# Project-MONAI/MONAI

Hardware: AMD Instinct MI355X
Metric: voxels/s sliding-window 3D seg (512^3 vol, 96^3 win, ov 0.5) at 1/8 GPU (higher is better)
Workload: dtype f32; 1 GPU; BasicUNet 5-class seed 1, 512^3 CT phantom in HBM, 96^3 win ov 0.5 gaussian, sw_batch 4 (engine: <= 64 windows per launch); parallelism=1 GPU

## Files before the change

include/monai_amd.h:

```cpp
#ifndef MONAI_AMD_H
#define MONAI_AMD_H

#include <stddef.h>
#include <stdint.h>

#ifdef __cplusplus
extern "C" {
#endif

#define MH_OK 0
#define MH_ERR_ARG (-1)
#define MH_ERR_LAUNCH (-2)
#define MH_ERR_UNSUPPORTED (-3)

typedef struct mh_tensor5 {
    float* data;
    int64_t n_stride;
    const float* nrm;
    int64_t nrm_n_stride;
    int32_t N, C, D, H, W;
} mh_tensor5;

int mh_version(void);
const char* mh_last_error(void);



int mh_window_extract_f32(const float* vol, int C, int D, int H, int W, const int32_t* sz, int nz,
                          const int32_t* sy, int ny, const int32_t* sx, int nx, int w0, int nwin, int rd, int rh,
                          int rw, float* out, void* stream);

int mh_sw_blend_f32(const float* logits, int64_t window_stride, const float* imp, float* out, int K, int D, int H, int W,
                    int rd, int rh, int rw, const int32_t* sz, int nz, const int32_t* sy, int ny, const int32_t* sx,
                    int nx, int premultiplied, void* stream);

int mh_sw_blend_buffered_f32(const float* logits, int64_t window_stride, const float* imp, float* out, int K, int D, int H, int W, int rd, int rh, int rw,
                             const int32_t* sz, int nz, const int32_t* sy, int ny, const int32_t* sx, int nx, int buffer_axis, int buffer_steps, int premultiplied, void* stream);

int mh_sw_mosaic_class_counts(int n, int log2m, int32_t* counts5);
int mh_sw_blend_mosaic_f32(const float* logits, const int64_t* class_base, int log2m_z, int log2m_y, int log2m_x, const float* imp, int imp_factored, float* out, int K,
                           int D, int H, int W, int rd, int rh, int rw, const int32_t* sz, int nz, const int32_t* sy, int ny, const int32_t* sx, int nx,
                           void* stream);

int mh_sw_blend_argmax_f32(const float* logits, int64_t window_stride, const float* imp, void* labels, int labels_u8, int K, int D,
                           int H, int W, int rd, int rh, int rw, const int32_t* sz, int nz, const int32_t* sy, int ny,
                           const int32_t* sx, int nx, int premultiplied, void* stream);

int mh_patch_accumulate_f32(float* values, uint8_t* counts, const float* patch, int NC, int D, int H, int W, int pd, int ph,
                            int pw, int z0, int y0, int x0, void* stream);
int mh_patch_accumulate_batch_f32(float* values, uint8_t* counts, const float* patches, int npatch, const int32_t* loc, int NC, int D, int H, int W,
                                  int pd, int ph, int pw, void* stream);
int mh_avg_finalize_f32(float* values, const uint8_t* counts, int64_t n, void* stream);


#define MH_ALGO_AUTO 0
#define MH_ALGO_DIRECT 1
#define MH_ALGO_WINO2D 2
#define MH_ALGO_H2 3
#define MH_ALGO_FP32 4
int mh_conv3d_k3_select(int algo, int input_bounded, int Cin, int Cout, int D, int H, int W);
int mh_conv3d_k3_num_configs(void);
int mh_conv3d_k3_h2_config(void);
int mh_conv3d_k3_h2c_config(void);
int mh_conv3d_k3_c1_config(void);
int mh_conv3d_k3_h2v_config(void);
int mh_conv3d_k3_h2w_config(void);
int mh_conv3d_k3_h2w_fits(int D, int H, int W);
int mh_conv3d_k3_accepts(int cfg, int Cin, int Cout);
int64_t mh_conv3d_k3_packed_floats(int cfg, int Cin, int Cout);
int mh_conv3d_k3_pack_f32(int cfg, const float* w, int Cin, int Cout, float* packed, void* stream);
int mh_conv3d_k3_stat_tiles(int cfg, int D, int H, int W);
int mh_conv3d_k3_f32(int cfg, const mh_tensor5* in, const float* packed_w, const float* bias,
                     const mh_tensor5* out, float* stats, void* stream);
int mh_conv3d_k3_pool_accepts(int cfg, int Cin, int Cout, int D, int H, int W);
int mh_conv3d_k3_pool_f32(int cfg, const mh_tensor5* in, const float* packed_w, const float* bias, const mh_tensor5* out, float* stats, float* pool_max, float* pool_min,
                          int64_t pool_n_stride, void* stream);
int mh_pool_select_f32(float* pool_max, const float* pool_min, const float* nrm, int64_t nrm_n_stride, int N, int C, int64_t n_stride, int64_t vol, void* stream);
int mh_conv3d_k3_accumulate_f32(int cfg, const mh_tensor5* in, const float* packed_w, const float* bias, const mh_tensor5* out, float* stats, void* stream);

int mh_instnorm_stat_tiles(int D, int H, int W);
int mh_instnorm_stats_f32(const mh_tensor5* x, float* stats, void* stream);
int mh_instnorm_finalize_f32(const float* stats, int tiles, int N, int C, const float* gamma, const float* beta,
                             float eps, float slope, float* nrm, int64_t nrm_n_stride, void* stream);
int mh_groupnorm_finalize_f32(const float* stats, int tiles, int N, int C, int groups, const float* gamma, const float* beta, float eps,
                              float slope, float* nrm, int64_t nrm_n_stride, void* stream);

int mh_nrm_identity_f32(float* nrm, int N, int C, int64_t nrm_n_stride, void* stream);

int mh_maxpool2_f32(const mh_tensor5* in, const mh_tensor5* out, void* stream);

int mh_deconv_k2s2_f32(const mh_tensor5* in, const float* w, const float* bias, const mh_tensor5* out,
                       void* stream);

int mh_deconv_k2s2_h2_accepts(int Cin, int Cout, int D, int H, int W);
int64_t mh_deconv_k2s2_h2_packed_floats(int Cin, int Cout);
int mh_deconv_k2s2_h2_pack_f32(const float* w, int Cin, int Cout, float* packed, void* stream);
int mh_deconv_k2s2_h2_f32(const mh_tensor5* in, const float* packed, const float* bias, const mh_tensor5* out, void* stream);

int mh_upconv_k4s2_accepts(int Cin, int Cout, int Dl, int Hl, int Wl);
int64_t mh_upconv_k4s2_packed_floats(int Cin, int Cout);
int mh_upconv_k4s2_pack_f32(const float* w4, int Cin, int Cout, float* packed, void* stream);
int mh_upconv_k4s2_stat_tiles(int Dl, int Hl, int Wl);
int mh_upconv_k4s2_f32(const mh_tensor5* low, const float* packed, const float* bias_table, const mh_tensor5* out, int accumulate, float* stats, void* stream);

int mh_conv3d_k3s2_accepts(int Cin, int Cout, int D, int H, int W);
int64_t mh_conv3d_k3s2_packed_floats(int Cin, int Cout);
int64_t mh_conv3d_k3s2_workspace_floats(int N, int Cin, int D, int H, int W);
int mh_conv3d_k3s2_stat_tiles(int D, int H, int W);
int mh_conv3d_k3s2_pack_f32(const float* w, int Cin, int Cout, float* packed, void* stream);
int mh_conv3d_k3s2_f32(const mh_tensor5* in, const float* packed, const float* bias, const mh_tensor5* out, float* workspace, float* stats, int fused, void* stream);

int mh_conv1x1_f32(const mh_tensor5* in, const float* w, const float* bias, const mh_tensor5* out,
                   void* stream);
int mh_conv1x1_stat_tiles(int D, int H, int W);
int mh_conv1x1_stats_f32(const mh_tensor5* in, const float* w, const float* bias, const mh_tensor5* out, float* stats, void* stream);

int mh_conv1x1_h2_accepts(int Cin, int Cout, int D, int H, int W);
int64_t mh_conv1x1_h2_packed_floats(int Cin, int Cout);
int mh_conv1x1_h2_pack_f32(const float* w, int Cout, int Cin, float* packed, void* stream);
int mh_conv1x1_h2_f32(const mh_tensor5* in, const float* packed, const float* bias, const mh_tensor5* out, float* stats, void* stream);

int mh_conv1x1_windows_f32(const mh_tensor5* in, const float* w, const float* bias, float* base, int Cout, const int64_t* place, void* stream);


int mh_add_act_f32(const mh_tensor5* a, const mh_tensor5* b, float slope, const mh_tensor5* out, void* stream);

int mh_conv1x1_sum2_accepts(int Cout, int D, int H, int W);
int mh_conv1x1_sum2_f32(const mh_tensor5* a, const mh_tensor5* b, float slope, const float* w, const float* bias, const mh_tensor5* out, void* stream);

int mh_pad_replicate_f32(const mh_tensor5* in, const mh_tensor5* out, void* stream);

int mh_pixelshuffle_f32(const mh_tensor5* in, const mh_tensor5* out, int fz, int pad_pool, void* stream);

int mh_attention_f32(const float* qkv, float* out, int B, int S, int heads, int head_dim, float scale, void* stream);

int mh_window_attention_f32(const float* qkv, const float* bias_t, const float* mask, float* out, int BW, int nW, int S, int heads,
                            int head_dim, float scale, int exact_fp32, void* stream);

int mh_window_attention_rel_accepts(int S, int head_dim, int table_rows);
int mh_window_attention_rel_f32(const float* qkv, const float* rel_table, int table_rows, const int32_t* coord, int coord_off, const int32_t* region,
                                float* out, int BW, int nW, int S, int heads, int head_dim, float scale, void* stream);

int64_t mh_linear_packed_floats(int N, int K);
int mh_linear_pack_f32(const float* w, int N, int K, float* packed, void* stream);
int mh_linear_f32(const float* x, const float* packed_w, const float* bias, const float* residual, float* y, int64_t M, int N, int K, int act,
                  void* stream);
int mh_linear_tile_f32(const float* x, const float* packed_w, const float* bias, const float* residual, float* y, int64_t M, int N, int K, int act,
                       int tile, void* stream);

int mh_layernorm_f32(const float* x, const float* gamma, const float* beta, float eps, float* y, int64_t M, int K, void* stream);

int mh_layernorm_gather_accepts(int K);
int mh_layernorm_gather_f32(const float* x, const float* gamma, const float* beta, float eps, float* y, int64_t M_out, int K, const int32_t* src_row, void* stream);
int mh_linear_scatter_f32(const float* x, const float* packed_w, const float* bias, const float* residual, float* y, int64_t M, int N, int K, int act,
                          const int32_t* dst_row, void* stream);


int mh_conv3d_k3_strided_f32(const mh_tensor5* in, const float* packed_w, const float* bias, const mh_tensor5* out,
                             int stride, void* stream);
int mh_conv3d_k3_strided3_f32(const mh_tensor5* in, const float* packed_w, const float* bias, const mh_tensor5* out, int sz, int sy, int sx,
                              void* stream);
int mh_deconv_ks_f32(const mh_tensor5* in, const float* w, const float* bias, const mh_tensor5* out, int fz, int fy, int fx, void* stream);

int mh_deconv_k3_f32(const mh_tensor5* in, const float* w, const float* bias, const mh_tensor5* out, int stride,
                     void* stream);


int64_t mh_affine_resample_workspace_bytes(int Do, int Ho, int Wo);
int mh_affine_resample_f32(const float* src, int NC, int Di, int Hi, int Wi, float* dst, int Do, int Ho, int Wo,
                           const double* m, int mode, int pad, int align_corners, int compute_f64, void* workspace,
                           void* stream);

int mh_grid_resample_f32(const float* src, int NC, int Di, int Hi, int Wi, const void* coords, int coords_f64,
                         const double* scale3, const double* offset3, float* dst, int Do, int Ho, int Wo, int mode,
                         int pad, int align_corners, int compute_f64, void* stream);

int mh_grid_pull(const void* src, const void* grid, void* out, int is_f64, int B, int C, int X, int Y, int Z, int Xo,
                 int Yo, int Zo, const int32_t* bound3, const int32_t* interp3, int extrapolate, void* stream);

int mh_pushpull(const void* source, const void* grid, const void* target, void* out, void* grad, int is_f64, int ndim, int B,
                int C, int X, int Y, int Z, int Xo, int Yo, int Zo, const int32_t* bound3, const int32_t* interp3,
                int extrapolate, int do_pull, int do_push, int do_count, int do_grad, int do_sgrad, int target_k, void* stream);


int mh_pointwise_f32(int op, const float* src, float* dst, int64_t n, float param, void* stream);
int mh_channel_reduce_f32(int op, const float* src, float* dst, int C, int64_t n, void* stream);
int mh_onehot_f32(const float* labels, float* dst, int K, int64_t n, void* stream);


int mh_scale_intensity_range_f32(const float* src, float* dst, int64_t n, float a_min, float a_div, int rescale, float b_scale, float b_min,
                                 int clip_lo, float lo, int clip_hi, float hi, void* stream);
int mh_foreground_bbox_workspace_ints(int D, int H);
int mh_foreground_bbox_f32(const float* src, int C, int D, int H, int W, int32_t* workspace, int32_t* box6, void* stream);
int mh_crop_pad_f32(const float* src, float* dst, int C, int D, int H, int W, int Do, int Ho, int Wo, int sz, int sy, int sx, float value,
                    void* stream);

int64_t mh_normalize_stats_workspace_doubles(int C, int64_t n);
int mh_normalize_stats_f32(const float* src, int C, int64_t n, int nonzero, double* workspace, float* subdiv, void* stream);
int mh_normalize_apply_f32(const float* src, float* dst, int C, int64_t n, int nonzero, const float* subdiv, void* stream);
int64_t mh_minmax_workspace_floats(int C, int64_t n);
int mh_minmax_f32(const float* src, int C, int64_t n, float* workspace, float* table, void* stream);
int mh_minmax_scale_f32(const float* src, float* dst, int C, int64_t n, const float* table, int rescale, float b_scale, float b_min,
                        int flat_has_mul, float flat_mul, void* stream);
int64_t mh_select_workspace_bytes(int C);
int mh_order_statistics_f32(const float* src, int C, int64_t n, int R, const int64_t* ranks, void* workspace, float* out, void* stream);
int mh_percentiles_f32(const float* src, int C, int64_t n, int P, const int64_t* ranks, const double* weights, int lerp_mode, void* workspace, float* table,
                       void* stream);
int mh_scale_intensity_table_f32(const float* src, float* dst, int C, int64_t n, const float* table, int rescale, float b_scale, float b_min, int flat_add,
                                 int clip_lo, float lo, int clip_hi, float hi, void* stream);
int mh_clamp_table_f32(const float* src, float* dst, int C, int64_t n, const float* table, void* stream);
int mh_flip_permute_f32(const float* src, float* dst, int C, const int32_t* in_size3, const int32_t* perm3, const int32_t* flip3, void* stream);


#define MH_OV_CHANNEL 0
#define MH_OV_LABELS 1
#define MH_OV_F32 0
#define MH_OV_U8 1
#define MH_OV_I64 2
int64_t mh_overlap_sums_workspace_bytes(int B, int K, int64_t n);
int mh_overlap_sums(const void* pred, int pred_form, int pred_dtype, const void* truth, int truth_form, int truth_dtype, int B, int K,
                    int64_t n, void* workspace, double* out, void* stream);


#define MH_ED_BOOL 3
#define MH_ED_ITEM_WORDS 16

int64_t mh_surface_bbox_workspace_bytes(int B, int nc);
int mh_surface_bbox(const void* pred, int pred_form, int pred_dtype, const void* truth, int truth_form, int truth_dtype, int B, int K, int c0,
                    int nc, int D, int H, int W, void* workspace, int32_t* boxes, void* stream);
// ... 60 lines not shown
```

monai_amd/_lib.py:

```python

from __future__ import annotations

import ctypes as C
import os
from typing import Optional, Sequence

import torch

from ._fallback import UnsupportedOnDevice

_HERE = os.path.dirname(os.path.abspath(__file__))
LIB_PATH = os.environ.get("MONAI_AMD_LIB") or os.path.join(_HERE, "csrc", "libmonai_amd.so")


class MhTensor5(C.Structure):

    _fields_ = [
        ("data", C.c_void_p),
        ("n_stride", C.c_int64),
        ("nrm", C.c_void_p),
        ("nrm_n_stride", C.c_int64),
        ("N", C.c_int32),
        ("C", C.c_int32),
        ("D", C.c_int32),
        ("H", C.c_int32),
        ("W", C.c_int32),
    ]


_I, _L, _P, _F = C.c_int, C.c_int64, C.c_void_p, C.c_float
_T = C.POINTER(MhTensor5)
_IA = C.POINTER(C.c_int32)

SIGNATURES = {
    "mh_version": (_I, []),
    "mh_last_error": (C.c_char_p, []),
    "mh_window_extract_f32": (_I, [_P, _I, _I, _I, _I, _IA, _I, _IA, _I, _IA, _I, _I, _I, _I, _I, _I, _P, _P]),
    "mh_patch_accumulate_f32": (_I, [_P, _P, _P] + [_I] * 10 + [_P]),
    "mh_patch_accumulate_batch_f32": (_I, [_P, _P, _P, _I, _IA] + [_I] * 7 + [_P]),
    "mh_avg_finalize_f32": (_I, [_P, _P, C.c_int64, _P]),
    "mh_pointwise_f32": (_I, [_I, _P, _P, _L, _F, _P]),
    "mh_channel_reduce_f32": (_I, [_I, _P, _P, _I, _L, _P]),
    "mh_onehot_f32": (_I, [_P, _P, _I, _L, _P]),
    "mh_scale_intensity_range_f32": (_I, [_P, _P, _L, _F, _F, _I, _F, _F, _I, _F, _I, _F, _P]),
    "mh_foreground_bbox_workspace_ints": (_I, [_I, _I]),
    "mh_foreground_bbox_f32": (_I, [_P, _I, _I, _I, _I, _P, _P, _P]),
    "mh_crop_pad_f32": (_I, [_P, _P] + [_I] * 10 + [_F, _P]),
    "mh_sw_blend_f32": (_I, [_P, _L, _P, _P, _I, _I, _I, _I, _I, _I, _I, _IA, _I, _IA, _I, _IA, _I, _I, _P]),
    "mh_sw_blend_buffered_f32": (_I, [_P, _L, _P, _P, _I, _I, _I, _I, _I, _I, _I, _IA, _I, _IA, _I, _IA, _I, _I, _I, _I, _P]),
    "mh_sw_mosaic_class_counts": (_I, [_I, _I, _IA]),
    "mh_sw_blend_mosaic_f32": (_I, [_P, C.POINTER(C.c_int64), _I, _I, _I, _P, _I, _P, _I, _I, _I, _I, _I, _I, _I, _IA, _I, _IA, _I, _IA, _I, _P]),
    "mh_sw_blend_argmax_f32": (_I, [_P, _L, _P, _P, _I, _I, _I, _I, _I, _I, _I, _I, _IA, _I, _IA, _I, _IA, _I, _I, _P]),
    "mh_conv3d_k3_select": (_I, [_I, _I, _I, _I, _I, _I, _I]),
    "mh_conv3d_k3_h2_config": (_I, []),
    "mh_conv3d_k3_h2c_config": (_I, []),
    "mh_conv3d_k3_c1_config": (_I, []),
    "mh_conv3d_k3_h2v_config": (_I, []),
    "mh_conv3d_k3_h2w_config": (_I, []),
    "mh_conv3d_k3_h2w_fits": (_I, [_I, _I, _I]),
    "mh_conv3d_k3_num_configs": (_I, []),
    "mh_conv3d_k3_accepts": (_I, [_I, _I, _I]),
    "mh_conv3d_k3_packed_floats": (_L, [_I, _I, _I]),
    "mh_conv3d_k3_pack_f32": (_I, [_I, _P, _I, _I, _P, _P]),
    "mh_conv3d_k3_stat_tiles": (_I, [_I, _I, _I, _I]),
    "mh_conv3d_k3_f32": (_I, [_I, _T, _P, _P, _T, _P, _P]),
    "mh_conv3d_k3_accumulate_f32": (_I, [_I, _T, _P, _P, _T, _P, _P]),
    "mh_conv3d_k3_pool_accepts": (_I, [_I, _I, _I, _I, _I, _I]),
    "mh_conv3d_k3_pool_f32": (_I, [_I, _T, _P, _P, _T, _P, _P, _P, _L, _P]),
    "mh_pool_select_f32": (_I, [_P, _P, _P, _L, _I, _I, _L, _L, _P]),
    "mh_instnorm_stat_tiles": (_I, [_I, _I, _I]),
    "mh_instnorm_stats_f32": (_I, [_T, _P, _P]),
    "mh_instnorm_finalize_f32": (_I, [_P, _I, _I, _I, _P, _P, _F, _F, _P, _L, _P]),
    "mh_groupnorm_finalize_f32": (_I, [_P, _I, _I, _I, _I, _P, _P, _F, _F, _P, _L, _P]),
    "mh_flip_permute_f32": (_I, [_P, _P, _I, _IA, _IA, _IA, _P]),
    "mh_normalize_stats_workspace_doubles": (_L, [_I, _L]),
    "mh_normalize_stats_f32": (_I, [_P, _I, _L, _I, _P, _P, _P]),
    "mh_normalize_apply_f32": (_I, [_P, _P, _I, _L, _I, _P, _P]),
    "mh_minmax_workspace_floats": (_L, [_I, _L]),
    "mh_minmax_f32": (_I, [_P, _I, _L, _P, _P, _P]),
    "mh_minmax_scale_f32": (_I, [_P, _P, _I, _L, _P, _I, _F, _F, _I, _F, _P]),
    "mh_select_workspace_bytes": (_L, [_I]),
    "mh_order_statistics_f32": (_I, [_P, _I, _L, _I, C.POINTER(C.c_int64), _P, _P, _P]),
    "mh_percentiles_f32": (_I, [_P, _I, _L, _I, C.POINTER(C.c_int64), C.POINTER(C.c_double), _I, _P, _P, _P]),
    "mh_scale_intensity_table_f32": (_I, [_P, _P, _I, _L, _P, _I, _F, _F, _I, _I, _F, _I, _F, _P]),
    "mh_clamp_table_f32": (_I, [_P, _P, _I, _L, _P, _P]),
    "mh_nrm_identity_f32": (_I, [_P, _I, _I, _L, _P]),
    "mh_maxpool2_f32": (_I, [_T, _T, _P]),
    "mh_deconv_k2s2_f32": (_I, [_T, _P, _P, _T, _P]),
    "mh_upconv_k4s2_accepts": (_I, [_I, _I, _I, _I, _I]),
    "mh_upconv_k4s2_packed_floats": (_L, [_I, _I]),
    "mh_upconv_k4s2_pack_f32": (_I, [_P, _I, _I, _P, _P]),
    "mh_upconv_k4s2_stat_tiles": (_I, [_I, _I, _I]),
    "mh_upconv_k4s2_f32": (_I, [_T, _P, _P, _T, _I, _P, _P]),
    "mh_deconv_k2s2_h2_accepts": (_I, [_I, _I, _I, _I, _I]),
    "mh_deconv_k2s2_h2_packed_floats": (_L, [_I, _I]),
    "mh_deconv_k2s2_h2_pack_f32": (_I, [_P, _I, _I, _P, _P]),
    "mh_deconv_k2s2_h2_f32": (_I, [_T, _P, _P, _T, _P]),
    "mh_conv3d_k3s2_accepts": (_I, [_I, _I, _I, _I, _I]),
    "mh_conv3d_k3s2_packed_floats": (_L, [_I, _I]),
    "mh_conv3d_k3s2_workspace_floats": (_L, [_I, _I, _I, _I, _I]),
    "mh_conv3d_k3s2_stat_tiles": (_I, [_I, _I, _I]),
    "mh_conv3d_k3s2_pack_f32": (_I, [_P, _I, _I, _P, _P]),
    "mh_conv3d_k3s2_f32": (_I, [_T, _P, _P, _T, _P, _P, _I, _P]),
    "mh_conv1x1_f32": (_I, [_T, _P, _P, _T, _P]),
    "mh_conv1x1_stat_tiles": (_I, [_I, _I, _I]),
    "mh_conv1x1_stats_f32": (_I, [_T, _P, _P, _T, _P, _P]),
    "mh_conv1x1_h2_accepts": (_I, [_I, _I, _I, _I, _I]),
    "mh_conv1x1_h2_packed_floats": (_L, [_I, _I]),
    "mh_conv1x1_h2_pack_f32": (_I, [_P, _I, _I, _P, _P]),
    "mh_conv1x1_h2_f32": (_I, [_T, _P, _P, _T, _P, _P]),
    "mh_conv1x1_sum2_accepts": (_I, [_I, _I, _I, _I]),
    "mh_conv1x1_sum2_f32": (_I, [_T, _T, _F, _P, _P, _T, _P]),
    "mh_conv1x1_windows_f32": (_I, [_T, _P, _P, _P, _I, C.POINTER(C.c_int64), _P]),
    "mh_conv3d_k3_strided_f32": (_I, [_T, _P, _P, _T, _I, _P]),
    "mh_conv3d_k3_strided3_f32": (_I, [_T, _P, _P, _T, _I, _I, _I, _P]),
    "mh_deconv_ks_f32": (_I, [_T, _P, _P, _T, _I, _I, _I, _P]),
    "mh_deconv_k3_f32": (_I, [_T, _P, _P, _T, _I, _P]),
    "mh_add_act_f32": (_I, [_T, _T, _F, _T, _P]),
    "mh_pad_replicate_f32": (_I, [_T, _T, _P]),
    "mh_pixelshuffle_f32": (_I, [_T, _T, _I, _I, _P]),
    "mh_attention_f32": (_I, [_P, _P, _I, _I, _I, _I, _F, _P]),
    "mh_window_attention_f32": (_I, [_P, _P, _P, _P, _I, _I, _I, _I, _I, _F, _I, _P]),
    "mh_window_attention_rel_accepts": (_I, [_I, _I, _I]),
    "mh_window_attention_rel_f32": (_I, [_P, _P, _I, _P, _I, _P, _P, _I, _I, _I, _I, _I, _F, _P]),
    "mh_linear_packed_floats": (_L, [_I, _I]),
    "mh_linear_pack_f32": (_I, [_P, _I, _I, _P, _P]),
    "mh_linear_f32": (_I, [_P, _P, _P, _P, _P, _L, _I, _I, _I, _P]),
    "mh_linear_tile_f32": (_I, [_P, _P, _P, _P, _P, _L, _I, _I, _I, _I, _P]),
    "mh_layernorm_f32": (_I, [_P, _P, _P, _F, _P, _L, _I, _P]),
    "mh_layernorm_gather_accepts": (_I, [_I]),
    "mh_layernorm_gather_f32": (_I, [_P, _P, _P, _F, _P, _L, _I, _P, _P]),
    "mh_linear_scatter_f32": (_I, [_P, _P, _P, _P, _P, _L, _I, _I, _I, _P, _P]),
    "mh_affine_resample_workspace_bytes": (_L, [_I, _I, _I]),
    "mh_affine_resample_f32": (_I, [_P, _I, _I, _I, _I, _P, _I, _I, _I, C.POINTER(C.c_double), _I, _I, _I, _I, _P, _P]),
    "mh_separable_filter3d_f32": (_I, [_P, _P, _I, _I, _I, _I, C.POINTER(C.c_float), _I, C.POINTER(C.c_float), _I, C.POINTER(C.c_float), _I, _P]),
    "mh_median_filter_accepts": (_I, [_I, _I, _I, _I, _I, _I]),
    "mh_median_filter_f32": (_I, [_P, _P, _I, _I, _I, _I, _I, _I, _I, _P]),
    "mh_spline_workspace_bytes": (_L, [_I] * 7),
    "mh_spline_prefilter_f64": (_I, [_P, _P] + [_I] * 7 + [_P]),
    "mh_spline_resample_affine_f32": (_I, [_P, _I, _I, _I, _I, _I, _P, _I, _I, _I, C.POINTER(C.c_double), _I, _I, _P]),
    "mh_spline_resample_grid_f32": (_I, [_P, _I, _I, _I, _I, _I, _P, _I, C.POINTER(C.c_double), C.POINTER(C.c_double), _P, _I, _I, _I, _I, _I, _P]),
    "mh_grid_pull": (_I, [_P, _P, _P, _I, _I, _I, _I, _I, _I, _I, _I, _I, _IA, _IA, _I, _P]),
    "mh_pushpull": (_I, [_P, _P, _P, _P, _P] + [_I] * 10 + [_IA, _IA] + [_I] * 7 + [_P]),
    "mh_grid_resample_f32": (_I, [_P, _I, _I, _I, _I, _P, _I, C.POINTER(C.c_double), C.POINTER(C.c_double), _P, _I, _I, _I, _I, _I, _I, _I, _P]),
    "mh_overlap_sums_workspace_bytes": (_L, [_I, _I, _L]),
    "mh_overlap_sums": (_I, [_P, _I, _I, _P, _I, _I, _I, _I, _L, _P, _P, _P]),
    "mh_surface_bbox_workspace_bytes": (_L, [_I, _I]),
    "mh_surface_bbox": (_I, [_P, _I, _I, _P, _I, _I] + [_I] * 7 + [_P, _P, _P]),
    "mh_mask_edges": (_I, [_P, _I, _I, _I, _I, _I, _I, _I, _I, _P, _P, _I, _L, _P, _P]),
    "mh_edt_workspace_bytes": (_L, [_L, _I]),
    "mh_edt": (_I, [_P, _I, _I, _P, _P, _I, _L, _I, _P, _P, _I, _P]),
    "mh_surface_records_workspace_bytes": (_L, [_I]),
    "mh_surface_records": (_I, [_P, _P, _I, _P, _P, _I, _L, _I, _P, _P, _P, _L, _P]),
    "mh_cc_label": (_I, [_P, _I, _L, _I, _I, _P, _P, _I, _L, _P, _P]),
    "mh_cc_records": (_I, [_P, _I, _P, _P, _I, _L, _P, _P, _P]),
    "mh_cc_keep": (_I, [_P, _I, _L, _P, _P, _I, _I, _P, _P, _I, _L, _P]),
    "mh_cc_fill": (_I, [_P, _I, _L, _P, _P, _I, _P, _P, _I, _L, _P]),
    "mh_cc_filter": (_I, [_P, _P, _I, _L, C.POINTER(C.c_double), _I, _P]),
}


class KernelRejected(RuntimeError):
    """An entry point declined a VALID call it has no kernel for (MH_ERR_UNSUPPORTED: a size / shape rule) without launching: callers with an alternative
    path catch THIS, not RuntimeError.  Bad arguments (MH_ERR_ARG: null pointers, mismatched shapes, misalignment -- caller bugs), launch failures and HIP
    errors stay plain RuntimeErrors and must surface."""


class Library:

    def __init__(self, path: str):
        if not os.path.exists(path):
            raise RuntimeError(
                f"monai_amd: HIP extension not built ({path} missing). Run `python -m monai_amd.build` "
                "(hipcc --offload-arch=gfx950); there is no CPU fallback."
            )
        self.path = path
        self._dll = C.CDLL(path)
        for name, (res, args) in SIGNATURES.items():
            fn = getattr(self._dll, name)
            fn.restype, fn.argtypes = res, args
            setattr(self, "_" + name, fn)

    def last_error(self) -> str:
        return self._mh_last_error().decode("utf-8", "replace")

    def check(self, rc: int) -> None:
        if rc == -3:
            raise KernelRejected(f"monai_amd: {self.last_error()} (code {rc})")
        if rc != 0:
            raise RuntimeError(f"monai_amd: {self.last_error()} (code {rc})")

    def call(self, name: str, *args) -> None:
        self.check(getattr(self, "_" + name)(*args))

    def query(self, name: str, *args) -> int:
        rc = getattr(self, "_" + name)(*args)
        if rc < 0:
            raise RuntimeError(f"monai_amd: {self.last_error()} (code {rc})")
        return int(rc)


_LIB: Optional[Library] = None


def lib() -> Library:
    global _LIB
    if _LIB is None:
        _LIB = Library(LIB_PATH)
    return _LIB


def require_device(*tensors: torch.Tensor, dtypes=(torch.float32,)) -> None:
    for t in tensors:
        if t is None:
            continue
        if not t.is_cuda:
            raise UnsupportedOnDevice(
                "monai_amd: this path runs only on an MI355X (ROCm) device tensor; got a CPU tensor. "
                "There is no CPU fallback in the product path."
            )
        if t.dtype not in dtypes:
# ... 35 lines not shown
```

monai_amd/config.py:

```python
import os

HAS_EXT = True
USE_COMPILED = HAS_EXT and os.getenv("BUILD_MONAI", "0") == "1"


CONV_ALGOS = {"auto": 0, "direct": 1, "wino2d": 2, "h2": 3, "fp32": 4}
CONV_ALGO = None


def conv_algo() -> int:
    name = CONV_ALGO if CONV_ALGO is not None else os.environ.get("MONAI_AMD_CONV_ALGO", "auto")
    try:
        return CONV_ALGOS[str(name).lower()]
    except KeyError:
        raise ValueError(f"monai_amd: unknown convolution family {name!r} (one of {sorted(CONV_ALGOS)})") from None


class conv_algo_scope:

    def __init__(self, name: str):
        if str(name).lower() not in CONV_ALGOS:
            raise ValueError(f"monai_amd: unknown convolution family {name!r} (one of {sorted(CONV_ALGOS)})")
        self.name = str(name).lower()

    def __enter__(self):
        global CONV_ALGO
        self._saved, CONV_ALGO = CONV_ALGO, self.name
        return self

    def __exit__(self, *exc):
        global CONV_ALGO
        CONV_ALGO = self._saved
        return False


UPCAT_FUSED = None


def upcat_fused() -> bool:
    v = UPCAT_FUSED if UPCAT_FUSED is not None else os.environ.get("MONAI_AMD_UPCAT_FUSED", "1")
    return str(v).lower() not in ("0", "false", "off", "no")


UPCAT_ORDER = None


def upcat_order() -> str:
    v = str(UPCAT_ORDER if UPCAT_ORDER is not None else os.environ.get("MONAI_AMD_UPCAT_ORDER", "conv_first")).lower()
    if v not in ("conv_first", "term_first"):
        raise ValueError(f"monai_amd: unknown UpCat order {v!r} (conv_first or term_first)")
    return v


CONV_HALVES = None


def conv_halves() -> bool:
    v = CONV_HALVES if CONV_HALVES is not None else os.environ.get("MONAI_AMD_CONV_HALVES", "1")
    return str(v).lower() not in ("0", "false", "off", "no")


RESIDUAL_ACC = None


def residual_accumulate() -> bool:
    v = RESIDUAL_ACC if RESIDUAL_ACC is not None else os.environ.get("MONAI_AMD_RESIDUAL_ACC", "1")
    return str(v).lower() not in ("0", "false", "off", "no")


POOL_FUSED = None


def pool_fused() -> bool:
    v = POOL_FUSED if POOL_FUSED is not None else os.environ.get("MONAI_AMD_POOL_FUSED", "1")
    return str(v).lower() not in ("0", "false", "off", "no")


STRIDED_H2 = None


def strided_h2() -> bool:
    v = STRIDED_H2 if STRIDED_H2 is not None else os.environ.get("MONAI_AMD_STRIDED_H2", "1")
    return str(v).lower() not in ("0", "false", "off", "no") and conv_algo() in (CONV_ALGOS["auto"], CONV_ALGOS["h2"])


STRIDED_H2_FUSED = None


def strided_h2_fused() -> str:
    v = str(STRIDED_H2_FUSED if STRIDED_H2_FUSED is not None else os.environ.get("MONAI_AMD_STRIDED_H2_FUSED", "auto")).lower()
    return "0" if v in ("0", "false", "off", "no") else ("1" if v in ("1", "true", "on", "yes") else "auto")


SMALL_VOLUME_H2 = None


def small_volume_h2() -> bool:
    v = SMALL_VOLUME_H2 if SMALL_VOLUME_H2 is not None else os.environ.get("MONAI_AMD_SMALL_VOLUME_H2", "1")
    return str(v).lower() not in ("0", "false", "off", "no")


DECONV_H2 = None


def deconv_h2() -> bool:
    v = DECONV_H2 if DECONV_H2 is not None else os.environ.get("MONAI_AMD_DECONV_H2", "1")
    return str(v).lower() not in ("0", "false", "off", "no") and conv_algo() in (CONV_ALGOS["auto"], CONV_ALGOS["h2"])


SWIN_FUSED_MOVES = None


def swin_fused_moves() -> bool:
    v = SWIN_FUSED_MOVES if SWIN_FUSED_MOVES is not None else os.environ.get("MONAI_AMD_SWIN_FUSED_MOVES", "1")
    return str(v).lower() not in ("0", "false", "off", "no")


SWIN_REL_ATTENTION = None


def swin_rel_attention() -> bool:
    v = SWIN_REL_ATTENTION if SWIN_REL_ATTENTION is not None else os.environ.get("MONAI_AMD_SWIN_REL_ATTENTION", "1")
    return str(v).lower() not in ("0", "false", "off", "no")
```

monai_amd/csrc/capi.hip:

```cpp
#include <hip/hip_runtime.h>

#include <stdarg.h>
#include <stdio.h>
#include <stdlib.h>
#include <string.h>

#include "kernels/common.h"
#include "kernels/attention.h"
#include "kernels/conv3d_mfma.h"
#include "kernels/conv3d_wino2p.h"
#include "kernels/conv3d_h2.h"
#include "kernels/conv3d_wino_h2.h"
#include "kernels/upconv_h2.h"
#include "kernels/conv3d_s2_h2.h"
#include "kernels/deconv_h2.h"
#include "kernels/conv3d_vol_h2.h"
#include "kernels/conv3d_c1.h"
#include "kernels/dense.h"
#include "kernels/gaussian.h"
#include "kernels/grid_pull.h"
#include "kernels/pushpull.h"
#include "kernels/post.h"
#include "kernels/metrics.h"
#include "kernels/edt.h"
// ... 238 lines not shown
    }
    WindowGrid g;
    if (int e = fill_grid(g, sz, nz, sy, ny, sx, nx)) return e;
    for (int k0 = 0; k0 < K; k0 += 8) {
        const int kt = K - k0 < 8 ? K - k0 : 8;
        if (v4) launch_blend<4>(kt, blocks_for(total), (hipStream_t)stream, logits, imp, out, K, k0, D, H, W, rd, rh, rw, g, premultiplied ? 1 : 0, window_stride);
        else launch_blend<1>(kt, blocks_for(total), (hipStream_t)stream, logits, imp, out, K, k0, D, H, W, rd, rh, rw, g, premultiplied ? 1 : 0, window_stride);
    }
    return launched("sw_blend");
}

int mh_sw_blend_buffered_f32(const float* logits, int64_t window_stride, const float* imp, float* out, int K, int D, int H, int W, int rd, int rh, int rw,
                             const int32_t* sz, int nz, const int32_t* sy, int ny, const int32_t* sx, int nx, int buffer_axis, int buffer_steps, int premultiplied, void* stream) {
    if (int e = blend_checks("sw_blend_buffered", logits, imp, out, K, D, H, W, rd, rh, rw, sz, nz, sy, ny, sx, nx, window_stride)) return e;
    if (buffer_axis < 0 || buffer_axis > 2 || buffer_steps < 1) return fail(MH_ERR_ARG, "sw_blend_buffered: buffer_axis in 0..2 and buffer_steps >= 1 (got %d, %d)", buffer_axis, buffer_steps);
    const bool v4 = W % 4 == 0 && rw % 4 == 0 && all_mult4(sx, nx);
    const long long total = (long long)D * H * (v4 ? W / 4 : W);
    WindowGrid g;
    if (int e = fill_grid(g, sz, nz, sy, ny, sx, nx)) return e;
    hipStream_t s = (hipStream_t)stream;
    for (int k0 = 0; k0 < K; k0 += 4) {
        const int kt = K - k0 < 4 ? K - k0 : 4;
#define MH_BB(KT_, V_)                                                                                                                                          \
    {                                                                                                                                                          \
        if (premultiplied) hipLaunchKernelGGL((sw_blend_buffered_kernel<KT_, V_, true>), dim3(blocks_for(total)), dim3(256), 0, s, logits, imp, out, K, k0, D, H, W, rd, rh, rw, g, buffer_axis, buffer_steps, (long long)window_stride); \
        else hipLaunchKernelGGL((sw_blend_buffered_kernel<KT_, V_, false>), dim3(blocks_for(total)), dim3(256), 0, s, logits, imp, out, K, k0, D, H, W, rd, rh, rw, g, buffer_axis, buffer_steps, (long long)window_stride);           \
    }
        if (v4) { if (kt == 4) MH_BB(4, 4) else if (kt == 3) MH_BB(3, 4) else if (kt == 2) MH_BB(2, 4) else MH_BB(1, 4) }
        else { if (kt == 4) MH_BB(4, 1) else if (kt == 3) MH_BB(3, 1) else if (kt == 2) MH_BB(2, 1) else MH_BB(1, 1) }
#undef MH_BB
    }
    return launched("sw_blend_buffered");
}

#ifndef MH_BLEND_IDX32_LIMIT
#define MH_BLEND_IDX32_LIMIT (1LL << 31)
#endif
int mh_sw_mosaic_class_counts(int n, int log2m, int32_t* counts5) {
    if (n < 1 || log2m < 0 || log2m > 2 || !counts5) return fail(MH_ERR_ARG, "sw_mosaic_class_counts: bad argument (1, 2 or 4 residue classes)");
    MosaicAxis a;
    mosaic_axis_fill(a, n, log2m);
    for (int c = 0; c < MOSAIC_MAX_CLASSES; ++c) counts5[c] = a.cnt[c];
    return MH_OK;
}

int mh_sw_blend_mosaic_f32(const float* logits, const int64_t* class_base, int log2m_z, int log2m_y, int log2m_x, const float* imp, int imp_factored, float* out, int K,
                           int D, int H, int W, int rd, int rh, int rw, const int32_t* sz, int nz, const int32_t* sy, int ny, const int32_t* sx, int nx,
                           void* stream) {
    int64_t dense = 0;
    if (int e = blend_checks("sw_blend_mosaic", logits, imp, out, K, D, H, W, rd, rh, rw, sz, nz, sy, ny, sx, nx, dense)) return e;
    if (!class_base || log2m_z < 0 || log2m_z > 2 || log2m_y < 0 || log2m_y > 2 || log2m_x < 0 || log2m_x > 2) return fail(MH_ERR_ARG, "sw_blend_mosaic: bad layout");
    if (K < 1 || K > 8) return fail(MH_ERR_UNSUPPORTED, "sw_blend_mosaic: 1 .. 8 classes (got %d): use the window-major layout", K);
    RegGrid rg;
    if (!regular_grid(rg, sz, nz, sy, ny, sx, nx, D, H, W)) return fail(MH_ERR_UNSUPPORTED, "sw_blend_mosaic: irregular window starts (use the window-major layout)");
    if (!(W % 4 == 0 && rw % 4 == 0 && all_mult4(sx, nx) && aligned(logits, 16) && aligned(imp, 16) && aligned(out, 16)) || (imp_factored && (rd + rh) % 4))
        return fail(MH_ERR_UNSUPPORTED, "sw_blend_mosaic: needs W, roi width and window starts divisible by 4 and 16-byte aligned buffers");
    const AxisWin* ax[3] = {&rg.z, &rg.y, &rg.x};
    const int lm[3] = {log2m_z, log2m_y, log2m_x}, rr[3] = {rd, rh, rw};
    for (int a = 0; a < 3; ++a)
        if (ax[a]->n > 2 && (long long)ax[a]->step << lm[a] < rr[a]) return fail(MH_ERR_ARG, "sw_blend_mosaic: %d residue classes do not separate the windows of axis %d", 1 << lm[a], a);
    Mosaic ms;
    mosaic_axis_fill(ms.z, nz, log2m_z); mosaic_axis_fill(ms.y, ny, log2m_y); mosaic_axis_fill(ms.x, nx, log2m_x);
    for (int i = 0; i < MOSAIC_MAX_CLASSES * MOSAIC_MAX_CLASSES * MOSAIC_MAX_CLASSES; ++i) {
        if (class_base[i] % 4) return fail(MH_ERR_ARG, "sw_blend_mosaic: class offsets must be multiples of 4 floats");
        ms.base[i] = class_base[i];
    }
    if (D > 65535) return fail(MH_ERR_UNSUPPORTED, "sw_blend_mosaic: more than 65535 planes (use the window-major layout)");
    const unsigned nb = blocks_for((long long)H * (W / 4));
    hipStream_t s = (hipStream_t)stream;
    long long max_cs = 0, max_zy = 0, max_ext = std::max((long long)rd * rh, (long long)rw);
    for (int a = 0; a < MOSAIC_MAX_CLASSES; ++a)
        for (int b = 0; b < MOSAIC_MAX_CLASSES; ++b) {
            const long long zy = (long long)ms.z.cnt[a] * rd * ((long long)ms.y.cnt[b] * rh);
            max_zy = std::max(max_zy, zy);
            for (int c = 0; c < MOSAIC_MAX_CLASSES; ++c) {
                max_cs = std::max(max_cs, zy * ((long long)ms.x.cnt[c] * rw));
                max_ext = std::max(max_ext, std::max((long long)ms.z.cnt[a] * rd, std::max((long long)ms.y.cnt[b] * rh, (long long)ms.x.cnt[c] * rw)));
            }
        }
    const bool fast = max_cs * K < MH_BLEND_IDX32_LIMIT && max_zy < (1LL << 24) && max_ext < (1LL << 23) && std::max(D, std::max(H, W)) < (1 << 23) && knob_int("MONAI_AMD_BLEND_IDX64", 0) == 0;
#define MH_BM(KT, G_, NT_, SEP_) { if (fast) hipLaunchKernelGGL((sw_blend_mosaic_kernel<KT, G_, NT_, SEP_, true>), dim3(nb, D), dim3(256), 0, s, logits, imp, out, K, D, H, W, rd, rh, rw, rg, ms); \
                                   else hipLaunchKernelGGL((sw_blend_mosaic_kernel<KT, G_, NT_, SEP_, false>), dim3(nb, D), dim3(256), 0, s, logits, imp, out, K, D, H, W, rd, rh, rw, rg, ms); }
#ifdef MH_DEV_KNOBS
    if (K == 5 && !imp_factored) {
        const int g_ = knob_int("MONAI_AMD_BLEND_G", MH_BLEND_G), nt_ = knob_int("MONAI_AMD_BLEND_NT", 0);
        if (g_ == 1 && !nt_) { MH_BM(5, 1, false, false) return launched("sw_blend_mosaic"); }
        if (g_ == 1 && nt_) { MH_BM(5, 1, true, false) return launched("sw_blend_mosaic"); }
        if (g_ == 2 && nt_) { MH_BM(5, 2, true, false) return launched("sw_blend_mosaic"); }
        if (g_ == 4 && !nt_) { MH_BM(5, 4, false, false) return launched("sw_blend_mosaic"); }
        if (g_ == 4 && nt_) { MH_BM(5, 4, true, false) return launched("sw_blend_mosaic"); }
    }
#endif
#define MH_BM_CASE(KT) case KT: if (imp_factored) MH_BM(KT, MH_BLEND_G, false, true) else MH_BM(KT, MH_BLEND_G, false, false) break;
    switch (K) { MH_BM_CASE(1) MH_BM_CASE(2) MH_BM_CASE(3) MH_BM_CASE(4) MH_BM_CASE(5) MH_BM_CASE(6) MH_BM_CASE(7) MH_BM_CASE(8) }
#undef MH_BM_CASE
#undef MH_BM
    return launched("sw_blend_mosaic");
}

int mh_sw_blend_argmax_f32(const float* logits, int64_t window_stride, const float* imp, void* labels, int labels_u8, int K, int D, int H, int W, int rd,
                           int rh, int rw, const int32_t* sz, int nz, const int32_t* sy, int ny, const int32_t* sx, int nx, int premultiplied, void* stream) {
    if (int e = blend_checks("sw_blend_argmax", logits, imp, labels, K, D, H, W, rd, rh, rw, sz, nz, sy, ny, sx, nx, window_stride)) return e;
    if (labels_u8 && K > 256) return fail(MH_ERR_UNSUPPORTED, "sw_blend_argmax: %d classes do not fit a uint8 label", K);
    RegGrid rg;
    if (!regular_grid(rg, sz, nz, sy, ny, sx, nx, D, H, W))
        return fail(MH_ERR_UNSUPPORTED, "sw_blend_argmax: irregular window starts (blend, then argmax)");
    const bool v4 = W % 4 == 0 && rw % 4 == 0 && window_stride % 4 == 0 && all_mult4(sx, nx) && aligned(logits, 16) && aligned(imp, 16) &&
                    aligned(labels, labels_u8 ? 4 : 16);
    const long long total = (long long)D * H * (v4 ? W / 4 : W);
    const bool nt = knob_int("MONAI_AMD_BLEND_NT", MH_BLEND_NT) != 0;
    if (int e = launch_blend_reg<true>(K < 8 ? K : 8, v4, MH_BLEND_G, nt, blocks_for(total), (hipStream_t)stream, logits, imp, labels, K, 0, D, H, W, rd, rh,
                                       rw, rg, premultiplied ? 1 : 0, labels_u8 ? 1 : 0, window_stride))
        return e;
    return launched("sw_blend_argmax");
}

typedef ConvCfg<32, 1, 1, 4, 4, 1, 1, 8, 2> Cfg1;
typedef ConvCfg<16, 2, 1, 4, 4, 1, 1, 8, 2> Cfg2;
typedef ConvCfg<8, 4, 1, 2, 2, 2, 1, 8, 2> Cfg3;
typedef ConvCfg<4, 4, 2, 1, 1, 4, 1, 4, 2> Cfg4;
typedef ConvCfg<4, 4, 2, 1, 1, 4, 2, 2, 2> Cfg5;
typedef ConvCfg<8, 4, 1, 2, 4, 1, 1, 8, 2> Cfg6;
typedef ConvCfg<32, 1, 1, 4, 4, 1, 1, 2, 4> Cfg7;
typedef ConvCfg<32, 1, 1, 4, 4, 1, 1, 4, 3> Cfg8;
typedef ConvCfg<16, 2, 1, 4, 4, 1, 1, 4, 3> Cfg9;
typedef ConvCfg<16, 2, 1, 4, 4, 1, 1, 2, 4> Cfg10;
typedef ConvCfg<8, 4, 1, 2, 2, 2, 1, 4, 3> Cfg11;
typedef ConvCfg<8, 4, 1, 2, 2, 2, 1, 2, 4> Cfg12;
typedef ConvCfg<4, 4, 2, 1, 1, 4, 1, 2, 4> Cfg13;
typedef ConvCfg<8, 4, 1, 2, 4, 1, 1, 2, 4> Cfg14;
#define MH_NUM_CFG 14

struct CfgInfo { int tx, ty, tz, cn, cc; };
#define MH_CFG_ROW(C) {C::TX, C::TY, C::TZ, C::CN, C::CC}
static const CfgInfo kCfg[MH_NUM_CFG + 1] = {
    {0, 0, 0, 0, 0}, MH_CFG_ROW(Cfg1), MH_CFG_ROW(Cfg2), MH_CFG_ROW(Cfg3), MH_CFG_ROW(Cfg4), MH_CFG_ROW(Cfg5),
    MH_CFG_ROW(Cfg6), MH_CFG_ROW(Cfg7), MH_CFG_ROW(Cfg8), MH_CFG_ROW(Cfg9), MH_CFG_ROW(Cfg10), MH_CFG_ROW(Cfg11),
    MH_CFG_ROW(Cfg12), MH_CFG_ROW(Cfg13), MH_CFG_ROW(Cfg14),
};
static const double kPref[MH_NUM_CFG + 1] = {0, 1.00, 1.00, 1.00, 1.00, 0.90, 1.00, 1.06, 1.04, 1.03, 1.05, 1.01, 1.02, 1.01, 1.02};
static inline int cdiv(int a, int b) { return (a + b - 1) / b; }
static inline int cin_padded(int cfg, int Cin) { return cfg == 0 ? Cin : cdiv(Cin, kCfg[cfg].cc) * kCfg[cfg].cc; }
static inline int cout_padded(int cfg, int Cout) { return cfg == 0 ? Cout : cdiv(Cout, kCfg[cfg].cn) * kCfg[cfg].cn; }

#define MH_CFG_WINO2D (MH_NUM_CFG + 1)
#define MH_CFG_H2 (MH_NUM_CFG + 2)
#define MH_CFG_C1 (MH_NUM_CFG + 3)
#define MH_CFG_H2C (MH_NUM_CFG + 5)
#define MH_CFG_H2V (MH_NUM_CFG + 6)
#define MH_CFG_H2W (MH_NUM_CFG + 7)
#ifndef MH_H2W_DEFAULT
#define MH_H2W_DEFAULT 1
#endif
#define MH_CFG_LAST MH_CFG_H2W
static inline bool hv_fits(int D, int H, int W) {
    const long long vol = (long long)D * H * W, padded = (long long)(D + 2) * (H + 2) * (W + 2);
    return vol >= 64 && vol <= 256 && padded <= HV_CELLS;
}
static inline int c1_chunks(int D) { return D >= 48 ? D / 24 : 1; }
static inline int c1_zchunk(int D) { return cdiv(D, c1_chunks(D)); }
static inline int c1_blocks(int D, int H, int W) { return cdiv(W, C1_TX) * cdiv(H, C1_TY) * cdiv(D, c1_zchunk(D)); }
static inline int wino2d_chunks(int D, int H, int W) {
    const int blocks = cdiv(W, W2_B) * cdiv(H, W2_B);
    if (const char* e = knob_str("MONAI_AMD_W2_CHUNKS")) {
        const int v = atoi(e);
        if (v >= 1 && v <= D) return v;
    }
    int nchunk = cdiv(16, blocks);
    if (nchunk > D / 12) nchunk = D / 12;
    if (nchunk < 1) nchunk = 1;
    return nchunk;
}
static inline int wino2d_zchunk(int D, int H, int W) { return cdiv(D, wino2d_chunks(D, H, W)); }
static inline int wino2d_blocks(int D, int H, int W) { return cdiv(W, W2_B) * cdiv(H, W2_B) * cdiv(D, wino2d_zchunk(D, H, W)); }
static inline bool h2_fits(int D, int H, int W) { return (long long)D * H * W * H2_CN * 4 < 0x80000000LL; }
static inline int h2_regions(int H, int W) { return h2_wide(H, W) ? cdiv(W, 32) * cdiv(H, 8) : cdiv(W, H2_B) * cdiv(H, H2_B); }
static inline int h2_zchunk(int D, int H, int W) {
    int nchunk = cdiv(16, h2_regions(H, W));
    if (const char* e = knob_str("MONAI_AMD_W2_CHUNKS")) {
        const int v = atoi(e);
        if (v >= 1 && v <= D) return cdiv(D, v);
    }
    if (nchunk > D / 12) nchunk = D / 12;
    if (nchunk < 1) nchunk = 1;
    return cdiv(D, nchunk);
}
static inline int h2_blocks(int D, int H, int W) { return h2_regions(H, W) * cdiv(D, h2_zchunk(D, H, W)); }
static inline bool hw_fits(int D, int H, int W) { return H >= HWG_BY && W >= HWG_BX && H % HWG_BY == 0 && W % HWG_BX == 0 && D >= 2 && h2_fits(D, H, W); }
static inline int hw_regions(int H, int W) { return (H / HWG_BY) * (W / HWG_BX); }
static inline int hw_zchunk(int D, int H, int W) {
    int nchunk = cdiv(32, hw_regions(H, W));
    if (const char* e = knob_str("MONAI_AMD_HW_CHUNKS")) {
        const int v = atoi(e);
        if (v >= 1 && v <= D) nchunk = v;
    }
    if (nchunk > D / 12) nchunk = D / 12;
    if (nchunk < 1) nchunk = 1;
    int zc = cdiv(D, nchunk);
    zc += zc & 1;
    return zc;
}
static inline int hw_blocks(int D, int H, int W) { return hw_regions(H, W) * cdiv(D, hw_zchunk(D, H, W)); }

int mh_conv3d_k3_num_configs(void) { return MH_CFG_WINO2D; }
int mh_conv3d_k3_h2_config(void) { return MH_CFG_H2; }
int mh_conv3d_k3_h2c_config(void) { return MH_CFG_H2C; }
int mh_conv3d_k3_c1_config(void) { return MH_CFG_C1; }
int mh_conv3d_k3_h2v_config(void) { return MH_CFG_H2V; }
int mh_conv3d_k3_h2w_config(void) { return MH_CFG_H2W; }
int mh_conv3d_k3_h2w_fits(int D, int H, int W) { return hw_fits(D, H, W) ? 1 : 0; }

int mh_conv3d_k3_pool_accepts(int cfg, int Cin, int Cout, int D, int H, int W) {
    if (cfg == MH_CFG_H2W) return Cin == HWG_CIN && Cout >= HWG_CN && Cout % HWG_CN == 0 && D % 2 == 0 && hw_fits(D, H, W);
    if (cfg != MH_CFG_H2 || D < 2 || H < 2 || W < 2 || D % 2 || H % 2 || W % 4) return 0;
    if (!(Cin >= H2_KC && Cin % H2_KC == 0 && Cin <= H2_NRM_MAX && Cout >= H2_CN && Cout % (H2_CN / 2) == 0) || !h2_fits(D, H, W)) return 0;
    return !h2_wide(H, W) && h2_zchunk(D, H, W) % 2 == 0;
}
int mh_conv3d_k3_accepts(int cfg, int Cin, int Cout) {
    if (cfg == 0) return 1;
    if (cfg == MH_CFG_WINO2D) return Cin >= 8 && Cin % 8 == 0 && Cout >= W2_CN && Cout % W2_CN == 0;
    if (cfg == MH_CFG_H2) return Cin >= H2_KC && Cin % H2_KC == 0 && Cin <= H2_NRM_MAX && Cout >= H2_CN && Cout % (H2_CN / 2) == 0;
    if (cfg == MH_CFG_H2C) return Cin >= H2_KC && Cin % H2_KC == 0 && Cin <= H2_NRM_MAX && Cout >= 16 && Cout % 16 == 0;
    if (cfg == MH_CFG_C1) return Cin == 1 && Cout >= 8 && Cout % 8 == 0;
    if (cfg == MH_CFG_H2V) return Cin >= 16 && Cin % 16 == 0 && Cin <= HV_CIN_MAX && Cout >= 32 && Cout % 32 == 0;
    if (cfg == MH_CFG_H2W) return Cin == HWG_CIN && Cout >= HWG_CN && Cout % HWG_CN == 0;
    if (cfg < 0 || cfg > MH_NUM_CFG) return 0;
    return Cout >= 1 && cin_padded(cfg, Cin) <= Cfg1::NRM_MAX;
}

int mh_conv3d_k3_select(int algo, int input_bounded, int Cin, int Cout, int D, int H, int W) {
    if (Cin < 1 || Cout < 1 || D < 1 || H < 1 || W < 1) return fail(MH_ERR_ARG, "conv3d_k3_select: bad argument");
    if (algo < MH_ALGO_AUTO || algo > MH_ALGO_FP32) return fail(MH_ERR_ARG, "conv3d_k3_select: unknown algorithm family %d", algo);
    int best = 0;
    double best_score = 0.0;
    for (int c = 1; c <= MH_NUM_CFG; ++c) {
        const CfgInfo& k = kCfg[c];
        if (!mh_conv3d_k3_accepts(c, Cin, Cout)) continue;
        const double util = (double)D * H * W / ((double)cdiv(D, k.tz) * k.tz * cdiv(H, k.ty) * k.ty * cdiv(W, k.tx) * k.tx);
        const double cpad = ((double)Cin / cin_padded(c, Cin)) * ((double)Cout / cout_padded(c, Cout));
        const double score = util * cpad * (1.0 + 0.02 * (k.cn / 32)) * kPref[c];
        if (score > best_score) { best_score = score; best = c; }
    }
    if (mh_conv3d_k3_accepts(MH_CFG_WINO2D, Cin, Cout) && H % 2 == 0 && W % 8 == 0) {
        const bool big = H % W2_B == 0 && W % W2_B == 0 && D >= 48 && H >= 48 && W >= 48;
        if (algo == MH_ALGO_WINO2D || ((algo == MH_ALGO_AUTO || algo == MH_ALGO_FP32) && big)) best = MH_CFG_WINO2D;
    }
    if ((algo == MH_ALGO_AUTO || algo == MH_ALGO_H2) && input_bounded && mh_conv3d_k3_accepts(MH_CFG_H2, Cin, Cout) && W % 4 == 0 && H >= 8 && W >= 8 && h2_fits(D, H, W))
        best = MH_CFG_H2;
    if ((algo == MH_ALGO_AUTO || algo == MH_ALGO_H2) && input_bounded && Cout == 16 && mh_conv3d_k3_accepts(MH_CFG_H2C, Cin, Cout) && W % 4 == 0 && H >= 8 && W >= 8 && h2_fits(D, H, W)
        && knob_int("MONAI_AMD_H2C", 1) != 0)
        best = MH_CFG_H2C;
    if ((algo == MH_ALGO_AUTO || algo == MH_ALGO_H2) && input_bounded && best != MH_CFG_H2 && best != MH_CFG_H2C && mh_conv3d_k3_accepts(MH_CFG_H2V, Cin, Cout) && hv_fits(D, H, W))
        best = MH_CFG_H2V;
    if (algo == MH_ALGO_AUTO && best == MH_CFG_H2 && mh_conv3d_k3_accepts(MH_CFG_H2W, Cin, Cout) && hw_fits(D, H, W) && D >= 24 && knob_int("MONAI_AMD_H2W", MH_H2W_DEFAULT) != 0)
        best = MH_CFG_H2W;
    if (algo != MH_ALGO_DIRECT && algo != MH_ALGO_WINO2D && mh_conv3d_k3_accepts(MH_CFG_C1, Cin, Cout) && W % 4 == 0 && knob_int("MONAI_AMD_C1", 1) != 0)
        best = MH_CFG_C1;
    return best;
}

int64_t mh_conv3d_k3_packed_floats(int cfg, int Cin, int Cout) {
    if (cfg == MH_CFG_WINO2D) return (int64_t)(Cin / W2_KC) * (Cout / W2_CN) * W2_UBUF;
    if (cfg == MH_CFG_H2) return (int64_t)(Cin / H2_KC) * cdiv(Cout, H2_CN) * H2_WB * 4 + H2_TAIL;
    if (cfg == MH_CFG_H2C) return (int64_t)(Cin / H2_KC) * (Cout / 16) * H2_WB * 4 + H2_TAIL;
    if (cfg == MH_CFG_C1) return (int64_t)27 * Cout;
    if (cfg == MH_CFG_H2V) return (int64_t)Cout * Cin * 27 + H2_TAIL;
    if (cfg == MH_CFG_H2W) return (int64_t)(Cout / HWG_CN) * HWG_WAVES * HWG_OPS * 64 * 4 + H2_TAIL;
    if (cfg < 0 || cfg > MH_NUM_CFG) return fail(MH_ERR_ARG, "conv3d_k3: unknown configuration %d", cfg);
    return (int64_t)cin_padded(cfg, Cin) * cout_padded(cfg, Cout) * 27;
}

int mh_conv3d_k3_pack_f32(int cfg, const float* w, int Cin, int Cout, float* packed, void* stream) {
    if (cfg == MH_CFG_WINO2D) {
        if (!w || !packed || !mh_conv3d_k3_accepts(cfg, Cin, Cout)) return fail(MH_ERR_ARG, "conv3d_k3_pack: in-plane Winograd needs Cin %% 8 == 0, Cout %% 16 == 0");
        if (hipMemsetAsync(packed, 0, sizeof(float) * (size_t)mh_conv3d_k3_packed_floats(cfg, Cin, Cout), (hipStream_t)stream) != hipSuccess)
            return fail(MH_ERR_LAUNCH, "conv3d_k3_pack: memset failed");
        hipLaunchKernelGGL(conv3d_k3_wino2d_pack_kernel, dim3(blocks_for((long long)Cin * Cout)), dim3(256), 0, (hipStream_t)stream, w, Cin, Cout, packed);
        return launched("conv3d_k3_wino2d_pack");
    }
    if (cfg == MH_CFG_H2C) {
        if (!w || !packed || !mh_conv3d_k3_accepts(cfg, Cin, Cout)) return fail(MH_ERR_ARG, "conv3d_k3_pack: the 16-couts fp16 split kernel needs Cin %% 16 == 0, Cout %% 16 == 0");
        const int64_t slab_floats = mh_conv3d_k3_packed_floats(cfg, Cin, Cout) - H2_TAIL;
        float* tail = packed + slab_floats;
        if (hipMemsetAsync(packed, 0, sizeof(float) * (size_t)slab_floats, (hipStream_t)stream) != hipSuccess)
            return fail(MH_ERR_LAUNCH, "conv3d_k3_pack: memset failed");
        hipLaunchKernelGGL(conv3d_k3_h2_scale_kernel, dim3(1), dim3(1024), 0, (hipStream_t)stream, w, (long long)Cin * Cout * 27, tail);
        hipLaunchKernelGGL(conv3d_k3_h2c_pack_kernel, dim3(blocks_for((long long)Cin * Cout)), dim3(256), 0, (hipStream_t)stream, w, Cin, Cout,
                           reinterpret_cast<_Float16*>(packed), tail);
        return launched("conv3d_k3_h2c_pack");
    }
    if (cfg == MH_CFG_H2) {
        if (!w || !packed || !mh_conv3d_k3_accepts(cfg, Cin, Cout)) return fail(MH_ERR_ARG, "conv3d_k3_pack: the fp16 split kernel needs Cin %% 16 == 0, Cout %% 16 == 0, Cout >= 32");
        const int64_t slab_floats = mh_conv3d_k3_packed_floats(cfg, Cin, Cout) - H2_TAIL;
        float* tail = packed + slab_floats;
        if (hipMemsetAsync(packed, 0, sizeof(float) * (size_t)slab_floats, (hipStream_t)stream) != hipSuccess)
            return fail(MH_ERR_LAUNCH, "conv3d_k3_pack: memset failed");
        hipLaunchKernelGGL(conv3d_k3_h2_scale_kernel, dim3(1), dim3(1024), 0, (hipStream_t)stream, w, (long long)Cin * Cout * 27, tail);
        hipLaunchKernelGGL(conv3d_k3_h2_pack_kernel, dim3(blocks_for((long long)Cin * Cout)), dim3(256), 0, (hipStream_t)stream, w, Cin, Cout,
                           reinterpret_cast<_Float16*>(packed), tail);
        return launched("conv3d_k3_h2_pack");
    }
    if (cfg == MH_CFG_H2W) {
        if (!w || !packed || !mh_conv3d_k3_accepts(cfg, Cin, Cout)) return fail(MH_ERR_ARG, "conv3d_k3_pack: the Winograd split kernel needs Cin == 32, Cout %% 32 == 0");
        float* tail = packed + (mh_conv3d_k3_packed_floats(cfg, Cin, Cout) - H2_TAIL);
        hipLaunchKernelGGL(conv3d_k3_h2_scale_kernel, dim3(1), dim3(1024), 0, (hipStream_t)stream, w, (long long)Cin * Cout * 27, tail);
        hipLaunchKernelGGL(conv3d_k3_h2w_scale_fix_kernel, dim3(1), dim3(64), 0, (hipStream_t)stream, tail);
        hipLaunchKernelGGL(conv3d_k3_h2w_pack_kernel, dim3(blocks_for((long long)Cin * Cout)), dim3(256), 0, (hipStream_t)stream, w, Cin, Cout,
                           reinterpret_cast<_Float16*>(packed), tail);
        return launched("conv3d_k3_h2w_pack");
    }
    if (cfg == MH_CFG_H2V) {
        if (!w || !packed || !mh_conv3d_k3_accepts(cfg, Cin, Cout)) return fail(MH_ERR_ARG, "conv3d_k3_pack: the small-volume split kernel needs Cin %% 16 == 0 (<= 768), Cout %% 32 == 0");
        float* tail = packed + (mh_conv3d_k3_packed_floats(cfg, Cin, Cout) - H2_TAIL);
        hipLaunchKernelGGL(conv3d_k3_h2_scale_kernel, dim3(1), dim3(1024), 0, (hipStream_t)stream, w, (long long)Cin * Cout * 27, tail);
        hipLaunchKernelGGL(conv3d_k3_vol_h2_pack_kernel, dim3(blocks_for((long long)Cin * Cout)), dim3(256), 0, (hipStream_t)stream, w, Cin, Cout, Cout % 64 == 0 ? 2 : 1,
                           reinterpret_cast<_Float16*>(packed), tail);
        return launched("conv3d_k3_vol_h2_pack");
    }
    if (cfg == MH_CFG_C1) {
        if (!w || !packed || !mh_conv3d_k3_accepts(cfg, Cin, Cout)) return fail(MH_ERR_ARG, "conv3d_k3_pack: the one-channel kernel needs Cin == 1, Cout %% 8 == 0");
        hipLaunchKernelGGL(conv3d_k3_pack_kernel, dim3(blocks_for(27LL * Cout)), dim3(256), 0, (hipStream_t)stream, w, 1, 1, Cout, Cout, Cout, packed);
        return launched("conv3d_k3_pack");
    }
    if (cfg < 0 || cfg > MH_NUM_CFG || !w || !packed) return fail(MH_ERR_ARG, "conv3d_k3_pack: bad argument");
    const int cn = cfg == 0 ? Cout : kCfg[cfg].cn;
    const int cinp = cin_padded(cfg, Cin), coutp = cout_padded(cfg, Cout);
    hipLaunchKernelGGL(conv3d_k3_pack_kernel, dim3(blocks_for((long long)cinp * coutp * 27)), dim3(256), 0, (hipStream_t)stream, w,
                       Cin, cinp, Cout, coutp, cn, packed);
    return launched("conv3d_k3_pack");
}

int mh_conv3d_k3_stat_tiles(int cfg, int D, int H, int W) {
    if (cfg == MH_CFG_WINO2D) return wino2d_blocks(D, H, W);
    if (cfg == MH_CFG_H2 || cfg == MH_CFG_H2C) return h2_blocks(D, H, W);
    if (cfg == MH_CFG_C1) return c1_blocks(D, H, W);
    if (cfg == MH_CFG_H2V) return 1;
    if (cfg == MH_CFG_H2W) return hw_fits(D, H, W) ? hw_blocks(D, H, W) : 0;
    if (cfg < 1 || cfg > MH_NUM_CFG) return 0;
    const CfgInfo& k = kCfg[cfg];
    return cdiv(W, k.tx) * cdiv(H, k.ty) * cdiv(D, k.tz);
}

template <class Cfg>
static void launch_mfma(const Tensor& in, const float* wp, const float* bias, const Tensor& out, float* stats, hipStream_t s) {
    const int tx = cdiv(out.W, Cfg::TX), ty = cdiv(out.H, Cfg::TY), tz = cdiv(out.D, Cfg::TZ);
    const dim3 grid((unsigned)(tx * ty * tz), (unsigned)cdiv(out.C, Cfg::CN), (unsigned)out.N);
    if (stats)
        hipLaunchKernelGGL((conv3d_k3_mfma_kernel<Cfg, true>), grid, dim3(256), 0, s, in, wp, bias, out, stats, tx, ty, tz);
    else
        hipLaunchKernelGGL((conv3d_k3_mfma_kernel<Cfg, false>), grid, dim3(256), 0, s, in, wp, bias, out, stats, tx, ty, tz);
}

struct PoolOut { float* mx; float* mn; long long n_stride; };
static int conv3d_k3_launch(int cfg, const mh_tensor5* in_, const float* packed_w, const float* bias, const mh_tensor5* out_, float* stats, void* stream, bool accumulate,
                            const PoolOut* pool = nullptr);
int mh_conv3d_k3_pool_accepts(int cfg, int Cin, int Cout, int D, int H, int W);
int mh_conv3d_k3_pool_f32(int cfg, const mh_tensor5* in_, const float* packed_w, const float* bias, const mh_tensor5* out_, float* stats, float* pool_max, float* pool_min,
                          int64_t pool_n_stride, void* stream) {
    if (!in_ || !out_ || !pool_max || !pool_min || !stats || !in_->nrm) return fail(MH_ERR_ARG, "conv3d_k3_pool: input records, statistics and both pooled tensors are required");
    if (!mh_conv3d_k3_pool_accepts(cfg, in_->C, out_->C, out_->D, out_->H, out_->W))
        return fail(MH_ERR_UNSUPPORTED, "conv3d_k3_pool: the pooling epilogue exists for the split-precision configuration on even extents with 16 x 16 regions");
    if (!aligned(pool_max, 8) || !aligned(pool_min, 8) || pool_n_stride % 2 || (long long)out_->C * (out_->D / 2) * (out_->H / 2) * (out_->W / 2) > pool_n_stride)
        return fail(MH_ERR_ARG, "conv3d_k3_pool: pooled tensors must be 8-byte aligned [N][>= C][D/2][H/2][W/2]");
    const PoolOut po{pool_max, pool_min, (long long)pool_n_stride};
    return conv3d_k3_launch(cfg, in_, packed_w, bias, out_, stats, stream, false, &po);
}
int mh_pool_select_f32(float* pool_max, const float* pool_min, const float* nrm, int64_t nrm_n_stride, int N, int C, int64_t n_stride, int64_t vol, void* stream) {
    if (!pool_max || !pool_min || !nrm || N < 1 || C < 1 || vol < 1) return fail(MH_ERR_ARG, "pool_select: bad argument");
    const unsigned nb = (unsigned)std::min<long long>(blocks_for(vol), 64);
    hipLaunchKernelGGL(pool_select_kernel, dim3(nb, (unsigned)C, (unsigned)N), dim3(256), 0, (hipStream_t)stream, pool_max, pool_min, nrm, (long long)nrm_n_stride, (long long)n_stride, (long long)vol);
    return launched("pool_select");
}
int mh_conv3d_k3_f32(int cfg, const mh_tensor5* in_, const float* packed_w, const float* bias, const mh_tensor5* out_,
                     float* stats, void* stream) {
    return conv3d_k3_launch(cfg, in_, packed_w, bias, out_, stats, stream, false);
}
int mh_conv3d_k3_accumulate_f32(int cfg, const mh_tensor5* in_, const float* packed_w, const float* bias, const mh_tensor5* out_,
                                float* stats, void* stream) {
    if ((cfg != MH_CFG_H2 && cfg != MH_CFG_H2C && cfg != MH_CFG_H2W) || !stats || !in_ || !in_->nrm)
        return fail(MH_ERR_UNSUPPORTED, "conv3d_k3_accumulate: the accumulating form exists for the split-precision configuration with input records and statistics");
    return conv3d_k3_launch(cfg, in_, packed_w, bias, out_, stats, stream, true);
}
static int conv3d_k3_launch(int cfg, const mh_tensor5* in_, const float* packed_w, const float* bias, const mh_tensor5* out_,
                            float* stats, void* stream, bool accumulate, const PoolOut* pool) {
    if (!dense_ok(in_) || !dense_ok(out_) || !packed_w) return fail(MH_ERR_ARG, "conv3d_k3: bad tensor");
    const Tensor in = from_c(*in_), out = from_c(*out_);
    if (in.N != out.N || in.D != out.D || in.H != out.H || in.W != out.W) return fail(MH_ERR_ARG, "conv3d_k3: shape mismatch");
    if (cfg < 0 || cfg > MH_CFG_LAST) return fail(MH_ERR_ARG, "conv3d_k3: unknown configuration %d", cfg);
    if (in.nrm && !aligned(in.nrm, 16)) return fail(MH_ERR_ARG, "conv3d_k3: nrm must be 16-byte aligned");
    hipStream_t s = (hipStream_t)stream;
    if (cfg == MH_CFG_C1) {
        if (!mh_conv3d_k3_accepts(cfg, in.C, out.C) || in.W % 4)
            return fail(MH_ERR_ARG, "conv3d_k3: the one-channel kernel needs Cin == 1, Cout %% 8 == 0, W %% 4 == 0 (got %d -> %d, %dx%dx%d)", in.C, out.C,
                        in.D, in.H, in.W);
        if (!aligned(out.data, 16) || out.n_stride % 4 || !aligned(in.data, 16) || in.n_stride % 4 || !aligned(packed_w, 4))
            return fail(MH_ERR_ARG, "conv3d_k3: the one-channel kernel needs 16-byte aligned input and output");
        const int txn = cdiv(out.W, C1_TX), tyn = cdiv(out.H, C1_TY), zc = c1_zchunk(out.D);
        constexpr int cot = 8;
        const dim3 grid((unsigned)(txn * tyn * cdiv(out.D, zc)), (unsigned)(out.C / cot), (unsigned)out.N);
        if (stats && in.nrm) hipLaunchKernelGGL((conv3d_k3_c1_kernel<cot, true, true>), grid, dim3(256), 0, s, in, packed_w, bias, out, stats, txn, tyn, zc);
        else if (stats) hipLaunchKernelGGL((conv3d_k3_c1_kernel<cot, true, false>), grid, dim3(256), 0, s, in, packed_w, bias, out, stats, txn, tyn, zc);
        else if (in.nrm) hipLaunchKernelGGL((conv3d_k3_c1_kernel<cot, false, true>), grid, dim3(256), 0, s, in, packed_w, bias, out, stats, txn, tyn, zc);
        else hipLaunchKernelGGL((conv3d_k3_c1_kernel<cot, false, false>), grid, dim3(256), 0, s, in, packed_w, bias, out, stats, txn, tyn, zc);
        return launched("conv3d_k3_c1");
    }
    if (cfg == MH_CFG_H2W) {
        if (!mh_conv3d_k3_accepts(cfg, in.C, out.C) || !hw_fits(in.D, in.H, in.W))
            return fail(MH_ERR_ARG, "conv3d_k3: the Winograd split kernel needs Cin == 32, Cout %% 32 == 0, H %% 4 == 0, W %% 16 == 0, D*H*W < 2^24 (got %d -> %d, %dx%dx%d)",
                        in.C, out.C, in.D, in.H, in.W);
        if (!in.nrm) return fail(MH_ERR_ARG, "conv3d_k3: the Winograd split kernel needs input records with magnitude bounds");
        if (!aligned(out.data, 16) || out.n_stride % 4 || !aligned(packed_w, 16)) return fail(MH_ERR_ARG, "conv3d_k3: the Winograd split kernel needs 16-byte aligned output and weights");
        if ((accumulate || pool) && !stats) return fail(MH_ERR_ARG, "conv3d_k3: the accumulating / pooling forms leave statistics");
        const int bxn = out.W / HWG_BX, byn = out.H / HWG_BY, zc = hw_zchunk(out.D, out.H, out.W);
        const unsigned nblk = (unsigned)(bxn * byn * cdiv(out.D, zc));
        const long long total = (long long)nblk * (out.C / HWG_CN) * out.N;
        if (total > 0x7fffffffLL) return fail(MH_ERR_UNSUPPORTED, "conv3d_k3: problem too large for one launch");
        const dim3 grid((unsigned)total);
        const uint4* wq = reinterpret_cast<const uint4*>(packed_w);
        const float* tail = packed_w + (mh_conv3d_k3_packed_floats(cfg, in.C, out.C) - H2_TAIL);
        if (pool) hipLaunchKernelGGL((conv3d_k3_h2w_kernel<true, false, true>), grid, dim3(64 * HWG_WAVES), 0, s, in, wq, tail, bias, out, stats, bxn, byn, zc, nblk, pool->mx, pool->mn, pool->n_stride);
        else if (accumulate) hipLaunchKernelGGL((conv3d_k3_h2w_kernel<true, true, false>), grid, dim3(64 * HWG_WAVES), 0, s, in, wq, tail, bias, out, stats, bxn, byn, zc, nblk, (float*)nullptr, (float*)nullptr, 0LL);
        else if (stats) hipLaunchKernelGGL((conv3d_k3_h2w_kernel<true, false, false>), grid, dim3(64 * HWG_WAVES), 0, s, in, wq, tail, bias, out, stats, bxn, byn, zc, nblk, (float*)nullptr, (float*)nullptr, 0LL);
        else hipLaunchKernelGGL((conv3d_k3_h2w_kernel<false, false, false>), grid, dim3(64 * HWG_WAVES), 0, s, in, wq, tail, bias, out, stats, bxn, byn, zc, nblk, (float*)nullptr, (float*)nullptr, 0LL);
        return launched("conv3d_k3_h2w");
    }
    if (cfg == MH_CFG_H2V) {
        if (accumulate || pool) return fail(MH_ERR_UNSUPPORTED, "conv3d_k3: the small-volume split kernel has no accumulating / pooling form");
        if (!mh_conv3d_k3_accepts(cfg, in.C, out.C) || !hv_fits(in.D, in.H, in.W))
            return fail(MH_ERR_ARG, "conv3d_k3: the small-volume split kernel needs Cin %% 16 == 0 (<= 768), Cout %% 32 == 0, 64 <= D*H*W <= 256, (D+2)(H+2)(W+2) <= 512 (got %d -> %d, %dx%dx%d)",
                        in.C, out.C, in.D, in.H, in.W);
        if (!in.nrm) return fail(MH_ERR_ARG, "conv3d_k3: the small-volume split kernel needs input records with magnitude bounds");
        if (!aligned(out.data, 16) || out.n_stride % 4 || !aligned(packed_w, 16)) return fail(MH_ERR_ARG, "conv3d_k3: the small-volume split kernel needs 16-byte aligned output and weights");
        const int ncgw = out.C % 64 == 0 ? 2 : 1;
        const long long total = (long long)(out.C / (32 * ncgw)) * out.N;
        if (total > 0x7fffffffLL) return fail(MH_ERR_UNSUPPORTED, "conv3d_k3: problem too large for one launch");
        const uint4* wq = reinterpret_cast<const uint4*>(packed_w);
        const float* tail = packed_w + (mh_conv3d_k3_packed_floats(cfg, in.C, out.C) - H2_TAIL);
        const dim3 grid((unsigned)total);
        if (ncgw == 2) {
            if (stats) hipLaunchKernelGGL((conv3d_k3_vol_h2_kernel<2, true>), grid, dim3(HV_NT), 0, s, in, wq, tail, bias, out, stats);
            else hipLaunchKernelGGL((conv3d_k3_vol_h2_kernel<2, false>), grid, dim3(HV_NT), 0, s, in, wq, tail, bias, out, stats);
        } else {
            if (stats) hipLaunchKernelGGL((conv3d_k3_vol_h2_kernel<1, true>), grid, dim3(HV_NT), 0, s, in, wq, tail, bias, out, stats);
            else hipLaunchKernelGGL((conv3d_k3_vol_h2_kernel<1, false>), grid, dim3(HV_NT), 0, s, in, wq, tail, bias, out, stats);
        }
        return launched("conv3d_k3_vol_h2");
    }
    if (cfg == MH_CFG_H2 || cfg == MH_CFG_H2C) {
        const bool c16 = cfg == MH_CFG_H2C;
        if (!mh_conv3d_k3_accepts(cfg, in.C, out.C) || in.W % 4)
            return fail(MH_ERR_ARG, "conv3d_k3: the fp16 split kernel needs Cin %% 16 == 0, Cout %% 16 == 0 (>= 32; any multiple of 16 in its 16-couts form), W %% 4 == 0 (got %d -> %d, %dx%dx%d)",
                        in.C, out.C, in.D, in.H, in.W);
        if (!aligned(out.data, 16) || out.n_stride % 4 || !aligned(packed_w, 16))
            return fail(MH_ERR_ARG, "conv3d_k3: the fp16 split kernel needs 16-byte aligned output and weights");
        if (!h2_fits(out.D, out.H, out.W))
            return fail(MH_ERR_UNSUPPORTED, "conv3d_k3: the fp16 split kernel addresses 32 output planes with 32-bit offsets (D*H*W < 2^24 voxels); mh_conv3d_k3_select does not return it beyond");
        const bool wide = h2_wide(out.H, out.W);
        const int bxn = wide ? cdiv(out.W, 32) : cdiv(out.W, H2_B), byn = wide ? cdiv(out.H, 8) : cdiv(out.H, H2_B), zc = h2_zchunk(out.D, out.H, out.W);
        const unsigned nblk = (unsigned)(bxn * byn * cdiv(out.D, zc));
        const long long total = (long long)nblk * (c16 ? out.C / 16 : cdiv(out.C, H2_CN)) * out.N;
        if (total > 0x7fffffffLL) return fail(MH_ERR_UNSUPPORTED, "conv3d_k3: problem too large for one launch");
        const dim3 grid((unsigned)total);
        const uint4* wq = reinterpret_cast<const uint4*>(packed_w);
        const float* tail = packed_w + (mh_conv3d_k3_packed_floats(cfg, in.C, out.C) - H2_TAIL);
#define MH_H2_LAUNCH(RES_, WIDE_, C16_)                                                                                                                  \
    {                                                                                                                                                \
        if (stats && in.nrm) hipLaunchKernelGGL((conv3d_k3_h2_kernel<true, true, RES_, WIDE_, C16_>), grid, dim3(512), 0, s, in, wq, tail, bias, out, stats, bxn, byn, zc, nblk, (float*)nullptr, (float*)nullptr, 0LL);   \
        else if (stats) hipLaunchKernelGGL((conv3d_k3_h2_kernel<true, false, RES_, WIDE_, C16_>), grid, dim3(512), 0, s, in, wq, tail, bias, out, stats, bxn, byn, zc, nblk, (float*)nullptr, (float*)nullptr, 0LL);       \
        else if (in.nrm) hipLaunchKernelGGL((conv3d_k3_h2_kernel<false, true, RES_, WIDE_, C16_>), grid, dim3(512), 0, s, in, wq, tail, bias, out, stats, bxn, byn, zc, nblk, (float*)nullptr, (float*)nullptr, 0LL);      \
        else hipLaunchKernelGGL((conv3d_k3_h2_kernel<false, false, RES_, WIDE_, C16_>), grid, dim3(512), 0, s, in, wq, tail, bias, out, stats, bxn, byn, zc, nblk, (float*)nullptr, (float*)nullptr, 0LL);                 \
    }
        if (pool) {
#define MH_H2_POOL(RES_) hipLaunchKernelGGL((conv3d_k3_h2_kernel<true, true, RES_, false, false, false, true>), grid, dim3(512), 0, s, in, wq, tail, bias, out, stats, bxn, byn, zc, nblk, pool->mx, pool->mn, pool->n_stride)
            if (in.C <= 2 * H2_KC) MH_H2_POOL(true); else MH_H2_POOL(false);
#undef MH_H2_POOL
            return launched("conv3d_k3_h2_pool");
        }
        if (accumulate) {
#define MH_H2_ACC(RES_, WIDE_, C16_) hipLaunchKernelGGL((conv3d_k3_h2_kernel<true, true, RES_, WIDE_, C16_, true>), grid, dim3(512), 0, s, in, wq, tail, bias, out, stats, bxn, byn, zc, nblk, (float*)nullptr, (float*)nullptr, 0LL)
            if (c16) {
                if (in.C <= 2 * H2_KC) { if (wide) MH_H2_ACC(true, true, true); else MH_H2_ACC(true, false, true); }
                else { if (wide) MH_H2_ACC(false, true, true); else MH_H2_ACC(false, false, true); }
            } else {
                if (in.C <= 2 * H2_KC) { if (wide) MH_H2_ACC(true, true, false); else MH_H2_ACC(true, false, false); }
                else { if (wide) MH_H2_ACC(false, true, false); else MH_H2_ACC(false, false, false); }
            }
#undef MH_H2_ACC
            return launched("conv3d_k3_h2_acc");
        }
        if (c16) {
            if (in.C <= 2 * H2_KC) { if (wide) MH_H2_LAUNCH(true, true, true) else MH_H2_LAUNCH(true, false, true) }
            else { if (wide) MH_H2_LAUNCH(false, true, true) else MH_H2_LAUNCH(false, false, true) }
        } else {
            if (in.C <= 2 * H2_KC) { if (wide) MH_H2_LAUNCH(true, true, false) else MH_H2_LAUNCH(true, false, false) }
            else { if (wide) MH_H2_LAUNCH(false, true, false) else MH_H2_LAUNCH(false, false, false) }
        }
#undef MH_H2_LAUNCH
        return launched(c16 ? "conv3d_k3_h2c" : "conv3d_k3_h2");
    }
    if (cfg == MH_CFG_WINO2D) {
        if (!mh_conv3d_k3_accepts(cfg, in.C, out.C) || in.H % 2 || in.W % 8)
            return fail(MH_ERR_ARG, "conv3d_k3: in-plane Winograd needs Cin %% 8 == 0, Cout %% 16 == 0, even H and W %% 8 == 0 (got %d -> %d, %dx%dx%d)",
                        in.C, out.C, in.D, in.H, in.W);
        if (!aligned(out.data, 16) || out.n_stride % 4 || !aligned(packed_w, 16))
            return fail(MH_ERR_ARG, "conv3d_k3: in-plane Winograd needs 16-byte aligned output and weights");
        const int bxn = cdiv(out.W, W2_B), byn = cdiv(out.H, W2_B), zc = wino2d_zchunk(out.D, out.H, out.W);
        const unsigned nblk = (unsigned)(bxn * byn * cdiv(out.D, zc));
        const long long total = (long long)nblk * (out.C / W2_CN) * out.N;
        if (total > 0x7fffffffLL) return fail(MH_ERR_UNSUPPORTED, "conv3d_k3: problem too large for one launch");
        const dim3 grid((unsigned)total);
        if (stats && in.nrm) hipLaunchKernelGGL((conv3d_k3_wino2p_kernel<true, true>), grid, dim3(512), 0, s, in, packed_w, bias, out, stats, bxn, byn, zc, nblk);
        else if (stats) hipLaunchKernelGGL((conv3d_k3_wino2p_kernel<true, false>), grid, dim3(512), 0, s, in, packed_w, bias, out, stats, bxn, byn, zc, nblk);
        else if (in.nrm) hipLaunchKernelGGL((conv3d_k3_wino2p_kernel<false, true>), grid, dim3(512), 0, s, in, packed_w, bias, out, stats, bxn, byn, zc, nblk);
        else hipLaunchKernelGGL((conv3d_k3_wino2p_kernel<false, false>), grid, dim3(512), 0, s, in, packed_w, bias, out, stats, bxn, byn, zc, nblk);
        return launched("conv3d_k3_wino2p");
    }
    if (cfg == 0) {
        if (stats) return fail(MH_ERR_ARG, "conv3d_k3: the direct kernel emits no statistics");
        constexpr int COT = 16;
        const dim3 grid(blocks_for((long long)out.D * out.H * out.W), (unsigned)cdiv(out.C, COT), (unsigned)out.N);
        hipLaunchKernelGGL((conv3d_k3_direct_kernel<COT>), grid, dim3(256), 0, s, in, packed_w, bias, out);
        return launched("conv3d_k3_direct");
    }
    const CfgInfo& k = kCfg[cfg];
    (void)k;
    if (!mh_conv3d_k3_accepts(cfg, in.C, out.C))
        return fail(MH_ERR_ARG, "conv3d_k3: configuration %d does not take Cin=%d Cout=%d", cfg, in.C, out.C);
    if (!aligned(packed_w, 16)) return fail(MH_ERR_ARG, "conv3d_k3: packed weights must be 16-byte aligned");
    switch (cfg) {
        case 1: launch_mfma<Cfg1>(in, packed_w, bias, out, stats, s); break;
        case 2: launch_mfma<Cfg2>(in, packed_w, bias, out, stats, s); break;
        case 3: launch_mfma<Cfg3>(in, packed_w, bias, out, stats, s); break;
        case 4: launch_mfma<Cfg4>(in, packed_w, bias, out, stats, s); break;
        case 5: launch_mfma<Cfg5>(in, packed_w, bias, out, stats, s); break;
        case 6: launch_mfma<Cfg6>(in, packed_w, bias, out, stats, s); break;
        case 7: launch_mfma<Cfg7>(in, packed_w, bias, out, stats, s); break;
        case 8: launch_mfma<Cfg8>(in, packed_w, bias, out, stats, s); break;
        case 9: launch_mfma<Cfg9>(in, packed_w, bias, out, stats, s); break;
        case 10: launch_mfma<Cfg10>(in, packed_w, bias, out, stats, s); break;
        case 11: launch_mfma<Cfg11>(in, packed_w, bias, out, stats, s); break;
        case 12: launch_mfma<Cfg12>(in, packed_w, bias, out, stats, s); break;
        case 13: launch_mfma<Cfg13>(in, packed_w, bias, out, stats, s); break;
        case 14: launch_mfma<Cfg14>(in, packed_w, bias, out, stats, s); break;
    }
    return launched("conv3d_k3_mfma");
}

int mh_instnorm_stat_tiles(int D, int H, int W) {
    return (int)(((long long)D * H * W + STAT_CHUNK - 1) / STAT_CHUNK);
}

int mh_instnorm_stats_f32(const mh_tensor5* x_, float* stats, void* stream) {
    if (!dense_ok(x_) || !stats) return fail(MH_ERR_ARG, "instnorm_stats: bad argument");
    const Tensor x = from_c(*x_);
    const int tiles = mh_instnorm_stat_tiles(x.D, x.H, x.W);
    hipLaunchKernelGGL(instnorm_stats_kernel, dim3((unsigned)tiles, (unsigned)x.C, (unsigned)x.N), dim3(256), 0,
                       (hipStream_t)stream, x, stats, tiles);
    return launched("instnorm_stats");
}

int mh_instnorm_finalize_f32(const float* stats, int tiles, int N, int C, const float* gamma, const float* beta, float eps,
                             float slope, float* nrm, int64_t nrm_n_stride, void* stream) {
    if (!stats || !nrm || tiles < 1 || N < 1 || C < 1 || nrm_n_stride < 4LL * C) return fail(MH_ERR_ARG, "instnorm_finalize: bad argument");
    hipLaunchKernelGGL(instnorm_finalize_kernel, dim3((unsigned)C, (unsigned)N), dim3(64), 0, (hipStream_t)stream, stats, tiles,
                       C, 1, gamma, beta, eps, slope, nrm, (long long)nrm_n_stride);
    return launched("instnorm_finalize");
}

int mh_groupnorm_finalize_f32(const float* stats, int tiles, int N, int C, int groups, const float* gamma, const float* beta, float eps,
                              float slope, float* nrm, int64_t nrm_n_stride, void* stream) {
    if (!stats || !nrm || tiles < 1 || N < 1 || C < 1 || groups < 1 || C % groups || nrm_n_stride < 4LL * C)
        return fail(MH_ERR_ARG, "groupnorm_finalize: bad argument (channels must be divisible by groups)");
    hipLaunchKernelGGL(instnorm_finalize_kernel, dim3((unsigned)groups, (unsigned)N), dim3(64), 0, (hipStream_t)stream, stats, tiles,
                       C, C / groups, gamma, beta, eps, slope, nrm, (long long)nrm_n_stride);
    return launched("groupnorm_finalize");
}
// ... 1792 lines not shown
```

monai_amd/csrc/kernels/conv3d_wino_h2.h:

```cpp
#pragma once
#include "common.h"
#include "conv3d_h2.h"

namespace mh {

constexpr int HWG_BY = 4, HWG_BX = 16;
constexpr int HWG_RY = HWG_BY + 2, HWG_RX = HWG_BX + 2;
constexpr int HWG_NP = HWG_RY * HWG_RX;
constexpr int HWG_PB = 144;
constexpr int HWG_DB = (HWG_NP + 1) * HWG_PB;
constexpr int HWG_ZB = 32 * 1024;
constexpr int HWG_OPS = 24;
constexpr int HWG_CIN = 32, HWG_CN = 32;
constexpr int HWG_WAVES = 8;
constexpr unsigned HWG_DROP = 0x80000000u;

__device__ __forceinline__ void hw_split4(const f32x4 v, u32x2& hi, u32x2& lo) {
    _Float16 h_[4], l_[4];
#pragma unroll
    for (int i = 0; i < 4; ++i) {
        h_[i] = (_Float16)v[i];
        float r = v[i] - (float)h_[i];
        MH_OPAQUE(r);
        l_[i] = (_Float16)r;
    }
    const f16x2 h01 = {h_[0], h_[1]}, h23 = {h_[2], h_[3]}, l01 = {l_[0], l_[1]}, l23 = {l_[2], l_[3]};
    hi = u32x2{__builtin_bit_cast(unsigned, h01), __builtin_bit_cast(unsigned, h23)};
    lo = u32x2{__builtin_bit_cast(unsigned, l01), __builtin_bit_cast(unsigned, l23)};
}

__device__ __forceinline__ f32x4 hw_fma4(const f32x4 a, const float s, const f32x4 c) { return __builtin_elementwise_fma(a, f32x4{s, s, s, s}, c); }
__device__ __forceinline__ void hw_split4p(const f32x4 v, const float m1, u32x2& hi, u32x2& lo) {
#ifdef MH_SIMT_EMULATOR
    f16x2 h01, l01, h23, l23;
    h2_split_pair(v[0], v[1], m1, h01, l01);
    h2_split_pair(v[2], v[3], m1, h23, l23);
    hi = u32x2{__builtin_bit_cast(unsigned, h01), __builtin_bit_cast(unsigned, h23)};
    lo = u32x2{__builtin_bit_cast(unsigned, l01), __builtin_bit_cast(unsigned, l23)};
#else
    unsigned h0, h1, l0, l1;
    asm("v_cvt_pk_f16_f32 %0, %1, %2" : "=v"(h0) : "v"(v[0]), "v"(v[1]));
    asm("v_cvt_pk_f16_f32 %0, %1, %2" : "=v"(h1) : "v"(v[2]), "v"(v[3]));
    asm("v_fma_mixlo_f16 %0, %1, %2, %3 op_sel_hi:[1,0,0]" : "=v"(l0) : "v"(h0), "v"(m1), "v"(v[0]));
    asm("v_fma_mixlo_f16 %0, %1, %2, %3 op_sel_hi:[1,0,0]" : "=v"(l1) : "v"(h1), "v"(m1), "v"(v[2]));
    asm("v_fma_mixhi_f16 %0, %1, %2, %3 op_sel:[1,0,0] op_sel_hi:[1,0,0]" : "+v"(l0) : "v"(h0), "v"(m1), "v"(v[1]));
    asm("v_fma_mixhi_f16 %0, %1, %2, %3 op_sel:[1,0,0] op_sel_hi:[1,0,0]" : "+v"(l1) : "v"(h1), "v"(m1), "v"(v[3]));
    hi = u32x2{h0, h1};
    lo = u32x2{l0, l1};
#endif
}
__device__ __forceinline__ float hw_uniform(const float x) {
#ifdef MH_SIMT_EMULATOR
    return x;
#else
    return __builtin_bit_cast(float, __builtin_amdgcn_readfirstlane(__builtin_bit_cast(int, x)));
#endif
}
__device__ __forceinline__ void hw_xchg32_pair(const float mx, const float mn, const int hi, float& own, float& rcv) {
#ifdef MH_SIMT_EMULATOR
    own = hi ? mn : mx;
    rcv = __shfl_xor(hi ? mx : mn, 32);
#else
    (void)hi;
    const auto r = __builtin_amdgcn_permlane32_swap(__builtin_bit_cast(unsigned, mx), __builtin_bit_cast(unsigned, mn), false, false);
    const unsigned r0 = r[0], r1 = r[1];
    own = __builtin_bit_cast(float, r0);
    rcv = __builtin_bit_cast(float, r1);
#endif
}
#ifdef MH_SIMT_EMULATOR
#define MH_HW_KEEP_BRANCH ((void)0)
#else
#define MH_HW_KEEP_BRANCH asm volatile("" ::: "memory")
#endif

struct HwFinish {
    int co_l, fa, g4, frp, fq;
};
__device__ __forceinline__ HwFinish hw_finish_role(const int wave, const int lane) {
    HwFinish r;
    r.fq = lane & 3;
    r.frp = r.fq & 1;
    r.fa = lane >> 5;
    r.g4 = ((wave >> 1) & 1) ? (r.fq >> 1 ? 2 : 1) : (r.fq >> 1 ? 3 : 0);
    r.co_l = (wave >> 2) * 16 + (wave & 1) * 8 + ((lane >> 2) & 7);
    return r;
}

template <bool STATS, bool ACC = false, bool POOL = false>
__global__ void __launch_bounds__(512)
conv3d_k3_h2w_kernel(Tensor in, const uint4* __restrict__ wp, const float* __restrict__ wtail, const float* __restrict__ bias, Tensor out,
                     float* __restrict__ stats, int bxn, int byn, int zchunk, unsigned nblk, float* __restrict__ pmax, float* __restrict__ pmin,
                     long long pool_n_stride) {
    __shared__ __attribute__((aligned(16))) char smem[3 * HWG_DB + 2 * HWG_ZB];
    __shared__ unsigned bound_s[4];
    char* const ds = smem;
    char* const zs_ = smem + 3 * HWG_DB;
    const int tid = threadIdx.x, lane = tid & 63;
    const int wave = __builtin_amdgcn_readfirstlane(tid >> 6);
    const int wi = wave & 3, jp = wave >> 2;
    const int Cout = out.C, D = out.D, H = out.H, W = out.W;
    const long long HW = (long long)H * W, DHW = (long long)D * HW;

    const unsigned ncg = (unsigned)(Cout / HWG_CN);
    unsigned lid = xcd_remap(blockIdx.x, gridDim.x);
    const int cg = (int)(lid % ncg);
    lid /= ncg;
    const unsigned b = lid % nblk;
    const int n = (int)(lid / nblk);
    const int x0 = (int)(b % bxn) * HWG_BX, y0 = (int)((b / bxn) % byn) * HWG_BY;
    const int zs = (int)(b / (bxn * byn)) * zchunk, ze = min(zs + zchunk, D);
    const int p_first = max(zs - 1, 0), p_last = min(ze, D - 1);

    unsigned soff;
    int loff[2];
    {
        const int pr = min(lane, 53);
        const int ly = pr / 9;
        int lx = 2 * (pr - 9 * ly);
        const int gy = y0 + ly - 1;
        int gx = x0 + lx - 1;
        if (gx < 0) { gx += 1; lx += 1; }
        if (gx + 1 >= W) { gx -= 1; lx -= 1; }
        const bool ok = lane < 54 && gy >= 0 && gy < H;
        soff = ok ? 4u * (unsigned)(gy * W + gx) : 0u;
        loff[0] = (ok ? ly * HWG_RX + lx : HWG_NP) * HWG_PB;
        loff[1] = (ok ? ly * HWG_RX + lx + 1 : HWG_NP) * HWG_PB;
    }
    for (int i = tid; i < (3 * HWG_DB + 2 * HWG_ZB) / 16; i += 512) reinterpret_cast<uint4*>(smem)[i] = make_uint4(0u, 0u, 0u, 0u);
    f32x4 nra, nrb, nrs;
    {
        unsigned mb = 0u;
        if (lane < HWG_CIN) {
            const float4 a = *reinterpret_cast<const float4*>(in.nrm + (long long)n * in.nrm_n_stride + 4LL * lane);
            const unsigned bb = abs_bits(a.w);
            mb = bb == 0u ? 0x7fc00000u : bb;
        }
        mb = wave_umax(mb);
        if (tid == 0) bound_s[0] = mb;
    }
    __syncthreads();
    int e_in = 0;
    bool poisoned = false;
    {
        const unsigned mb = bound_s[0];
        poisoned = mb >= 0x7f800000u;
        e_in = poisoned ? 0 : min(max(13 - ((int)(mb >> 23) - 126), -100), 100);
        const float p_ = __uint_as_float((unsigned)(e_in + 127) << 23);
#pragma unroll
        for (int i = 0; i < 4; ++i) {
            const float4 a = *reinterpret_cast<const float4*>(in.nrm + (long long)n * in.nrm_n_stride + 4LL * (4 * wave + i));
            nra[i] = hw_uniform(a.x * p_); nrb[i] = a.y * p_; nrs[i] = a.z;
        }
    }
    f32x4 nrk;
#pragma unroll
    for (int i = 0; i < 4; ++i) nrk[i] = hw_uniform(nrs[i] <= 1.0f ? __builtin_inff() : -__builtin_inff());
    const auto xrs = __builtin_amdgcn_make_buffer_rsrc(const_cast<float*>(in.data + (long long)n * in.n_stride + (long long)(4 * wave) * DHW), 0, 0x7fffffff, 0x00020000);
    const unsigned hw4 = (unsigned)(HW * 4);
    unsigned voff = soff + (unsigned)p_first * hw4;
    const unsigned cso1 = (unsigned)(DHW * 4), cso2 = 2u * cso1, cso3 = 3u * cso1;
    f32x2 xin[4];
#define MH_HW_LDX                                                                                     \
    {                                                                                                 \
        xin[0] = __builtin_bit_cast(f32x2, __builtin_amdgcn_raw_buffer_load_b64(xrs, voff, 0u, 0));   \
        xin[1] = __builtin_bit_cast(f32x2, __builtin_amdgcn_raw_buffer_load_b64(xrs, voff, cso1, 0)); \
        xin[2] = __builtin_bit_cast(f32x2, __builtin_amdgcn_raw_buffer_load_b64(xrs, voff, cso2, 0)); \
        xin[3] = __builtin_bit_cast(f32x2, __builtin_amdgcn_raw_buffer_load_b64(xrs, voff, cso3, 0)); \
    }
#define MH_HW_CONV(DBO)                                                                               \
    {                                                                                                 \
        char* const db_ = ds + (DBO) + 16 * wave;                                                     \
        f32x4 y_[2];                                                                                  \
        _Pragma("unroll") for (int i = 0; i < 4; ++i) {                                               \
            const f32x2 t_ = __builtin_elementwise_fma(xin[i], f32x2{nra[i], nra[i]}, f32x2{nrb[i], nrb[i]}), u_ = t_ * nrs[i]; \
            _Pragma("unroll") for (int j = 0; j < 2; ++j) y_[j][i] = __builtin_amdgcn_fmed3f(t_[j], u_[j], nrk[i]);       \
        }                                                                                             \
        _Pragma("unroll") for (int j = 0; j < 2; ++j) *reinterpret_cast<f32x4*>(db_ + loff[j]) = y_[j]; \
    }
    int staged = p_first;
#define MH_HW_ADV { voff += staged < p_last ? hw4 : 0u; staged += 1; }

    u32x4 wu[HWG_OPS];
    {
        const u32x4* wg = reinterpret_cast<const u32x4*>(wp) + ((long long)(cg * 8 + wave) * HWG_OPS) * 64 + lane;
#pragma unroll
        for (int r = 0; r < HWG_OPS; ++r) wu[r] = wg[r * 64];
    }
#define MH_HW_U(SL, T, CB, PC) __builtin_bit_cast(f16x8, wu[(((SL) * 3 + (T)) * 2 + (CB)) * 2 + (PC)])

    const int rho = lane & 15, kg = lane >> 4;
    const int tty = (rho >= 4 && rho < 12) ? 1 : 0, ttx = rho < 4 ? rho : rho < 12 ? rho - 4 : rho - 8;
    const int ra = wi == 0 ? 0 : wi == 2 ? 2 : 1, rb = wi == 0 ? 2 : wi == 1 ? 2 : wi == 2 ? 1 : 3;
    const float sgn = wi == 1 ? 1.0f : -1.0f;
    const float fsg = jp ? -1.0f : 1.0f;
    const float m1 = h2_minus_one();
    const int ab0 = ((2 * tty + ra) * HWG_RX + 2 * ttx + jp) * HWG_PB + kg * 16;
    const int ab1 = ((2 * tty + rb) * HWG_RX + 2 * ttx + jp) * HWG_PB + kg * 16;

    f32x4 acc[3][2][2];
#pragma unroll
    for (int s = 0; s < 3; ++s)
#pragma unroll
        for (int j = 0; j < 2; ++j)
#pragma unroll
            for (int c = 0; c < 2; ++c) acc[s][j][c] = f32x4{0.0f, 0.0f, 0.0f, 0.0f};

    const HwFinish fr = hw_finish_role(wave, lane);
    const int fcb = wave >> 2, fty = (wave >> 1) & 1;
    const int fa = fr.fa, fq = fr.fq, frp = fr.frp, g4 = fr.g4;
    const int ftx = 2 * fq;
    const int c16 = fr.co_l & 15;
    const int co_l = fr.co_l, co = cg * HWG_CN + co_l;
    const float bco = bias ? bias[co] : 0.0f;
    const float fs2 = fa ? -1.0f : 1.0f;
    const int zwr = wave * 4096 + (lane ^ ((lane >> 5) * 12)) * 16;
    const int zrd = fa * 4096 + fcb * 2048 + (g4 * 16 + (c16 ^ (fq >> 1 ? 12 : 0))) * 16 + frp * 8;
    float inv_a, inv_b;
    {
        const int t_ = -((int)((__float_as_uint(wtail[1]) >> 23) & 0xffu) - 127) - e_in;
        const int t1_ = t_ / 2, t2_ = t_ - t1_;
        inv_a = hw_uniform(poisoned ? __uint_as_float(0x7fc00000u) : __uint_as_float((unsigned)(t1_ + 127) << 23));
        inv_b = hw_uniform(__uint_as_float((unsigned)(t2_ + 127) << 23));
    }
    const auto orsrc = __builtin_amdgcn_make_buffer_rsrc(out.data + (long long)n * out.n_stride + (long long)(cg * HWG_CN) * DHW, 0, (int)(HWG_CN * DHW * 4), 0x00020000);
    const unsigned ooff = 4u * (unsigned)((long long)co_l * DHW + (long long)(y0 + 2 * fty + fa) * W + x0 + 2 * ftx);
    float pivot = 0.0f;
    bool have_c = false;
    f32x4 s1 = {0.0f, 0.0f, 0.0f, 0.0f}, s2 = s1;
    const long long PHW = (long long)(H / 2) * (W / 2), PDHW = (long long)(D / 2) * PHW;
    float* const pbase_mx = POOL ? pmax + (long long)n * pool_n_stride + (long long)(cg * HWG_CN) * PDHW : out.data;
    float* const pbase_mn = POOL ? pmin + (long long)n * pool_n_stride + (long long)(cg * HWG_CN) * PDHW : out.data;
    const int pbytes = POOL ? (int)(HWG_CN * PDHW * 4) : 0;
    const unsigned phw4 = (unsigned)(PHW * 4);
    const unsigned poff = (4u * (unsigned)((long long)co_l * PDHW + (long long)((y0 >> 1) + fty) * (W / 2) + (x0 >> 1) + ftx)) | (fa ? HWG_DROP : 0u);
    const float pk_ = fa ? -__builtin_inff() : __builtin_inff();
    f32x2 hm = {0.0f, 0.0f};
    f32x4 pv = {0.0f, 0.0f, 0.0f, 0.0f};

    u32x4 ah[2], al[2];
#define MH_HW_XFORM(DBO)                                                                              \
    {                                                                                                 \
        const char* const db_ = ds + (DBO);                                                           \
        _Pragma("unroll") for (int h = 0; h < 2; ++h) {                                               \
            f32x4 r_[3];                                                                              \
            _Pragma("unroll") for (int bq = 0; bq < 3; ++bq) {                                        \
                const f32x4 u_ = *reinterpret_cast<const f32x4*>(db_ + ab0 + bq * HWG_PB + h * 64);   \
                const f32x4 v_ = *reinterpret_cast<const f32x4*>(db_ + ab1 + bq * HWG_PB + h * 64);   \
                r_[bq] = hw_fma4(v_, sgn, u_);                                                        \
            }                                                                                         \
            const f32x4 e_ = hw_fma4(r_[2], m1, r_[0]);                                               \
            f32x4 f_;                                                                                 \
            if (jp) { f_ = hw_fma4(r_[0], m1, r_[1]); MH_HW_KEEP_BRANCH; } else f_ = r_[1] + r_[2];   \
            u32x2 hh_, ll_;                                                                           \
            hw_split4p(e_, m1, hh_, ll_); ah[0][2 * h] = hh_[0]; ah[0][2 * h + 1] = hh_[1]; al[0][2 * h] = ll_[0]; al[0][2 * h + 1] = ll_[1]; \
            hw_split4p(f_, m1, hh_, ll_); ah[1][2 * h] = hh_[0]; ah[1][2 * h + 1] = hh_[1]; al[1][2 * h] = ll_[0]; al[1][2 * h + 1] = ll_[1]; \
        }                                                                                             \
    }
#define MH_HW_MM(S, SL, CB, A, B, FRESH)                                                              \
    acc[S][SL][CB] = __builtin_amdgcn_mfma_f32_16x16x32_f16(__builtin_bit_cast(f16x8, A), B, (FRESH) ? f32x4{0.0f, 0.0f, 0.0f, 0.0f} : acc[S][SL][CB], 0, 0, 0);
#define MH_HW_MMS(S0, S1, S2)                                                                         \
    _Pragma("unroll") for (int sl = 0; sl < 2; ++sl)                                                  \
        _Pragma("unroll") for (int cb = 0; cb < 2; ++cb) {                                            \
            MH_HW_MM(S0, sl, cb, ah[sl], MH_HW_U(sl, 0, cb, 0), true)  MH_HW_MM(S1, sl, cb, ah[sl], MH_HW_U(sl, 1, cb, 0), false) MH_HW_MM(S2, sl, cb, ah[sl], MH_HW_U(sl, 2, cb, 0), false) \
            MH_HW_MM(S0, sl, cb, al[sl], MH_HW_U(sl, 0, cb, 0), false) MH_HW_MM(S1, sl, cb, al[sl], MH_HW_U(sl, 1, cb, 0), false) MH_HW_MM(S2, sl, cb, al[sl], MH_HW_U(sl, 2, cb, 0), false) \
            MH_HW_MM(S0, sl, cb, ah[sl], MH_HW_U(sl, 0, cb, 1), false) MH_HW_MM(S1, sl, cb, ah[sl], MH_HW_U(sl, 1, cb, 1), false) MH_HW_MM(S2, sl, cb, ah[sl], MH_HW_U(sl, 2, cb, 1), false) \
        }
#define MH_HW_SKIP(S0)                                                                                \
    { _Pragma("unroll") for (int sl = 0; sl < 2; ++sl) _Pragma("unroll") for (int cb = 0; cb < 2; ++cb) acc[S0][sl][cb] = f32x4{0.0f, 0.0f, 0.0f, 0.0f}; }
#define MH_HW_ZOUT(S2, Q)                                                                             \
    {                                                                                                 \
        char* const zb_ = zs_ + ((Q) & 1) * HWG_ZB + zwr;                                             \
        _Pragma("unroll") for (int cb = 0; cb < 2; ++cb) {                                            \
            *reinterpret_cast<f32x4*>(zb_ + cb * 2048) = acc[S2][0][cb] + acc[S2][1][cb];             \
            *reinterpret_cast<f32x4*>(zb_ + cb * 2048 + 1024) = acc[S2][1][cb];                       \
        }                                                                                             \
    }
#define MH_HW_FINISH(Q, ON, ST)                                                                       \
    {                                                                                                 \
        const bool on_ = (ST) ? true : (ON);                                                          \
        const char* const zb_ = zs_ + ((Q) & 1) * HWG_ZB + zrd;                                       \
        f32x2 z0_[3], z1_[3];                                                                         \
        _Pragma("unroll") for (int i = 0; i < 3; ++i) {                                               \
            z0_[i] = *reinterpret_cast<const f32x2*>(zb_ + i * 4096) + *reinterpret_cast<const f32x2*>(zb_ + i * 4096 + 16384 + 1024);        \
            z1_[i] = *reinterpret_cast<const f32x2*>(zb_ + i * 4096 + 1024) - *reinterpret_cast<const f32x2*>(zb_ + i * 4096 + 16384);        \
        }                                                                                             \
        const f32x2 fs_ = {fs2, fs2};                                                                 \
        const f32x2 y0_ = __builtin_elementwise_fma(z0_[2], fs_, __builtin_elementwise_fma(z0_[1], fs_, z0_[0])) * inv_a; \
        const f32x2 y1_ = __builtin_elementwise_fma(z1_[2], fs_, __builtin_elementwise_fma(z1_[1], fs_, z1_[0])) * inv_a; \
        f32x4 o_ = {__builtin_fmaf(y0_[0], inv_b, bco), __builtin_fmaf(y1_[0], inv_b, bco), __builtin_fmaf(y0_[1], inv_b, bco), __builtin_fmaf(y1_[1], inv_b, bco)}; \
        if (ACC) o_ += pv;       \
        if (ST) __builtin_amdgcn_raw_buffer_store_b128(__builtin_bit_cast(u32x4, o_), orsrc, ooff, (unsigned)(Q) * hw4, 0); \
        else __builtin_amdgcn_raw_buffer_store_b128(__builtin_bit_cast(u32x4, o_), orsrc, on_ ? ooff + (unsigned)(Q) * hw4 : HWG_DROP, 0, 0); \
        if (STATS) {         \
            if (!(ST)) {                                                                              \
                pivot = (on_ && !have_c) ? o_[0] : pivot;                                             \
                have_c = have_c || on_;                                                               \
            }                                                                                         \
            const f32x4 d_ = o_ - pivot, dw_ = (ST) ? d_ : d_ * (on_ ? 1.0f : 0.0f);                  \
            s1 += dw_;                                                                                \
            s2 = __builtin_elementwise_fma(dw_, d_, s2);                                              \
        }                                                                                             \
        if (POOL && !(HWX_OFF & 32)) {          \
            const f32x2 mx_ = {fmaxf(o_[0], o_[1]), fmaxf(o_[2], o_[3])}, mn_ = {fminf(o_[0], o_[1]), fminf(o_[2], o_[3])}; \
            float own0_, rcv0_, own1_, rcv1_;                                                         \
            hw_xchg32_pair(mx_[0], mn_[0], fa, own0_, rcv0_);                                         \
            hw_xchg32_pair(mx_[1], mn_[1], fa, own1_, rcv1_);                                         \
            const f32x2 y_ = {__builtin_amdgcn_fmed3f(own0_, rcv0_, pk_), __builtin_amdgcn_fmed3f(own1_, rcv1_, pk_)};       \
            const f32x2 f_ = {__builtin_amdgcn_fmed3f(y_[0], hm[0], pk_), __builtin_amdgcn_fmed3f(y_[1], hm[1], pk_)}; \
            const int pn_ = (on_ && ((Q) & 1) && !(HWX_OFF & 64)) ? pbytes : 0;                       \
            const unsigned ps_ = (unsigned)((Q) >> 1) * phw4;                                         \
            __builtin_amdgcn_raw_buffer_store_b64(__builtin_bit_cast(u32x2, f_), __builtin_amdgcn_make_buffer_rsrc(pbase_mx, 0, pn_, 0x00020000), poff, ps_, 0); \
            __builtin_amdgcn_raw_buffer_store_b64(__builtin_bit_cast(u32x2, f_), __builtin_amdgcn_make_buffer_rsrc(pbase_mn, 0, pn_, 0x00020000), poff ^ HWG_DROP, ps_, 0); \
            hm = on_ ? y_ : hm;                                                                       \
        }                                                                                             \
    }
#ifdef HWX_PROF
#define MH_HW_T(K) { const long long t_ = __builtin_readcyclecounter(); tacc[K] += t_ - tlast; tlast = t_; }
    long long tacc[8] = {0, 0, 0, 0, 0, 0, 0, 0}, tlast = __builtin_readcyclecounter();
#else
#define MH_HW_T(K)
#endif
#ifndef HWX_OFF
#define HWX_OFF 0
#endif
#ifndef HWX_DEAL
#define HWX_DEAL 2
#endif
#define MH_HW_DEAL                                                                                    \
    if constexpr (ACC || POOL) {                                                                      \
        _Pragma("unroll") for (int g_ = 0; g_ < 36; ++g_) {                                           \
            __builtin_amdgcn_sched_group_barrier(0x008, 1, 0);                                        \
            __builtin_amdgcn_sched_group_barrier(0x100, 1, 0);                                        \
            __builtin_amdgcn_sched_group_barrier(0x006, HWX_DEAL, 0);                                 \
            __builtin_amdgcn_sched_group_barrier(0x230, 1, 0);                                        \
        }                                                                                             \
    }
#define MH_HW_ITER(P, R, ST)                                                                          \
    {                                                                                                 \
        constexpr int S0 = (3 - (R)) % 3, S1 = (S0 + 1) % 3, S2 = (S0 + 2) % 3;       \
        constexpr int db0 = (R) * HWG_DB, db2 = (((R) + 2) % 3) * HWG_DB;             \
        const int p_ = (P);                                                                           \
        const bool valid_ = (ST) ? true : (p_ >= p_first && p_ <= p_last);                            \
        const int qf_ = p_ - 2;                                                                       \
        if (ACC) {                                                                                    \
            if (ST) pv = __builtin_bit_cast(f32x4, __builtin_amdgcn_raw_buffer_load_b128(orsrc, ooff, (unsigned)qf_ * hw4, 0)); \
            else { const bool nx_ = qf_ >= zs && qf_ < ze; pv = __builtin_bit_cast(f32x4, __builtin_amdgcn_raw_buffer_load_b128(orsrc, nx_ ? ooff + (unsigned)qf_ * hw4 : HWG_DROP, 0, 0)); } \
        }                                                                                             \
        if (valid_) { if (!(HWX_OFF & 1)) MH_HW_XFORM(db0) }                                          \
        MH_HW_T(0)                                                                                    \
        __syncthreads();                                                                              \
        MH_HW_T(1)                                                                                    \
        if (valid_) {                                                                                 \
            __builtin_amdgcn_sched_barrier(0);                                                        \
            if (!(HWX_OFF & 2)) { MH_HW_CONV(db2) MH_HW_LDX MH_HW_ADV }                               \
            if (!(HWX_OFF & 4)) MH_HW_FINISH(qf_, qf_ >= zs && qf_ < ze, ST)                          \
            if (!(HWX_OFF & 8)) MH_HW_MMS(S0, S1, S2)                                                 \
            MH_HW_DEAL                                                                                \
            __builtin_amdgcn_sched_barrier(0);                                                        \
        } else {                                                                                      \
            MH_HW_SKIP(S0)                                                                            \
            if (!(HWX_OFF & 4)) MH_HW_FINISH(qf_, qf_ >= zs && qf_ < ze, false)                       \
        }                                                                                             \
        if (!(HWX_OFF & 16)) if ((ST) || (p_ - 1 >= zs && p_ - 1 < ze)) MH_HW_ZOUT(S2, p_ - 1)        \
        MH_HW_T(2)                                                                                    \
        __syncthreads();                                                                              \
        MH_HW_T(3)                                                                                    \
    }

    {
        const int k0 = p_first - (zs - 1);
        MH_HW_LDX MH_HW_ADV
        __syncthreads();
        MH_HW_CONV((k0 % 3) * HWG_DB)
        MH_HW_LDX MH_HW_ADV
        MH_HW_CONV(((k0 + 1) % 3) * HWG_DB)
        MH_HW_LDX MH_HW_ADV
        __syncthreads();
    }
    if (jp) __syncthreads();
    int p = zs - 1;
#define MH_HW_STEADY(P) ((P) >= zs + 5 && (P) + 2 <= p_last && (P) + 1 < ze)
#define MH_HW_BLOCK(ST) { MH_HW_ITER(p, 0, ST) MH_HW_ITER(p + 1, 1, ST) MH_HW_ITER(p + 2, 2, ST) }
    for (; p <= ze + 1 && !MH_HW_STEADY(p); p += 3) MH_HW_BLOCK(false)
    for (; MH_HW_STEADY(p); p += 3) MH_HW_BLOCK(true)
    for (; p <= ze + 1; p += 3) MH_HW_BLOCK(false)
#undef MH_HW_BLOCK
#undef MH_HW_STEADY
    if (!jp) __syncthreads();
#ifdef HWX_PROF
    if (blockIdx.x == 0 && lane == 0) { _Pragma("unroll") for (int k = 0; k < 8; ++k) reinterpret_cast<long long*>(pmax)[wave * 8 + k] = tacc[k]; }
#endif
#undef MH_HW_T
#undef MH_HW_DEAL
#undef MH_HW_ITER
#undef MH_HW_FINISH
#undef MH_HW_ZOUT
#undef MH_HW_SKIP
#undef MH_HW_MMS
#undef MH_HW_MM
#undef MH_HW_XFORM
#undef MH_HW_U
#undef MH_HW_ADV
#undef MH_HW_CONV
#undef MH_HW_LDX

    if (STATS) {
        Stat run;
        {
            const float a1 = (s1[0] + s1[1]) + (s1[2] + s1[3]), a2 = (s2[0] + s2[1]) + (s2[2] + s2[3]);
            run.n = 4.0f * (float)(ze - zs);
            const float dm = a1 / run.n;
            run.mean = pivot + dm;
            run.m2 = fmaxf(a2 - a1 * dm, 0.0f);
        }
        __syncthreads();
        float* red = reinterpret_cast<float*>(smem);
        {
            int t_ = tid;
            MH_OPAQUE(t_);
            const HwFinish e = hw_finish_role(t_ >> 6, t_ & 63);
            float* leaf = red + (((e.co_l * 2 + e.fa) * 4 + e.g4) * 2 + e.frp) * 3;
            leaf[0] = run.n; leaf[1] = run.mean; leaf[2] = run.m2;
        }
        __syncthreads();
        if (tid < HWG_CN) {
            const auto leaf_of = [&](int a, int g, int rp) {
                const float* l = red + (((tid * 2 + a) * 4 + g) * 2 + rp) * 3;
                Stat s;
                s.n = l[0]; s.mean = l[1]; s.m2 = l[2];
                return s;
            };
            Stat st;
            st.n = 0.0f; st.mean = 0.0f; st.m2 = 0.0f;
#pragma unroll
            for (int w = 0; w < 4; ++w) {
                const int rp = w >> 1, ge = 2 * (w & 1);
                const Stat r0 = stat_merge(leaf_of(0, ge, rp), leaf_of(0, ge + 1, rp)), r1 = stat_merge(leaf_of(1, ge, rp), leaf_of(1, ge + 1, rp));
                st = stat_merge(st, stat_merge(r0, r1));
            }
            float* rec = stats + (((long long)n * Cout + cg * HWG_CN + tid) * nblk + b) * 3;
            rec[0] = st.n; rec[1] = st.mean; rec[2] = st.m2;
        }
    }
}

__global__ void conv3d_k3_h2w_scale_fix_kernel(float* __restrict__ tail) {
    if (threadIdx.x == 0 && blockIdx.x == 0) { tail[0] *= 4.0f; tail[1] *= 0.25f; }
}
__global__ void __launch_bounds__(256)
conv3d_k3_h2w_pack_kernel(const float* __restrict__ w, int Cin, int Cout, _Float16* __restrict__ packed, const float* __restrict__ tail) {
    const int idx = blockIdx.x * 256 + threadIdx.x;
    if (idx >= Cin * Cout) return;
    const int ci = idx % Cin, co = idx / Cin;
    const float s = tail[1];
    const double G[4][3] = {{1.0, 0.0, 0.0}, {0.5, 0.5, 0.5}, {0.5, -0.5, 0.5}, {0.0, 0.0, 1.0}};
    const int cg = co / HWG_CN, cb = (co % HWG_CN) / 16, nn = co % 16;
    const int kg = ci < 16 ? ci / 4 : (ci - 16) / 4, e = ci < 16 ? ci % 4 : 4 + (ci - 16) % 4;
    const int ln = kg * 16 + nn;
    for (int t = 0; t < 3; ++t) {
        double g[3][3], tm[4][3];
        for (int ky = 0; ky < 3; ++ky)
            for (int kx = 0; kx < 3; ++kx) g[ky][kx] = (double)w[((long long)co * Cin + ci) * 27 + t * 9 + ky * 3 + kx];
        for (int i = 0; i < 4; ++i)
            for (int kx = 0; kx < 3; ++kx) tm[i][kx] = G[i][0] * g[0][kx] + G[i][1] * g[1][kx] + G[i][2] * g[2][kx];
        for (int i = 0; i < 4; ++i)
            for (int j = 0; j < 4; ++j) {
                const double u = tm[i][0] * G[j][0] + tm[i][1] * G[j][1] + tm[i][2] * G[j][2];
                _Float16 pc[2];
                h2_split((float)(u * (double)s), pc[0], pc[1]);
                const int jpq = j >> 1, slot = (j == 0 || j == 3) ? 0 : 1;
                for (int p = 0; p < 2; ++p) {
                    const long long r = (((long long)(cg * 8 + jpq * 4 + i) * HWG_OPS) + ((slot * 3 + t) * 2 + cb) * 2 + p) * 64 + ln;
                    packed[r * 8 + e] = pc[p];
                }
            }
    }
}

}
```

monai_amd/networks/_conv_engine.py:

```python

from __future__ import annotations

from typing import Optional

import torch

from .. import _prof, ops

__all__ = ["ConvEngine", "split_configs", "accumulates", "identity_records"]


def split_configs() -> tuple:
    return ops.conv3d_k3_h2_config(), ops.conv3d_k3_h2c_config(), ops.conv3d_k3_h2w_config()


def accumulates(cfg: int) -> bool:
    return cfg in split_configs()


def identity_records(t: torch.Tensor) -> torch.Tensor:
    return ops.nrm_identity(torch.empty((t.shape[0], t.shape[1], 4), dtype=torch.float32, device=t.device))


def _kernel3(w: torch.Tensor) -> torch.Tensor:
    if w.dim() == 4:
        w = w.unsqueeze(2)
    if tuple(w.shape[2:]) == (3, 3, 3):
        return w
    w3 = torch.zeros(w.shape[:2] + (3, 3, 3), dtype=w.dtype, device=w.device)
    w3[(slice(None), slice(None)) + tuple(slice(0, 3) if k == 3 else slice(1, 2) for k in w.shape[2:])] = w
    return w3


class ConvEngine:
    def __init__(self):
        self._derived: dict = {}
        self._scratch: dict = {}

    def derived(self, slot, sources, build, *extra):
        key = tuple((t.data_ptr(), t._version, str(t.device)) for t in sources) + extra
        hit = self._derived.get(slot)
        if hit is None or hit[0] != key:
            hit = self._derived[slot] = (key, build())
        return hit[1]

    def conv3_pack(self, conv, cfg: int, cin: Optional[tuple] = None, cout: Optional[tuple] = None) -> torch.Tensor:
        def build():
            w = _kernel3(conv.weight)
            if cout is not None:
                w = w[cout[0]:cout[1]]
            if cin is not None:
                w = w[:, cin[0]:cin[1]].contiguous()
            return ops.conv3d_k3_pack(cfg, w)

        return self.derived((id(conv), "k3", cfg, cin, cout), [conv.weight], build)

    def conv3s2_pack(self, conv) -> torch.Tensor:
        return self.derived((id(conv), "s2"), [conv.weight], lambda: ops.conv3d_k3s2_pack(conv.weight))

    def conv1x1_h2_pack(self, conv) -> torch.Tensor:
        return self.derived((id(conv), "1x1"), [conv.weight], lambda: ops.conv1x1_h2_pack(conv.weight.view(conv.weight.shape[0], -1)))

    def upconv_pack(self, conv, dec, at: int):
        def build():
            w4, table = ops.upconv_k4s2_weights(dec.weight, dec.bias, conv.weight[:, at:])
            return ops.upconv_k4s2_pack(w4), table

        return self.derived((id(conv), "upconv"), [conv.weight, dec.weight] + ([dec.bias] if dec.bias is not None else []), build)

    def linear_pack(self, weight: torch.Tensor) -> torch.Tensor:
        return self.derived((id(weight), "lin"), [weight], lambda: ops.linear_pack(weight.reshape(weight.shape[0], -1)))

    def scalar(self, param: torch.Tensor) -> float:
        return self.derived((id(param), "scalar"), [param], lambda: float(param.detach().float().cpu()))

    def bn_fold(self, bn, slope: float) -> torch.Tensor:
        if bn.running_mean is None or bn.running_var is None:
            raise NotImplementedError("monai_amd: BatchNorm without running statistics is not on the (inference) HIP path")

        def build():
            invstd = 1.0 / torch.sqrt(bn.running_var.float() + bn.eps)
            alpha = invstd * bn.weight.float() if bn.affine else invstd
            beta = (bn.bias.float() if bn.affine else 0.0) - bn.running_mean.float() * alpha
            return torch.stack([alpha, beta, torch.full_like(alpha, slope), torch.zeros_like(alpha)], dim=1).contiguous()

        return self.derived((id(bn), "bn"), [bn.running_mean, bn.running_var] + ([bn.weight, bn.bias] if bn.affine else []), build, slope)

    def act_records(self, slope: float, n: int, c: int, device) -> torch.Tensor:
        return self.derived(("act", slope, n, c, str(device)), [],
                            lambda: torch.tensor([1.0, 0.0, slope, 0.0], dtype=torch.float32, device=device).repeat(n, c, 1).contiguous())

    def _buf(self, what: str, floats: int, device) -> torch.Tensor:
        buf = self._scratch.get((what, device))
        if buf is None or buf.numel() < floats:
            buf = self._scratch[(what, device)] = torch.empty(floats, dtype=torch.float32, device=device)
        return buf

    def stats_buf(self, floats: int, device) -> torch.Tensor:
        return self._buf("stats", floats, device)

    def epilogue_stats(self, cfg: int, out):
        n, cout, d, h, w = out.shape
        tiles = ops.conv3d_k3_stat_tiles(cfg, d, h, w)
        return (self.stats_buf(n * cout * tiles * 3, out.device), tiles) if tiles else (None, 0)

    def launch3(self, cfg: int, x, x_nrm, packed, bias, out, want_stats: bool = True, accumulate: bool = False, pool=None, stats=None):
        n, cout, d, h, w = out.shape
        own, tiles = self.epilogue_stats(cfg, out) if want_stats else (None, 0)
        stats = (own if stats is None else stats) if tiles else None
        with _prof.span(f"conv3d_k3/cfg{cfg}", 2.0 * 27 * x.shape[1] * cout * d * h * w * n):
            if pool is not None:
                ops.conv3d_k3_pool(cfg, x, x_nrm, packed, bias, out, stats, *pool)
            else:
                ops.conv3d_k3(cfg, x, x_nrm, packed, bias, out, stats, accumulate=accumulate)
        return stats, tiles

    def conv3(self, conv, x, x_nrm, stride=1, out=None, *, bounded: bool, want_stats: bool = True, tiny_direct: bool = False, accumulate: bool = False, pool=None):
        n, cin, d, h, w = x.shape
        cout = conv.weight.shape[0]
        st = (int(stride),) * 3 if isinstance(stride, int) else tuple(stride)
        sp = tuple((v - 1) // s + 1 for v, s in zip((d, h, w), st))
        if out is None:
            out = torch.empty((n, cout) + sp, dtype=torch.float32, device=x.device)
        if st == (1, 1, 1) and not (tiny_direct and cin <= 8 and cout <= 8):
            cfg = ops.conv3d_k3_select(cin, cout, d, h, w, bounded=bounded)
            return (out,) + self.launch3(cfg, x, x_nrm, self.conv3_pack(conv, cfg), conv.bias, out, want_stats, accumulate, pool)
        if tuple(conv.weight.shape[2:]) == (3, 3, 3) and ops.conv3d_k3s2_selected(cin, cout, d, h, w, st, bounded=bounded):
            tiles = ops.conv3d_k3s2_stat_tiles(d, h, w)
            stats = self.stats_buf(n * cout * tiles * 3, x.device)
            with _prof.span("conv3d_k3s2", 2.0 * 27 * cin * cout * sp[0] * sp[1] * sp[2] * n):
                fused = ops.conv3d_k3s2_fused(cin, cout, d * h * w)
                ws = None if fused else self._buf("s2 workspace", ops.conv3d_k3s2_workspace_floats(n, cin, d, h, w), x.device)
                ops.conv3d_k3s2(x, x_nrm, self.conv3s2_pack(conv), conv.bias, out, stats, ws, fused)
            return out, stats, (tiles if want_stats else 0)
        if isinstance(stride, int):
            ops.conv3d_k3_strided(x, x_nrm, self.conv3_pack(conv, 0), conv.bias, out, stride)
        else:
            ops.conv3d_k3_strided3(x, x_nrm, self.conv3_pack(conv, 0), conv.bias, out, st)
        return out, None, 0

    def conv3_split(self, conv, cfg: int, x, x_nrm, at: int, out, bias_on: Optional[str]):
        cin, b = x.shape[1], conv.bias
        self.launch3(cfg, x[:, :at], x_nrm[:, :at], self.conv3_pack(conv, cfg, cin=(0, at)), b if bias_on == "first" else None, out, want_stats=False)
        return self.launch3(cfg, x[:, at:], x_nrm[:, at:], self.conv3_pack(conv, cfg, cin=(at, cin)), b if bias_on == "second" else None, out, accumulate=True)

    def norm_record(self, raw, stats, tiles: int, norm, slope: float, groups: Optional[int] = None, out=None):
        n, c = raw.shape[:2]
        if not tiles:
            tiles = ops.instnorm_stat_tiles(*raw.shape[2:])
            stats = self.stats_buf(n * c * tiles * 3, raw.device)
            ops.instnorm_stats(raw, stats)
        if out is None:
            out = torch.empty((n, c, 4), dtype=torch.float32, device=raw.device)
        gamma, beta, eps = (None, None, 1e-5) if norm is None else (norm.weight, norm.bias, norm.eps)
        if groups is None:
            return ops.instnorm_finalize(stats, tiles, n, c, gamma, beta, eps, slope, out)
        return ops.groupnorm_finalize(stats, tiles, n, c, groups, gamma, beta, eps, slope, out)
```

monai_amd/networks/nets/basic_unet.py:

```python

from __future__ import annotations

import threading
from collections.abc import Sequence

import torch
import torch.nn as nn

from ... import _lib, _prof, config, ops
from .._conv_engine import ConvEngine, split_configs

__all__ = ["BasicUNet", "BasicUnet", "Basicunet", "basicunet"]


_BUILD = threading.local()


def _nd(three, two):
    return two if getattr(_BUILD, "dims", 3) == 2 else three


def _w5(w: torch.Tensor) -> torch.Tensor:
    return w if w.dim() == 5 else w.unsqueeze(2)

# ... 94 lines not shown
    if kind == "group":
        if "num_groups" not in args:
            raise TypeError("GroupNorm.__init__() missing 1 required positional argument: 'num_groups'")
        return kind, {k: v for k, v in args.items() if k in ("num_groups", "eps", "affine")}
    raise NotImplementedError(f"monai_amd.BasicUNet: norm {norm!r} is not on the HIP path yet (instance / batch / group are)")


class BasicUNet(nn.Module):
    def __init__(
        self,
        spatial_dims: int = 3,
        in_channels: int = 1,
        out_channels: int = 2,
        features: Sequence[int] = (32, 32, 64, 128, 256, 32),
        act: str | tuple = ("LeakyReLU", {"negative_slope": 0.1, "inplace": True}),
        norm: str | tuple = ("instance", {"affine": True}),
        bias: bool = True,
        dropout: float | tuple = 0.0,
        upsample: str = "deconv",
    ):
        super().__init__()
        if spatial_dims not in (2, 3):
            raise NotImplementedError("monai_amd.BasicUNet: spatial_dims 2 and 3 are on the HIP path")
        if upsample not in ("deconv", "nontrainable", "pixelshuffle"):
            raise NotImplementedError("monai_amd.BasicUNet: upsample='deconv', 'nontrainable' and 'pixelshuffle' are on the HIP path")
        fea = tuple(features)
        if len(fea) != 6:
            raise ValueError(f"Sequence must have length 6, got length {len(fea)}.")
        print(f"BasicUNet features: {fea}.")
        slope = _parse_act(act)
        kw = dict(bias=bias, norm=_parse_norm(norm), slope=slope)
        self.features, self.in_channels, self.out_channels = fea, in_channels, out_channels
        self.spatial_dims, self.upsample = spatial_dims, upsample
        _BUILD.dims = spatial_dims
        try:
            self._build(in_channels, out_channels, fea, kw)
        finally:
            _BUILD.dims = 3
        self._plans: dict = {}
        self._engine = ConvEngine()
        self.fused_stats = True

    def _build(self, in_channels, out_channels, fea, kw):
        self.conv_0 = _TwoConv(in_channels, fea[0], **kw)
        self.down_1 = _Down(fea[0], fea[1], **kw)
        self.down_2 = _Down(fea[1], fea[2], **kw)
        self.down_3 = _Down(fea[2], fea[3], **kw)
        self.down_4 = _Down(fea[3], fea[4], **kw)
        up = self.upsample
        self.upcat_4 = _UpCat(fea[4], fea[3], fea[3], upsample=up, **kw)
        self.upcat_3 = _UpCat(fea[3], fea[2], fea[2], upsample=up, **kw)
        self.upcat_2 = _UpCat(fea[2], fea[1], fea[1], upsample=up, **kw)
        self.upcat_1 = _UpCat(fea[1], fea[0], fea[5], halves=False, upsample=up, **kw)
        self.final_conv = _nd(nn.Conv3d, nn.Conv2d)(fea[5], out_channels, kernel_size=1)

    def forward(self, x: torch.Tensor) -> torch.Tensor:
        if torch.is_grad_enabled() and x.requires_grad:
            raise NotImplementedError("monai_amd.BasicUNet: gradients w.r.t. the input are not on the (inference-only) HIP path")
        _lib.require_device(x)
        if self.spatial_dims == 2:
            if x.dim() != 4 or x.shape[1] != self.in_channels:
                raise RuntimeError(f"monai_amd.BasicUNet: expected input (B,{self.in_channels},H,W), got {tuple(x.shape)}")
            out = torch.empty((x.shape[0], self.out_channels) + tuple(x.shape[2:]), dtype=torch.float32, device=x.device)
            return self.forward_into(x, out)
        if x.dim() != 5 or x.shape[1] != self.in_channels:
            raise RuntimeError(f"monai_amd.BasicUNet: expected input (B,{self.in_channels},D,H,W), got {tuple(x.shape)}")
        out = torch.empty((x.shape[0], self.out_channels) + tuple(x.shape[2:]), dtype=torch.float32, device=x.device)
        return self.forward_into(x, out)

    @torch.no_grad()
    def forward_into(self, x: torch.Tensor, out: torch.Tensor) -> torch.Tensor:
        _lib.require_device(x, out[0].flat if isinstance(out, tuple) else out)
        if self.spatial_dims == 2 and x.dim() == 4 and not isinstance(out, tuple) and out.dim() == 4:
            self.forward_into(x.unsqueeze(2), out.unsqueeze(2))
            return out
        if self.training:
            raise NotImplementedError("monai_amd.BasicUNet: training mode (autograd) is not on the HIP path -- the engine is inference-only; with MONAI installed the call falls through to the reference module, which shares these parameters")
        x = x.contiguous()
        n, _, d, h, w = x.shape
        if self.spatial_dims == 2 and d != 1:
            raise RuntimeError(f"monai_amd.BasicUNet: a 2-D network takes one plane, got {tuple(x.shape)}")
        if min((h, w) if self.spatial_dims == 2 else (d, h, w)) < 16:
            raise RuntimeError(f"monai_amd.BasicUNet: window {d}x{h}x{w} is too small for four 2x poolings")
        key = (n, d, h, w, str(x.device))
        plan = self._plans.get(key)
        if plan is None:
            if len(self._plans) >= 4:
                self._plans.clear()
            plan = self._plans[key] = _Plan(self, n, (d, h, w), x.device)
        plan.run(self, x, out)
        return out


    @torch.no_grad()
    def forward_into_windows(self, x: torch.Tensor, mosaic, w0: int) -> None:
        self.forward_into(x, (mosaic, int(w0)))


BasicUnet = Basicunet = basicunet = BasicUNet


class _Plan:

    def __init__(self, net: "BasicUNet", n: int, dims, device):
        f = net.features
        self.n, self.dims = n, tuple(dims)
        self.planar = net.spatial_dims == 2
        self.sp = [tuple(v if (self.planar and a == 0) else v >> l for a, v in enumerate(dims)) for l in range(5)]
        up = [f[1], f[2] // 2, f[3] // 2, f[4] // 2]
        dec_out = [f[5], f[1], f[2], f[3]]
        e = lambda c, l: torch.empty((n, c) + self.sp[l], dtype=torch.float32, device=device)
        nz = lambda c: torch.zeros((n, c, 4), dtype=torch.float32, device=device)
        self.cat = [e(f[l] + up[l], l) for l in range(4)]
        self.cat_nrm = [nz(f[l] + up[l]) for l in range(4)]
        for l in range(4):
            self.cat_nrm[l][:, f[l]:, 0] = 1.0
            self.cat_nrm[l][:, f[l]:, 2] = 1.0
        self.tmp = [e(max(f[l], dec_out[l]) if l < 4 else f[4], l) for l in range(5)]
        self.tmp_nrm = [nz(max(f[l], dec_out[l]) if l < 4 else f[4]) for l in range(5)]
        self.pool = [None] + [e(f[l - 1], l) for l in range(1, 5)]
        self.pool_min = [None] * 5
        self.pool_nrm = [None] + [nz(f[l - 1]) for l in range(1, 5)]
        self.odd = [any(v & 1 for a, v in enumerate(self.sp[l]) if not (self.planar and a == 0)) for l in range(4)]
        self.up_scratch = [torch.empty((n, up[l]) + tuple(v if (self.planar and a == 0) else 2 * v for a, v in enumerate(self.sp[l + 1])),
                                       dtype=torch.float32, device=device)
                           if self.odd[l] else None for l in range(4)]
        self.up_scratch_nrm = [nz(up[l]) if self.odd[l] else None for l in range(4)]
        self.x4, self.x4_nrm = e(f[4], 4), nz(f[4])
        self.u = [e(dec_out[l], l) for l in range(4)]
        self.u_nrm = [nz(dec_out[l]) for l in range(4)]
        self.up, self.dec_out = up, dec_out
        self.batchnorm = isinstance(net.conv_0.conv_0.adn.N, (nn.BatchNorm3d, nn.BatchNorm2d))
        self.interp = net.upsample == "nontrainable"
        self.shuffle = net.upsample == "pixelshuffle"
        self.sub = [e((4 if self.planar else 8) * up[l], l + 1) if self.shuffle else None for l in range(4)]
        self.low = [e(up[l], l + 1) if self.interp else None for l in range(4)]

    @staticmethod
    def _slope(net, adn: _ADN) -> float:
        return net._engine.scalar(adn.A.weight) if hasattr(adn, "A") else adn.negative_slope

    def _record(self, net, block: _Convolution, raw, stats, tiles, out_nrm) -> None:
        norm, slope = block.adn.N, self._slope(net, block.adn)
        if self.batchnorm:
            out_nrm.copy_(net._engine.bn_fold(norm, slope)[None].expand(out_nrm.shape[0], -1, -1))
        else:
            net._engine.norm_record(raw, stats, tiles, norm, slope, groups=norm.num_groups if isinstance(norm, nn.GroupNorm) else None, out=out_nrm)

    def _conv(self, net, block: _Convolution, x, x_nrm, out, out_nrm, bounded: bool = True, pool_level: int = 0) -> bool:
        _, cout, d, h, w = out.shape
        cin = x.shape[1]
        bounded = x_nrm is not None and bounded and not self.batchnorm
        pool = None
        if (pool_level and self._slope(net, block.adn) >= 0.0
                and self._poolable(net, ops.conv3d_k3_select(cin, cout, d, h, w, bounded=bounded), cin, cout, d, h, w, pool_level, x_nrm)):
            if self.pool_min[pool_level] is None:
                self.pool_min[pool_level] = torch.empty_like(self.pool[pool_level])
            pool = (self.pool[pool_level], self.pool_min[pool_level])
        _, stats, tiles = net._engine.conv3(block.conv, x, x_nrm, out=out, bounded=bounded, want_stats=net.fused_stats and not self.batchnorm, pool=pool)
        self._record(net, block, out, stats, tiles, out_nrm)
        if pool is not None:
            ops.pool_select(*pool, out_nrm)
        return pool is not None

    def _halves_cfg(self, net, l: int, cout: int, bounded: bool) -> int:
        f = net.features
        if not config.conv_halves() or self.batchnorm or not net.fused_stats or not bounded or 2 * f[l] != int(self.cat[l].shape[1]):
            return -1
        _, _, d, h, w = self.cat[l].shape
        cfg = ops.conv3d_k3_select(f[l], cout, d, h, w, bounded=True)
        if cfg != split_configs()[2] or ops.conv3d_k3_select(2 * f[l], cout, d, h, w, bounded=True) == cfg:
            return -1
        return cfg

    def _conv_halves(self, net, block: _Convolution, l: int, cfg: int, out, out_nrm) -> None:
        fl = net.features[l]
        for half in ((0, fl), (fl, 2 * fl)):
            net._engine.conv3_pack(block.conv, cfg, cin=half)
        stats, tiles = net._engine.conv3_split(block.conv, cfg, self.cat[l], self.cat_nrm[l], fl, out, bias_on="second")
        self._record(net, block, out, stats, tiles, out_nrm)

    def _poolable(self, net, cfg: int, cin: int, cout: int, d: int, h: int, w: int, level: int, x_nrm) -> bool:
        if self.planar or self.batchnorm or not net.fused_stats or x_nrm is None or not config.pool_fused():
            return False
        if tuple(self.sp[level]) != (d // 2, h // 2, w // 2) or tuple(self.pool[level].shape[1:]) != (cout, d // 2, h // 2, w // 2):
            return False
        return ops.conv3d_k3_pool_accepts(cfg, cin, cout, d, h, w)

    def _interpolate(self, up: _UpSample, src, src_nrm, low, dst) -> None:
        if hasattr(up, "preconv"):
            pc = up.preconv
            ops.conv1x1(src, src_nrm, pc.weight.view(pc.weight.shape[0], -1), pc.bias, low)
        else:
            ops.add_act(src, src_nrm, None, None, 1.0, low)
        n, c, d, h, w = low.shape
        osz = (d if self.planar else 2 * d, 2 * h, 2 * w)
        a = [1.0 if (self.planar or d == 1) else (d - 1) / (osz[0] - 1), (h - 1) / (osz[1] - 1), (w - 1) / (osz[2] - 1)]
        m = [a[0], 0, 0, 0, 0, a[1], 0, 0, 0, 0, a[2], 0]
        hi = ops.affine_resample(low.reshape(n * c, d, h, w), m, osz, "bilinear", "border", False, False)
        dst.copy_(hi.reshape((n, c) + osz))

    def _subpixel(self, net, conv: nn.Conv3d, src, src_nrm, sub, dst, dst_nrm) -> None:
        net._engine.conv3(conv, src, src_nrm, out=sub, bounded=src_nrm is not None and not self.batchnorm, want_stats=False)
        ops.pixelshuffle(sub, dst, 1 if self.planar else 2, True, dst_nrm)

    def _fusable(self, net, l: int, src: torch.Tensor, cout: int) -> bool:
        if self.interp or self.shuffle or self.planar or self.odd[l] or self.batchnorm or not net.fused_stats or not config.upcat_fused():
            return False
        if config.conv_algo() not in (config.CONV_ALGOS["auto"], config.CONV_ALGOS["h2"]):
            return False
        return ops.upconv_k4s2_accepts(int(src.shape[1]), int(cout), *self.sp[l + 1])

    def _upcat_fused(self, net, l: int, upc: "_UpCat", src, src_nrm, out, out_nrm) -> None:
        f, eng = net.features, net._engine
        block = upc.convs.conv_0
        conv, dec = block.conv, upc.upsample.deconv
        n, cout, d, h, w = out.shape
        skip, skip_nrm = self.cat[l][:, : f[l]], self.cat_nrm[l][:, : f[l]]
        cfg = ops.conv3d_k3_select(f[l], cout, d, h, w, bounded=True)
        packed_skip = eng.conv3_pack(conv, cfg, cin=(0, f[l]))
        packed_up, table = eng.upconv_pack(conv, dec, f[l])
        up_flops = 2.0 * 8 * int(src.shape[1]) * cout * d * h * w * n
        h2, _, hw = split_configs()
        if cfg in (h2, hw) and config.upcat_order() == "term_first":
            with _prof.span("upconv_k4s2", up_flops):
                ops.upconv_k4s2(src, src_nrm, packed_up, table, out, accumulate=False)
            stats, tiles = eng.launch3(cfg, skip, skip_nrm, packed_skip, conv.bias, out, accumulate=True)
        else:
            eng.launch3(cfg, skip, skip_nrm, packed_skip, conv.bias, out, want_stats=False)
            tiles = ops.upconv_k4s2_stat_tiles(*self.sp[l + 1])
            stats = eng.stats_buf(n * cout * tiles * 3, out.device)
            with _prof.span("upconv_k4s2", up_flops):
                ops.upconv_k4s2(src, src_nrm, packed_up, table, out, accumulate=True, stats=stats)
        self._record(net, block, out, stats, tiles, out_nrm)

    def run(self, net: "BasicUNet", x: torch.Tensor, logits: torch.Tensor) -> None:
        f = net.features
        downs = [None, net.down_1, net.down_2, net.down_3, net.down_4]
        ups = [net.upcat_1, net.upcat_2, net.upcat_3, net.upcat_4]

        t, tn = self.tmp[0][:, : f[0]], self.tmp_nrm[0][:, : f[0]]
        self._conv(net, net.conv_0.conv_0, x, None, t, tn)
        pooled = self._conv(net, net.conv_0.conv_1, t, tn, self.cat[0][:, : f[0]], self.cat_nrm[0][:, : f[0]], pool_level=1)
        for l in range(1, 5):
            skip, skip_nrm = self.cat[l - 1][:, : f[l - 1]], self.cat_nrm[l - 1][:, : f[l - 1]]
            if pooled:
                p_in, p_nrm = self.pool[l], skip_nrm
            else:
                ops.maxpool2(skip, skip_nrm, self.pool[l], self.pool_nrm[l])
                p_in, p_nrm = self.pool[l], self.pool_nrm[l]
            t, tn = self.tmp[l][:, : f[l]], self.tmp_nrm[l][:, : f[l]]
            self._conv(net, downs[l].convs.conv_0, p_in, p_nrm, t, tn)
            if l < 4:
                o, on = self.cat[l][:, : f[l]], self.cat_nrm[l][:, : f[l]]
            else:
                o, on = self.x4, self.x4_nrm
            pooled = self._conv(net, downs[l].convs.conv_1, t, tn, o, on, pool_level=l + 1 if l < 4 else 0)

        src, src_nrm = self.x4, self.x4_nrm
        for l in range(3, -1, -1):
            upc = ups[l]
            co = self.dec_out[l]
            t, tn = self.tmp[l][:, :co], self.tmp_nrm[l][:, :co]
            if self._fusable(net, l, src, co):
                self._upcat_fused(net, l, upc, src, src_nrm, t, tn)
            else:
                dst = self.up_scratch[l] if self.odd[l] else self.cat[l][:, f[l]:]
                dst_nrm = ops.nrm_identity(self.up_scratch_nrm[l] if self.odd[l] else self.cat_nrm[l][:, f[l]:])
                if self.interp:
                    self._interpolate(upc.upsample, src, src_nrm, self.low[l], dst)
                elif self.shuffle:
                    self._subpixel(net, upc.upsample.pixelshuffle.conv_block, src, src_nrm, self.sub[l], dst, dst_nrm)
                elif self.planar:
                    ops.deconv_ks(src, src_nrm, _w5(upc.upsample.deconv.weight).contiguous(), upc.upsample.deconv.bias, dst, (1, 2, 2), dst_nrm)
                else:
                    ops.deconv_k2s2(src, src_nrm, upc.upsample.deconv.weight, upc.upsample.deconv.bias, dst, dst_nrm, bounded=src_nrm is not None and not self.batchnorm)
                if self.odd[l]:
                    ops.pad_replicate(self.up_scratch[l], self.cat[l][:, f[l]:], self.up_scratch_nrm[l], self.cat_nrm[l][:, f[l]:])
                hcfg = self._halves_cfg(net, l, co, bounded=not self.interp)
                if hcfg >= 0:
                    self._conv_halves(net, upc.convs.conv_0, l, hcfg, t, tn)
                else:
                    self._conv(net, upc.convs.conv_0, self.cat[l], self.cat_nrm[l], t, tn, bounded=not self.interp)
            self._conv(net, upc.convs.conv_1, t, tn, self.u[l], self.u_nrm[l])
            src, src_nrm = self.u[l], self.u_nrm[l]

        fc = net.final_conv
        if isinstance(logits, tuple):
            ops.conv1x1_windows(src, src_nrm, fc.weight.view(fc.weight.shape[0], -1), fc.bias, logits[0], logits[1])
        else:
            ops.conv1x1(src, src_nrm, fc.weight.view(fc.weight.shape[0], -1), fc.bias, logits)
```

monai_amd/ops.py:

```python

from __future__ import annotations

import ctypes as C
from typing import Optional, Sequence

import torch

from . import _lib

Grid = Sequence[Sequence[int]]


def _s(t):
    return _lib.stream_ptr(t)


def window_extract(vol: torch.Tensor, grid: Grid, w0: int, nwin: int, roi: Sequence[int], out: torch.Tensor) -> torch.Tensor:
    _lib.require_device(vol, out)
    if vol.dim() != 4 or not vol.is_contiguous() or not out.is_contiguous():
        raise RuntimeError("monai_amd.window_extract: vol must be a contiguous [C,D,H,W] tensor")
    c, d, h, w = vol.shape
    sz, sy, sx = grid
    _lib.lib().call(
        "mh_window_extract_f32", _lib.ptr(vol), c, d, h, w, _lib.int_array(sz), len(sz), _lib.int_array(sy), len(sy),
# ... 81 lines not shown

def onehot(labels: torch.Tensor, num_classes: int) -> torch.Tensor:
    _lib.require_device(labels)
    if not labels.is_contiguous() or labels.shape[0] != 1:
        raise RuntimeError("monai_amd.onehot: contiguous [1, spatial] tensor required")
    out = torch.empty((int(num_classes),) + tuple(labels.shape[1:]), dtype=torch.float32, device=labels.device)
    if labels.numel():
        _lib.lib().call("mh_onehot_f32", _lib.ptr(labels), _lib.ptr(out), int(num_classes), int(labels.numel()), _s(labels))
    return out


def patch_accumulate(values: torch.Tensor, counts: torch.Tensor, patch: torch.Tensor, location: Sequence[int]) -> None:
    _lib.require_device(values, patch)
    _lib.require_device(counts, dtypes=(torch.uint8,))
    if not (values.is_contiguous() and counts.is_contiguous() and patch.is_contiguous()):
        raise RuntimeError("monai_amd.patch_accumulate: contiguous tensors required")
    sd = values.dim() - 2
    if sd < 1 or sd > 3 or patch.dim() != values.dim() or tuple(patch.shape[:2]) != tuple(values.shape[:2]) or counts.shape != values.shape:
        raise RuntimeError(f"monai_amd.patch_accumulate: shapes {tuple(values.shape)} / {tuple(counts.shape)} / {tuple(patch.shape)} do not match")
    pad = 3 - sd
    v3 = [1] * pad + [int(v) for v in values.shape[2:]]
    p3 = [1] * pad + [int(v) for v in patch.shape[2:]]
    l3 = [0] * pad + [int(v) for v in location]
    _lib.lib().call("mh_patch_accumulate_f32", _lib.ptr(values), _lib.ptr(counts), _lib.ptr(patch), int(values.shape[0] * values.shape[1]),
                    *v3, *p3, *l3, _s(values))


def patch_accumulate_batch(values: torch.Tensor, counts: torch.Tensor, patches: torch.Tensor, locations: Sequence[Sequence[int]]) -> None:
    _lib.require_device(values, patches)
    _lib.require_device(counts, dtypes=(torch.uint8,))
    if not (values.is_contiguous() and counts.is_contiguous() and patches.is_contiguous()):
        raise RuntimeError("monai_amd.patch_accumulate_batch: contiguous tensors required")
    sd, npatch = values.dim() - 2, len(locations)
    if (sd < 1 or sd > 3 or patches.dim() != values.dim() or npatch < 1 or patches.shape[0] != npatch * values.shape[0] or patches.shape[1] != values.shape[1]
            or counts.shape != values.shape):
        raise RuntimeError(f"monai_amd.patch_accumulate_batch: shapes {tuple(values.shape)} / {tuple(counts.shape)} / {tuple(patches.shape)} x {npatch} do not match")
    pad = 3 - sd
    v3 = [1] * pad + [int(v) for v in values.shape[2:]]
    p3 = [1] * pad + [int(v) for v in patches.shape[2:]]
    flat = [int(v) for loc in locations for v in ([0] * pad + list(loc))]
    _lib.lib().call("mh_patch_accumulate_batch_f32", _lib.ptr(values), _lib.ptr(counts), _lib.ptr(patches), npatch, _lib.int_array(flat),
                    int(values.shape[0] * values.shape[1]), *v3, *p3, _s(values))


def avg_finalize(values: torch.Tensor, counts: torch.Tensor) -> torch.Tensor:
    _lib.require_device(values)
    _lib.require_device(counts, dtypes=(torch.uint8,))
    if not (values.is_contiguous() and counts.is_contiguous()) or counts.shape != values.shape:
        raise RuntimeError("monai_amd.avg_finalize: contiguous tensors of one shape required")
    _lib.lib().call("mh_avg_finalize_f32", _lib.ptr(values), _lib.ptr(counts), int(values.numel()), _s(values))
    return values


class LogitsMosaic:

    CLASSES = 5

    @staticmethod
    def residue_log2(n: int, step: int, roi: int):
        if n <= 2:
            return 0
        for lg in (0, 1, 2):
            if (step << lg) >= roi:
                return lg
        return None

    @classmethod
    def supported(cls, grid, roi, k: int) -> bool:
        if k < 1 or k > 8 or roi[2] % 4 or any(v % 4 for v in grid[2]):
            return False
        for starts, r in zip(grid, roi):
            n = len(starts)
            if n > 1 and any(starts[i] != i * starts[1] for i in range(n - 1)):
                return False
            if n > 2 and cls.residue_log2(n, starts[1], r) is None:
                return False
        return True

    def __init__(self, grid, roi, k: int, device, dtype=torch.float32, allocate: bool = True):
        self.grid, self.roi, self.k = [list(g) for g in grid], tuple(int(v) for v in roi), int(k)
        self.n = [len(g) for g in self.grid]
        self.log2m = [self.residue_log2(n, g[1] if n > 1 else 1, r) for n, g, r in zip(self.n, self.grid, self.roi)]
        self.cnt = []
        for n, lg in zip(self.n, self.log2m):
            c = (C.c_int32 * self.CLASSES)()
            _lib.lib().call("mh_sw_mosaic_class_counts", int(n), int(lg), c)
            self.cnt.append([int(v) for v in c])
        self.base = [0] * self.CLASSES ** 3
        total = 0
        for cz in range(self.CLASSES):
            for cy in range(self.CLASSES):
                for cx in range(self.CLASSES):
                    size = self.k * self.cnt[0][cz] * self.roi[0] * self.cnt[1][cy] * self.roi[1] * self.cnt[2][cx] * self.roi[2]
                    self.base[(cz * self.CLASSES + cy) * self.CLASSES + cx] = total
                    if size:
                        total = (total + size + 3) // 4 * 4
                        if size * 4 >= (1 << 20):
                            total = (total + 63) // 64 * 64 + 17 * 64
        self.total, self._device, self._dtype = max(total, 4), device, dtype
        self.flat = None
        if allocate:
            self.allocate()

    def allocate(self):
        self.flat = torch.empty(self.total, dtype=self._dtype, device=self._device)
        return self

    def place(self, w: int):
        nz, ny, nx = self.n
        idx = (w // (ny * nx), (w // nx) % ny, w % nx)
        cls, j = [], []
        for a in range(3):
            last = idx[a] == self.n[a] - 1
            m = 1 << self.log2m[a]
            cls.append(m if last else idx[a] & (m - 1))
            j.append(0 if last else idx[a] >> self.log2m[a])
        dc, hc, wc = (self.cnt[a][cls[a]] * self.roi[a] for a in range(3))
        off = self.base[(cls[0] * self.CLASSES + cls[1]) * self.CLASSES + cls[2]] + ((j[0] * self.roi[0]) * hc + j[1] * self.roi[1]) * wc + j[2] * self.roi[2]
        return off, dc * hc * wc, hc * wc, wc

    def window_view(self, w: int) -> torch.Tensor:
        off, sc, sd, sh = self.place(w)
        return self.flat.as_strided((self.k,) + self.roi, (sc, sd, sh, 1), off)

    def places(self, w0: int, n: int):
        flat = [int(v) for w in range(w0, w0 + n) for v in self.place(w)]
        return (C.c_int64 * len(flat))(*flat)


def sw_blend_mosaic(mosaic: LogitsMosaic, imp: torch.Tensor, out: torch.Tensor) -> torch.Tensor:
    _lib.require_device(mosaic.flat, imp, out)
    if not (imp.is_contiguous() and out.is_contiguous()):
        raise RuntimeError("monai_amd.sw_blend_mosaic: contiguous tensors required")
    factored = imp.dim() == 1
    if factored and imp.numel() != sum(mosaic.roi) + 1:
        raise RuntimeError("monai_amd.sw_blend_mosaic: factored importance map must hold rd + rh + rw + 1 floats")
    k, d, h, w = out.shape
    sz, sy, sx = mosaic.grid
    _lib.lib().call("mh_sw_blend_mosaic_f32", _lib.ptr(mosaic.flat), (C.c_int64 * len(mosaic.base))(*mosaic.base), *[int(v) for v in mosaic.log2m], _lib.ptr(imp),
                    int(factored), _lib.ptr(out), k, d, h, w, *mosaic.roi, _lib.int_array(sz), len(sz), _lib.int_array(sy), len(sy), _lib.int_array(sx), len(sx), _s(out))
    return out


def conv1x1_windows(x, x_nrm, weight, bias, mosaic: LogitsMosaic, w0: int):
    _lib.require_device(x, x_nrm, weight, bias, mosaic.flat)
    xi = _lib.tensor5(x, x_nrm)
    _lib.lib().call("mh_conv1x1_windows_f32", C.byref(xi), _lib.ptr(weight), _lib.ptr(bias), _lib.ptr(mosaic.flat), int(weight.shape[0]),
                    mosaic.places(int(w0), int(x.shape[0])), _s(x))


def conv3d_k3_select(cin: int, cout: int, d: int, h: int, w: int, bounded: bool = False, algo: Optional[int] = None) -> int:
    from . import config

    cfg = _lib.lib().query("mh_conv3d_k3_select", config.conv_algo() if algo is None else int(algo), int(bool(bounded)), cin, cout, d, h, w)
    if not config.small_volume_h2() and cfg == _lib.lib().query("mh_conv3d_k3_h2v_config"):
        cfg = _lib.lib().query("mh_conv3d_k3_select", config.CONV_ALGOS["fp32"], int(bool(bounded)), cin, cout, d, h, w)
    return cfg


def conv3d_k3_num_configs() -> int:
    return _lib.lib().query("mh_conv3d_k3_num_configs")


def conv3d_k3_h2_config() -> int:
    return _lib.lib().query("mh_conv3d_k3_h2_config")


def conv3d_k3_h2c_config() -> int:
    return _lib.lib().query("mh_conv3d_k3_h2c_config")


def conv3d_k3_c1_config() -> int:
    return _lib.lib().query("mh_conv3d_k3_c1_config")


def conv3d_k3_h2v_config() -> int:
    return _lib.lib().query("mh_conv3d_k3_h2v_config")


def conv3d_k3_h2w_config() -> int:
    return _lib.lib().query("mh_conv3d_k3_h2w_config")


def conv3d_k3_h2w_fits(d: int, h: int, w: int) -> bool:
    return bool(_lib.lib().query("mh_conv3d_k3_h2w_fits", int(d), int(h), int(w)))


def conv3d_k3_accepts(cfg: int, cin: int, cout: int) -> bool:
    return bool(_lib.lib().query("mh_conv3d_k3_accepts", int(cfg), int(cin), int(cout)))


def conv3d_k3_pack(cfg: int, weight: torch.Tensor) -> torch.Tensor:
    _lib.require_device(weight)
    cout, cin = weight.shape[:2]
    wc = weight.detach().contiguous()
    packed = torch.empty(_lib.lib().query("mh_conv3d_k3_packed_floats", cfg, cin, cout), dtype=torch.float32, device=weight.device)
    _lib.lib().call("mh_conv3d_k3_pack_f32", cfg, _lib.ptr(wc), cin, cout, _lib.ptr(packed), _s(weight))
    return packed


def conv3d_k3_stat_tiles(cfg: int, d: int, h: int, w: int) -> int:
    return _lib.lib().query("mh_conv3d_k3_stat_tiles", cfg, d, h, w)


def conv3d_k3(cfg, x, x_nrm, packed_w, bias, out, stats: Optional[torch.Tensor] = None, accumulate: bool = False):
    _lib.require_device(x, x_nrm, packed_w, bias, out, stats)
    xi, xo = _lib.tensor5(x, x_nrm), _lib.tensor5(out)
    _lib.lib().call("mh_conv3d_k3_accumulate_f32" if accumulate else "mh_conv3d_k3_f32", int(cfg), C.byref(xi), _lib.ptr(packed_w), _lib.ptr(bias), C.byref(xo),
                    _lib.ptr(stats), _s(x))
    return out


def conv3d_k3_pool_accepts(cfg: int, cin: int, cout: int, d: int, h: int, w: int) -> bool:
    return bool(_lib.lib().query("mh_conv3d_k3_pool_accepts", int(cfg), int(cin), int(cout), int(d), int(h), int(w)))


def conv3d_k3_pool(cfg, x, x_nrm, packed_w, bias, out, stats, pool_max: torch.Tensor, pool_min: torch.Tensor):
    _lib.require_device(x, x_nrm, packed_w, bias, out, stats, pool_max, pool_min)
    if pool_max.shape != pool_min.shape or pool_max.stride() != pool_min.stride() or not pool_max[0].is_contiguous():
        raise RuntimeError("monai_amd.conv3d_k3_pool: pool_max / pool_min must be two equally laid out [N, C, D/2, H/2, W/2] tensors, dense per sample")
    xi, xo = _lib.tensor5(x, x_nrm), _lib.tensor5(out)
    _lib.lib().call("mh_conv3d_k3_pool_f32", int(cfg), C.byref(xi), _lib.ptr(packed_w), _lib.ptr(bias), C.byref(xo), _lib.ptr(stats), _lib.ptr(pool_max), _lib.ptr(pool_min),
                    int(pool_max.stride(0)), _s(x))
    return out


def pool_select(pool_max: torch.Tensor, pool_min: torch.Tensor, nrm: torch.Tensor) -> torch.Tensor:
    _lib.require_device(pool_max, pool_min, nrm)
    n, c = int(pool_max.shape[0]), int(pool_max.shape[1])
    vol = int(pool_max.shape[2] * pool_max.shape[3] * pool_max.shape[4])
    if nrm.dim() != 3 or nrm.shape[2] != 4 or nrm.stride(2) != 1 or nrm.stride(1) != 4:
        raise RuntimeError("monai_amd.pool_select: nrm must be an [N, C, 4] record view")
    _lib.lib().call("mh_pool_select_f32", _lib.ptr(pool_max), _lib.ptr(pool_min), _lib.ptr(nrm), int(nrm.stride(0)), n, c, int(pool_max.stride(0)), vol, _s(pool_max))
    return pool_max


def instnorm_stat_tiles(d: int, h: int, w: int) -> int:
    return _lib.lib().query("mh_instnorm_stat_tiles", d, h, w)


def instnorm_stats(x: torch.Tensor, stats: torch.Tensor):
    _lib.require_device(x, stats)
    xi = _lib.tensor5(x)
    _lib.lib().call("mh_instnorm_stats_f32", C.byref(xi), _lib.ptr(stats), _s(x))
    return stats


def instnorm_finalize(stats, tiles: int, n: int, c: int, gamma, beta, eps: float, slope: float, nrm: torch.Tensor):
    _lib.require_device(stats, gamma, beta, nrm)
    if nrm.dim() != 3 or nrm.shape[2] != 4 or nrm.stride(2) != 1 or nrm.stride(1) != 4:
        raise RuntimeError("monai_amd.instnorm_finalize: nrm must be a [N,C,4] slice")
    ns = nrm.stride(0) if n > 1 else max(nrm.stride(0), 4 * c)
    _lib.lib().call(
        "mh_instnorm_finalize_f32", _lib.ptr(stats), int(tiles), int(n), int(c), _lib.ptr(gamma), _lib.ptr(beta), float(eps),
        float(slope), _lib.ptr(nrm), int(ns), _s(stats),
    )
    return nrm


def nrm_identity(nrm: torch.Tensor) -> torch.Tensor:
    _lib.require_device(nrm)
    if nrm.dim() != 3 or nrm.shape[2] != 4 or nrm.stride(2) != 1 or nrm.stride(1) != 4:
        raise RuntimeError("monai_amd.nrm_identity: nrm must be a [N,C,4] slice")
    n, c = nrm.shape[:2]
    _lib.lib().call("mh_nrm_identity_f32", _lib.ptr(nrm), int(n), int(c), int(nrm.stride(0) if n > 1 else max(nrm.stride(0), 4 * c)), _s(nrm))
    return nrm


def maxpool2(x, x_nrm, out, out_nrm=None):
    _lib.require_device(x, x_nrm, out, out_nrm)
    xi, xo = _lib.tensor5(x, x_nrm), _lib.tensor5(out, out_nrm)
    _lib.lib().call("mh_maxpool2_f32", C.byref(xi), C.byref(xo), _s(x))
    return out


_DECONV_H2_PACKED: dict = {}


def deconv_k2s2_h2_packed(weight: torch.Tensor) -> torch.Tensor:
    import weakref

    hit = _DECONV_H2_PACKED.get(id(weight))
    if hit is None or hit[0]() is not weight or hit[1] != weight._version or hit[2] != str(weight.device) or hit[3] != weight.data_ptr():
        if len(_DECONV_H2_PACKED) > 256:
            for k in [k for k, v in _DECONV_H2_PACKED.items() if v[0]() is None]:
                del _DECONV_H2_PACKED[k]
        cin, cout = int(weight.shape[0]), int(weight.shape[1])
        packed = torch.zeros(_lib.lib().query("mh_deconv_k2s2_h2_packed_floats", cin, cout), dtype=torch.float32, device=weight.device)
        _lib.lib().call("mh_deconv_k2s2_h2_pack_f32", _lib.ptr(weight.detach().contiguous()), cin, cout, _lib.ptr(packed), _s(weight))
        hit = (weakref.ref(weight), weight._version, str(weight.device), weight.data_ptr(), packed)
        _DECONV_H2_PACKED[id(weight)] = hit
    return hit[4]


def deconv_k2s2(x, x_nrm, weight, bias, out, out_nrm=None, bounded: bool = False):
    _lib.require_device(x, x_nrm, weight, bias, out, out_nrm)
    xi, xo = _lib.tensor5(x, x_nrm), _lib.tensor5(out, out_nrm)
    if bounded and x_nrm is not None and tuple(weight.shape[2:]) == (2, 2, 2):
        from . import config

        cin, cout = int(weight.shape[0]), int(weight.shape[1])
        if config.deconv_h2() and _lib.lib().query("mh_deconv_k2s2_h2_accepts", cin, cout, int(x.shape[2]), int(x.shape[3]), int(x.shape[4])):
            _lib.lib().call("mh_deconv_k2s2_h2_f32", C.byref(xi), _lib.ptr(deconv_k2s2_h2_packed(weight)), _lib.ptr(bias), C.byref(xo), _s(x))
            return out
    _lib.lib().call("mh_deconv_k2s2_f32", C.byref(xi), _lib.ptr(weight), _lib.ptr(bias), C.byref(xo), _s(x))
    return out


def upconv_k4s2_accepts(cin: int, cout: int, dl: int, hl: int, wl: int) -> bool:
    return bool(_lib.lib().query("mh_upconv_k4s2_accepts", int(cin), int(cout), int(dl), int(hl), int(wl)))


def upconv_k4s2_weights(deconv_w: torch.Tensor, deconv_b: Optional[torch.Tensor], conv_w_up: torch.Tensor):
    wd, wc = deconv_w.detach().float(), conv_w_up.detach().float()
    cin, cout = wd.shape[0], wc.shape[0]
    pairs = {-1: ((0, 2),), 0: ((0, 1), (1, 2)), 1: ((0, 0), (1, 1)), 2: ((1, 0),)}
    w4 = torch.zeros((cin, cout, 4, 4, 4), dtype=torch.float32, device=wd.device)
    for uz, pz_ in pairs.items():
        for uy, py_ in pairs.items():
            for ux, px_ in pairs.items():
                acc = None
                for dz, kz in pz_:
                    for dy, ky in py_:
                        for dx, kx in px_:
                            t = wd[:, :, dz, dy, dx] @ wc[:, :, kz, ky, kx].t()
                            acc = t if acc is None else acc + t
                w4[:, :, uz + 1, uy + 1, ux + 1] = acc
    inside = ((1, 2), (0, 1, 2), (0, 1))
    table = torch.zeros((27, cout), dtype=torch.float32, device=wd.device)
    if deconv_b is not None:
        bd = deconv_b.detach().float()
        for cz in range(3):
            for cy in range(3):
                for cx in range(3):
                    wsum = wc[:, :, list(inside[cz])][:, :, :, list(inside[cy])][:, :, :, :, list(inside[cx])].sum(dim=(2, 3, 4))
                    table[(cz * 3 + cy) * 3 + cx] = wsum @ bd
    return w4.contiguous(), table.contiguous()


def upconv_k4s2_pack(w4: torch.Tensor) -> torch.Tensor:
    _lib.require_device(w4)
    cin, cout = int(w4.shape[0]), int(w4.shape[1])
    packed = torch.zeros(_lib.lib().query("mh_upconv_k4s2_packed_floats", cin, cout), dtype=torch.float32, device=w4.device)
    _lib.lib().call("mh_upconv_k4s2_pack_f32", _lib.ptr(w4.contiguous()), cin, cout, _lib.ptr(packed), _s(w4))
    return packed


def upconv_k4s2_stat_tiles(dl: int, hl: int, wl: int) -> int:
    return _lib.lib().query("mh_upconv_k4s2_stat_tiles", int(dl), int(hl), int(wl))


def upconv_k4s2(low, low_nrm, packed, bias_table, out, accumulate: bool = False, stats=None):
    _lib.require_device(low, low_nrm, packed, bias_table, out, stats)
    xi, xo = _lib.tensor5(low, low_nrm), _lib.tensor5(out)
    _lib.lib().call("mh_upconv_k4s2_f32", C.byref(xi), _lib.ptr(packed), _lib.ptr(bias_table), C.byref(xo), int(bool(accumulate)), _lib.ptr(stats), _s(out))
    return out


def conv1x1_stat_tiles(d: int, h: int, w: int) -> int:
    return _lib.lib().query("mh_conv1x1_stat_tiles", d, h, w)


def conv1x1(x, x_nrm, weight, bias, out, stats=None):
    _lib.require_device(x, x_nrm, weight, bias, out, stats)
    xi, xo = _lib.tensor5(x, x_nrm), _lib.tensor5(out)
    if stats is None:
        _lib.lib().call("mh_conv1x1_f32", C.byref(xi), _lib.ptr(weight), _lib.ptr(bias), C.byref(xo), _s(x))
    else:
        _lib.lib().call("mh_conv1x1_stats_f32", C.byref(xi), _lib.ptr(weight), _lib.ptr(bias), C.byref(xo), _lib.ptr(stats), _s(x))
    return out


def conv1x1_h2_accepts(cin: int, cout: int, d: int, h: int, w: int) -> bool:
    return bool(_lib.lib().query("mh_conv1x1_h2_accepts", int(cin), int(cout), int(d), int(h), int(w)))

# ... 898 lines not shown
```

Measured before the change: 222.1 million voxels/s.

## Route wide-input convs through sliced Winograd kernel with accumulating pool epilogue

Generalises the two-half Winograd split into `conv3_slices`, which cuts any conv with a multiple of 32 input channels (at least 64) into 32-channel slices. Each slice runs on the Winograd split kernel and accumulates into the output, where such convs previously used the plain H2 kernel in one launch. A pooling-plus-accumulate kernel variant lets the final slice also produce the fused max/min pool outputs, so pooled encoder layers can take this path. It also adds an optional 8x8 spatial tile geometry for the Winograd kernel, off by default, for shapes that do not tile into the default region. The cost is more launches and extra read-modify-write traffic on the output per slice.

Result: no change. 222.2 million voxels/s, median of 4 (+0.1%).

```diff
diff --git a/include/monai_amd.h b/include/monai_amd.h
--- a/include/monai_amd.h
+++ b/include/monai_amd.h
@@ -58,6 +58,7 @@
 #define MH_ALGO_WINO2D 2
 #define MH_ALGO_H2 3
 #define MH_ALGO_FP32 4
+#define MH_ALGO_H2W8 0x100
 int mh_conv3d_k3_select(int algo, int input_bounded, int Cin, int Cout, int D, int H, int W);
 int mh_conv3d_k3_num_configs(void);
 int mh_conv3d_k3_h2_config(void);
@@ -66,6 +67,7 @@
 int mh_conv3d_k3_h2v_config(void);
 int mh_conv3d_k3_h2w_config(void);
 int mh_conv3d_k3_h2w_fits(int D, int H, int W);
+int mh_conv3d_k3_h2w_geometry(int D, int H, int W);
 int mh_conv3d_k3_accepts(int cfg, int Cin, int Cout);
 int64_t mh_conv3d_k3_packed_floats(int cfg, int Cin, int Cout);
 int mh_conv3d_k3_pack_f32(int cfg, const float* w, int Cin, int Cout, float* packed, void* stream);
@@ -75,6 +77,8 @@
 int mh_conv3d_k3_pool_accepts(int cfg, int Cin, int Cout, int D, int H, int W);
 int mh_conv3d_k3_pool_f32(int cfg, const mh_tensor5* in, const float* packed_w, const float* bias, const mh_tensor5* out, float* stats, float* pool_max, float* pool_min,
                           int64_t pool_n_stride, void* stream);
+int mh_conv3d_k3_pool_accumulate_f32(int cfg, const mh_tensor5* in, const float* packed_w, const float* bias, const mh_tensor5* out, float* stats, float* pool_max,
+                                     float* pool_min, int64_t pool_n_stride, void* stream);
 int mh_pool_select_f32(float* pool_max, const float* pool_min, const float* nrm, int64_t nrm_n_stride, int N, int C, int64_t n_stride, int64_t vol, void* stream);
 int mh_conv3d_k3_accumulate_f32(int cfg, const mh_tensor5* in, const float* packed_w, const float* bias, const mh_tensor5* out, float* stats, void* stream);
 
diff --git a/monai_amd/_lib.py b/monai_amd/_lib.py
--- a/monai_amd/_lib.py
+++ b/monai_amd/_lib.py
@@ -58,6 +58,7 @@
     "mh_conv3d_k3_h2v_config": (_I, []),
     "mh_conv3d_k3_h2w_config": (_I, []),
     "mh_conv3d_k3_h2w_fits": (_I, [_I, _I, _I]),
+    "mh_conv3d_k3_h2w_geometry": (_I, [_I, _I, _I]),
     "mh_conv3d_k3_num_configs": (_I, []),
     "mh_conv3d_k3_accepts": (_I, [_I, _I, _I]),
     "mh_conv3d_k3_packed_floats": (_L, [_I, _I, _I]),
@@ -67,6 +68,7 @@
     "mh_conv3d_k3_accumulate_f32": (_I, [_I, _T, _P, _P, _T, _P, _P]),
     "mh_conv3d_k3_pool_accepts": (_I, [_I, _I, _I, _I, _I, _I]),
     "mh_conv3d_k3_pool_f32": (_I, [_I, _T, _P, _P, _T, _P, _P, _P, _L, _P]),
+    "mh_conv3d_k3_pool_accumulate_f32": (_I, [_I, _T, _P, _P, _T, _P, _P, _P, _L, _P]),
     "mh_pool_select_f32": (_I, [_P, _P, _P, _L, _I, _I, _L, _L, _P]),
     "mh_instnorm_stat_tiles": (_I, [_I, _I, _I]),
     "mh_instnorm_stats_f32": (_I, [_T, _P, _P]),
diff --git a/monai_amd/config.py b/monai_amd/config.py
--- a/monai_amd/config.py
+++ b/monai_amd/config.py
@@ -57,6 +57,14 @@
 
 def conv_halves() -> bool:
     v = CONV_HALVES if CONV_HALVES is not None else os.environ.get("MONAI_AMD_CONV_HALVES", "1")
+    return str(v).lower() not in ("0", "false", "off", "no")
+
+
+H2W_8X8 = None
+
+
+def h2w_8x8() -> bool:
+    v = H2W_8X8 if H2W_8X8 is not None else os.environ.get("MONAI_AMD_H2W_8X8", "0")
     return str(v).lower() not in ("0", "false", "off", "no")
 
 
diff --git a/monai_amd/csrc/capi.hip b/monai_amd/csrc/capi.hip
--- a/monai_amd/csrc/capi.hip
+++ b/monai_amd/csrc/capi.hip
@@ -414,6 +414,9 @@
 #ifndef MH_H2W_DEFAULT
 #define MH_H2W_DEFAULT 1
 #endif
+#ifndef MH_H2W8_DEFAULT
+#define MH_H2W8_DEFAULT 0
+#endif
 #define MH_CFG_LAST MH_CFG_H2W
 static inline bool hv_fits(int D, int H, int W) {
     const long long vol = (long long)D * H * W, padded = (long long)(D + 2) * (H + 2) * (W + 2);
@@ -448,8 +451,13 @@
     return cdiv(D, nchunk);
 }
 static inline int h2_blocks(int D, int H, int W) { return h2_regions(H, W) * cdiv(D, h2_zchunk(D, H, W)); }
-static inline bool hw_fits(int D, int H, int W) { return H >= HWG_BY && W >= HWG_BX && H % HWG_BY == 0 && W % HWG_BX == 0 && D >= 2 && h2_fits(D, H, W); }
-static inline int hw_regions(int H, int W) { return (H / HWG_BY) * (W / HWG_BX); }
+static inline int hw_geo(int H, int W) {
+    if (H >= HWG_BY && W >= HWG_BX && H % HWG_BY == 0 && W % HWG_BX == 0) return 0;
+    if (H >= 8 && W >= 8 && H % 8 == 0 && W % 8 == 0) return 1;
+    return -1;
+}
+static inline bool hw_fits(int D, int H, int W) { return hw_geo(H, W) >= 0 && D >= 2 && h2_fits(D, H, W); }
+static inline int hw_regions(int H, int W) { return hw_geo(H, W) == 1 ? (H / 8) * (W / 8) : (H / HWG_BY) * (W / HWG_BX); }
 static inline int hw_zchunk(int D, int H, int W) {
     int nchunk = cdiv(32, hw_regions(H, W));
     if (const char* e = knob_str("MONAI_AMD_HW_CHUNKS")) {
@@ -470,7 +478,8 @@
 int mh_conv3d_k3_c1_config(void) { return MH_CFG_C1; }
 int mh_conv3d_k3_h2v_config(void) { return MH_CFG_H2V; }
 int mh_conv3d_k3_h2w_config(void) { return MH_CFG_H2W; }
-int mh_conv3d_k3_h2w_fits(int D, int H, int W) { return hw_fits(D, H, W) ? 1 : 0; }
+int mh_conv3d_k3_h2w_fits(int D, int H, int W) { return hw_fits(D, H, W) && hw_geo(H, W) == 0 ? 1 : 0; }
+int mh_conv3d_k3_h2w_geometry(int D, int H, int W) { return !hw_fits(D, H, W) ? 0 : hw_geo(H, W) == 1 ? 8 : HWG_BY; }
 
 int mh_conv3d_k3_pool_accepts(int cfg, int Cin, int Cout, int D, int H, int W) {
     if (cfg == MH_CFG_H2W) return Cin == HWG_CIN && Cout >= HWG_CN && Cout % HWG_CN == 0 && D % 2 == 0 && hw_fits(D, H, W);
@@ -492,6 +501,8 @@
 
 int mh_conv3d_k3_select(int algo, int input_bounded, int Cin, int Cout, int D, int H, int W) {
     if (Cin < 1 || Cout < 1 || D < 1 || H < 1 || W < 1) return fail(MH_ERR_ARG, "conv3d_k3_select: bad argument");
+    const bool w8 = (algo & MH_ALGO_H2W8) != 0 || knob_int("MONAI_AMD_H2W8", MH_H2W8_DEFAULT) != 0;
+    if (algo >= 0) algo &= ~MH_ALGO_H2W8;
     if (algo < MH_ALGO_AUTO || algo > MH_ALGO_FP32) return fail(MH_ERR_ARG, "conv3d_k3_select: unknown algorithm family %d", algo);
     int best = 0;
     double best_score = 0.0;
@@ -514,7 +525,8 @@
         best = MH_CFG_H2C;
     if ((algo == MH_ALGO_AUTO || algo == MH_ALGO_H2) && input_bounded && best != MH_CFG_H2 && best != MH_CFG_H2C && mh_conv3d_k3_accepts(MH_CFG_H2V, Cin, Cout) && hv_fits(D, H, W))
         best = MH_CFG_H2V;
-    if (algo == MH_ALGO_AUTO && best == MH_CFG_H2 && mh_conv3d_k3_accepts(MH_CFG_H2W, Cin, Cout) && hw_fits(D, H, W) && D >= 24 && knob_int("MONAI_AMD_H2W", MH_H2W_DEFAULT) != 0)
+    if (algo == MH_ALGO_AUTO && best == MH_CFG_H2 && mh_conv3d_k3_accepts(MH_CFG_H2W, Cin, Cout) && hw_fits(D, H, W) && D >= 24 && knob_int("MONAI_AMD_H2W", MH_H2W_DEFAULT) != 0
+        && (hw_geo(H, W) == 0 || (Cout >= 2 * HWG_CN && w8)))
         best = MH_CFG_H2W;
     if (algo != MH_ALGO_DIRECT && algo != MH_ALGO_WINO2D && mh_conv3d_k3_accepts(MH_CFG_C1, Cin, Cout) && W % 4 == 0 && knob_int("MONAI_AMD_C1", 1) != 0)
         best = MH_CFG_C1;
@@ -617,15 +629,24 @@
 static int conv3d_k3_launch(int cfg, const mh_tensor5* in_, const float* packed_w, const float* bias, const mh_tensor5* out_, float* stats, void* stream, bool accumulate,
                             const PoolOut* pool = nullptr);
 int mh_conv3d_k3_pool_accepts(int cfg, int Cin, int Cout, int D, int H, int W);
-int mh_conv3d_k3_pool_f32(int cfg, const mh_tensor5* in_, const float* packed_w, const float* bias, const mh_tensor5* out_, float* stats, float* pool_max, float* pool_min,
-                          int64_t pool_n_stride, void* stream) {
+static int conv3d_k3_pool(int cfg, const mh_tensor5* in_, const float* packed_w, const float* bias, const mh_tensor5* out_, float* stats, float* pool_max, float* pool_min,
+                          int64_t pool_n_stride, void* stream, bool accumulate) {
     if (!in_ || !out_ || !pool_max || !pool_min || !stats || !in_->nrm) return fail(MH_ERR_ARG, "conv3d_k3_pool: input records, statistics and both pooled tensors are required");
     if (!mh_conv3d_k3_pool_accepts(cfg, in_->C, out_->C, out_->D, out_->H, out_->W))
         return fail(MH_ERR_UNSUPPORTED, "conv3d_k3_pool: the pooling epilogue exists for the split-precision configuration on even extents with 16 x 16 regions");
     if (!aligned(pool_max, 8) || !aligned(pool_min, 8) || pool_n_stride % 2 || (long long)out_->C * (out_->D / 2) * (out_->H / 2) * (out_->W / 2) > pool_n_stride)
         return fail(MH_ERR_ARG, "conv3d_k3_pool: pooled tensors must be 8-byte aligned [N][>= C][D/2][H/2][W/2]");
     const PoolOut po{pool_max, pool_min, (long long)pool_n_stride};
-    return conv3d_k3_launch(cfg, in_, packed_w, bias, out_, stats, stream, false, &po);
+    if (accumulate && cfg != MH_CFG_H2W) return fail(MH_ERR_UNSUPPORTED, "conv3d_k3_pool_accumulate: the accumulating pooling form exists for the Winograd split configuration");
+    return conv3d_k3_launch(cfg, in_, packed_w, bias, out_, stats, stream, accumulate, &po);
+}
+int mh_conv3d_k3_pool_f32(int cfg, const mh_tensor5* in_, const float* packed_w, const float* bias, const mh_tensor5* out_, float* stats, float* pool_max, float* pool_min,
+                          int64_t pool_n_stride, void* stream) {
+    return conv3d_k3_pool(cfg, in_, packed_w, bias, out_, stats, pool_max, pool_min, pool_n_stride, stream, false);
+}
+int mh_conv3d_k3_pool_accumulate_f32(int cfg, const mh_tensor5* in_, const float* packed_w, const float* bias, const mh_tensor5* out_, float* stats, float* pool_max,
+                                     float* pool_min, int64_t pool_n_stride, void* stream) {
+    return conv3d_k3_pool(cfg, in_, packed_w, bias, out_, stats, pool_max, pool_min, pool_n_stride, stream, true);
 }
 int mh_pool_select_f32(float* pool_max, const float* pool_min, const float* nrm, int64_t nrm_n_stride, int N, int C, int64_t n_stride, int64_t vol, void* stream) {
     if (!pool_max || !pool_min || !nrm || N < 1 || C < 1 || vol < 1) return fail(MH_ERR_ARG, "pool_select: bad argument");
@@ -668,22 +689,30 @@
     }
     if (cfg == MH_CFG_H2W) {
         if (!mh_conv3d_k3_accepts(cfg, in.C, out.C) || !hw_fits(in.D, in.H, in.W))
-            return fail(MH_ERR_ARG, "conv3d_k3: the Winograd split kernel needs Cin == 32, Cout %% 32 == 0, H %% 4 == 0, W %% 16 == 0, D*H*W < 2^24 (got %d -> %d, %dx%dx%d)",
+            return fail(MH_ERR_ARG, "conv3d_k3: the Winograd split kernel needs Cin == 32, Cout %% 32 == 0, H %% 4 == 0, W %% 16 == 0 (or H %% 8 == 0, W %% 8 == 0), D*H*W < 2^24 (got %d -> %d, %dx%dx%d)",
                         in.C, out.C, in.D, in.H, in.W);
         if (!in.nrm) return fail(MH_ERR_ARG, "conv3d_k3: the Winograd split kernel needs input records with magnitude bounds");
         if (!aligned(out.data, 16) || out.n_stride % 4 || !aligned(packed_w, 16)) return fail(MH_ERR_ARG, "conv3d_k3: the Winograd split kernel needs 16-byte aligned output and weights");
         if ((accumulate || pool) && !stats) return fail(MH_ERR_ARG, "conv3d_k3: the accumulating / pooling forms leave statistics");
-        const int bxn = out.W / HWG_BX, byn = out.H / HWG_BY, zc = hw_zchunk(out.D, out.H, out.W);
+        const bool g8 = hw_geo(out.H, out.W) == 1;
+        const int bxn = g8 ? out.W / 8 : out.W / HWG_BX, byn = g8 ? out.H / 8 : out.H / HWG_BY, zc = hw_zchunk(out.D, out.H, out.W);
         const unsigned nblk = (unsigned)(bxn * byn * cdiv(out.D, zc));
         const long long total = (long long)nblk * (out.C / HWG_CN) * out.N;
         if (total > 0x7fffffffLL) return fail(MH_ERR_UNSUPPORTED, "conv3d_k3: problem too large for one launch");
         const dim3 grid((unsigned)total);
         const uint4* wq = reinterpret_cast<const uint4*>(packed_w);
         const float* tail = packed_w + (mh_conv3d_k3_packed_floats(cfg, in.C, out.C) - H2_TAIL);
-        if (pool) hipLaunchKernelGGL((conv3d_k3_h2w_kernel<true, false, true>), grid, dim3(64 * HWG_WAVES), 0, s, in, wq, tail, bias, out, stats, bxn, byn, zc, nblk, pool->mx, pool->mn, pool->n_stride);
-        else if (accumulate) hipLaunchKernelGGL((conv3d_k3_h2w_kernel<true, true, false>), grid, dim3(64 * HWG_WAVES), 0, s, in, wq, tail, bias, out, stats, bxn, byn, zc, nblk, (float*)nullptr, (float*)nullptr, 0LL);
-        else if (stats) hipLaunchKernelGGL((conv3d_k3_h2w_kernel<true, false, false>), grid, dim3(64 * HWG_WAVES), 0, s, in, wq, tail, bias, out, stats, bxn, byn, zc, nblk, (float*)nullptr, (float*)nullptr, 0LL);
-        else hipLaunchKernelGGL((conv3d_k3_h2w_kernel<false, false, false>), grid, dim3(64 * HWG_WAVES), 0, s, in, wq, tail, bias, out, stats, bxn, byn, zc, nblk, (float*)nullptr, (float*)nullptr, 0LL);
+#define MH_HW_LAUNCH(ST_, ACC_, POOL_, MX_, MN_, PS_)                                                                                                    \
+    {                                                                                                                                                \
+        if (g8) hipLaunchKernelGGL((conv3d_k3_h2w_kernel<ST_, ACC_, POOL_, true>), grid, dim3(64 * HWG_WAVES), 0, s, in, wq, tail, bias, out, stats, bxn, byn, zc, nblk, MX_, MN_, PS_);   \
+        else hipLaunchKernelGGL((conv3d_k3_h2w_kernel<ST_, ACC_, POOL_, false>), grid, dim3(64 * HWG_WAVES), 0, s, in, wq, tail, bias, out, stats, bxn, byn, zc, nblk, MX_, MN_, PS_);     \
+    }
+        if (pool && accumulate) MH_HW_LAUNCH(true, true, true, pool->mx, pool->mn, pool->n_stride)
+        else if (pool) MH_HW_LAUNCH(true, false, true, pool->mx, pool->mn, pool->n_stride)
+        else if (accumulate) MH_HW_LAUNCH(true, true, false, (float*)nullptr, (float*)nullptr, 0LL)
+        else if (stats) MH_HW_LAUNCH(true, false, false, (float*)nullptr, (float*)nullptr, 0LL)
+        else MH_HW_LAUNCH(false, false, false, (float*)nullptr, (float*)nullptr, 0LL)
+#undef MH_HW_LAUNCH
         return launched("conv3d_k3_h2w");
     }
     if (cfg == MH_CFG_H2V) {
diff --git a/monai_amd/csrc/kernels/conv3d_wino_h2.h b/monai_amd/csrc/kernels/conv3d_wino_h2.h
--- a/monai_amd/csrc/kernels/conv3d_wino_h2.h
+++ b/monai_amd/csrc/kernels/conv3d_wino_h2.h
@@ -87,7 +87,7 @@
     return r;
 }
 
-template <bool STATS, bool ACC = false, bool POOL = false>
+template <bool STATS, bool ACC = false, bool POOL = false, bool G8 = false>
 __global__ void __launch_bounds__(512)
 conv3d_k3_h2w_kernel(Tensor in, const uint4* __restrict__ wp, const float* __restrict__ wtail, const float* __restrict__ bias, Tensor out,
                      float* __restrict__ stats, int bxn, int byn, int zchunk, unsigned nblk, float* __restrict__ pmax, float* __restrict__ pmin,
@@ -96,6 +96,10 @@
     __shared__ unsigned bound_s[4];
     char* const ds = smem;
     char* const zs_ = smem + 3 * HWG_DB;
+    constexpr int GBY = G8 ? 8 : HWG_BY, GBX = G8 ? 8 : HWG_BX;
+    constexpr int GRX = GBX + 2, GNP = (GBY + 2) * GRX;
+    constexpr int GPR = GRX / 2, GNL = (GBY + 2) * GPR;
+    static_assert(GNP <= HWG_NP && GNL <= 64, "the staged plane must fit the input buffers and one wave");
     const int tid = threadIdx.x, lane = tid & 63;
     const int wave = __builtin_amdgcn_readfirstlane(tid >> 6);
     const int wi = wave & 3, jp = wave >> 2;
@@ -108,24 +112,24 @@
     lid /= ncg;
     const unsigned b = lid % nblk;
     const int n = (int)(lid / nblk);
-    const int x0 = (int)(b % bxn) * HWG_BX, y0 = (int)((b / bxn) % byn) * HWG_BY;
+    const int x0 = (int)(b % bxn) * GBX, y0 = (int)((b / bxn) % byn) * GBY;
     const int zs = (int)(b / (bxn * byn)) * zchunk, ze = min(zs + zchunk, D);
     const int p_first = max(zs - 1, 0), p_last = min(ze, D - 1);
 
     unsigned soff;
     int loff[2];
     {
-        const int pr = min(lane, 53);
-        const int ly = pr / 9;
-        int lx = 2 * (pr - 9 * ly);
+        const int pr = min(lane, GNL - 1);
+        const int ly = pr / GPR;
+        int lx = 2 * (pr - GPR * ly);
         const int gy = y0 + ly - 1;
         int gx = x0 + lx - 1;
         if (gx < 0) { gx += 1; lx += 1; }
         if (gx + 1 >= W) { gx -= 1; lx -= 1; }
-        const bool ok = lane < 54 && gy >= 0 && gy < H;
+        const bool ok = lane < GNL && gy >= 0 && gy < H;
         soff = ok ? 4u * (unsigned)(gy * W + gx) : 0u;
-        loff[0] = (ok ? ly * HWG_RX + lx : HWG_NP) * HWG_PB;
-        loff[1] = (ok ? ly * HWG_RX + lx + 1 : HWG_NP) * HWG_PB;
+        loff[0] = (ok ? ly * GRX + lx : GNP) * HWG_PB;
+        loff[1] = (ok ? ly * GRX + lx + 1 : GNP) * HWG_PB;
     }
     for (int i = tid; i < (3 * HWG_DB + 2 * HWG_ZB) / 16; i += 512) reinterpret_cast<uint4*>(smem)[i] = make_uint4(0u, 0u, 0u, 0u);
     f32x4 nra, nrb, nrs;
@@ -190,13 +194,14 @@
 #define MH_HW_U(SL, T, CB, PC) __builtin_bit_cast(f16x8, wu[(((SL) * 3 + (T)) * 2 + (CB)) * 2 + (PC)])
 
     const int rho = lane & 15, kg = lane >> 4;
-    const int tty = (rho >= 4 && rho < 12) ? 1 : 0, ttx = rho < 4 ? rho : rho < 12 ? rho - 4 : rho - 8;
+    const int tty = G8 ? (rho < 8 ? rho >> 2 : 5 - (rho >> 2)) : (rho >= 4 && rho < 12) ? 1 : 0;
+    const int ttx = G8 ? (rho & 3) : rho < 4 ? rho : rho < 12 ? rho - 4 : rho - 8;
     const int ra = wi == 0 ? 0 : wi == 2 ? 2 : 1, rb = wi == 0 ? 2 : wi == 1 ? 2 : wi == 2 ? 1 : 3;
     const float sgn = wi == 1 ? 1.0f : -1.0f;
     const float fsg = jp ? -1.0f : 1.0f;
     const float m1 = h2_minus_one();
-    const int ab0 = ((2 * tty + ra) * HWG_RX + 2 * ttx + jp) * HWG_PB + kg * 16;
-    const int ab1 = ((2 * tty + rb) * HWG_RX + 2 * ttx + jp) * HWG_PB + kg * 16;
+    const int ab0 = ((2 * tty + ra) * GRX + 2 * ttx + jp) * HWG_PB + kg * 16;
+    const int ab1 = ((2 * tty + rb) * GRX + 2 * ttx + jp) * HWG_PB + kg * 16;
 
     f32x4 acc[3][2][2];
 #pragma unroll
@@ -209,7 +214,8 @@
     const HwFinish fr = hw_finish_role(wave, lane);
     const int fcb = wave >> 2, fty = (wave >> 1) & 1;
     const int fa = fr.fa, fq = fr.fq, frp = fr.frp, g4 = fr.g4;
-    const int ftx = 2 * fq;
+    const int ftx = G8 ? 2 * frp : 2 * fq;
+    const int frw = G8 ? (g4 < 2 ? g4 : 5 - g4) : fty;
     const int c16 = fr.co_l & 15;
     const int co_l = fr.co_l, co = cg * HWG_CN + co_l;
     const float bco = bias ? bias[co] : 0.0f;
@@ -224,7 +230,7 @@
         inv_b = hw_uniform(__uint_as_float((unsigned)(t2_ + 127) << 23));
     }
     const auto orsrc = __builtin_amdgcn_make_buffer_rsrc(out.data + (long long)n * out.n_stride + (long long)(cg * HWG_CN) * DHW, 0, (int)(HWG_CN * DHW * 4), 0x00020000);
-    const unsigned ooff = 4u * (unsigned)((long long)co_l * DHW + (long long)(y0 + 2 * fty + fa) * W + x0 + 2 * ftx);
+    const unsigned ooff = 4u * (unsigned)((long long)co_l * DHW + (long long)(y0 + 2 * frw + fa) * W + x0 + 2 * ftx);
     float pivot = 0.0f;
     bool have_c = false;
     f32x4 s1 = {0.0f, 0.0f, 0.0f, 0.0f}, s2 = s1;
@@ -233,7 +239,7 @@
     float* const pbase_mn = POOL ? pmin + (long long)n * pool_n_stride + (long long)(cg * HWG_CN) * PDHW : out.data;
     const int pbytes = POOL ? (int)(HWG_CN * PDHW * 4) : 0;
     const unsigned phw4 = (unsigned)(PHW * 4);
-    const unsigned poff = (4u * (unsigned)((long long)co_l * PDHW + (long long)((y0 >> 1) + fty) * (W / 2) + (x0 >> 1) + ftx)) | (fa ? HWG_DROP : 0u);
+    const unsigned poff = (4u * (unsigned)((long long)co_l * PDHW + (long long)((y0 >> 1) + frw) * (W / 2) + (x0 >> 1) + ftx)) | (fa ? HWG_DROP : 0u);
     const float pk_ = fa ? -__builtin_inff() : __builtin_inff();
     f32x2 hm = {0.0f, 0.0f};
     f32x4 pv = {0.0f, 0.0f, 0.0f, 0.0f};
@@ -336,6 +342,11 @@
             __builtin_amdgcn_sched_group_barrier(0x230, 1, 0);                                        \
         }                                                                                             \
     }
+#define MH_HW_OLD(QF, ST)                                                                             \
+    {                                                                                                 \
+        if (ST) pv = __builtin_bit_cast(f32x4, __builtin_amdgcn_raw_buffer_load_b128(orsrc, ooff, (unsigned)(QF) * hw4, 0)); \
+        else { const bool nx_ = (QF) >= zs && (QF) < ze; pv = __builtin_bit_cast(f32x4, __builtin_amdgcn_raw_buffer_load_b128(orsrc, nx_ ? ooff + (unsigned)(QF) * hw4 : HWG_DROP, 0, 0)); } \
+    }
 #define MH_HW_ITER(P, R, ST)                                                                          \
     {                                                                                                 \
         constexpr int S0 = (3 - (R)) % 3, S1 = (S0 + 1) % 3, S2 = (S0 + 2) % 3;       \
@@ -343,14 +354,12 @@
         const int p_ = (P);                                                                           \
         const bool valid_ = (ST) ? true : (p_ >= p_first && p_ <= p_last);                            \
         const int qf_ = p_ - 2;                                                                       \
-        if (ACC) {                                                                                    \
-            if (ST) pv = __builtin_bit_cast(f32x4, __builtin_amdgcn_raw_buffer_load_b128(orsrc, ooff, (unsigned)qf_ * hw4, 0)); \
-            else { const bool nx_ = qf_ >= zs && qf_ < ze; pv = __builtin_bit_cast(f32x4, __builtin_amdgcn_raw_buffer_load_b128(orsrc, nx_ ? ooff + (unsigned)qf_ * hw4 : HWG_DROP, 0, 0)); } \
-        }                                                                                             \
+        if (ACC && !POOL) MH_HW_OLD(qf_, ST)                                                          \
         if (valid_) { if (!(HWX_OFF & 1)) MH_HW_XFORM(db0) }                                          \
         MH_HW_T(0)                                                                                    \
         __syncthreads();                                                                              \
         MH_HW_T(1)                                                                                    \
+        if (ACC && POOL) MH_HW_OLD(qf_, ST)                                                           \
         if (valid_) {                                                                                 \
             __builtin_amdgcn_sched_barrier(0);                                                        \
             if (!(HWX_OFF & 2)) { MH_HW_CONV(db2) MH_HW_LDX MH_HW_ADV }                               \
@@ -394,6 +403,7 @@
 #undef MH_HW_T
 #undef MH_HW_DEAL
 #undef MH_HW_ITER
+#undef MH_HW_OLD
 #undef MH_HW_FINISH
 #undef MH_HW_ZOUT
 #undef MH_HW_SKIP
diff --git a/monai_amd/networks/_conv_engine.py b/monai_amd/networks/_conv_engine.py
--- a/monai_amd/networks/_conv_engine.py
+++ b/monai_amd/networks/_conv_engine.py
@@ -110,7 +110,7 @@
         stats = (own if stats is None else stats) if tiles else None
         with _prof.span(f"conv3d_k3/cfg{cfg}", 2.0 * 27 * x.shape[1] * cout * d * h * w * n):
             if pool is not None:
-                ops.conv3d_k3_pool(cfg, x, x_nrm, packed, bias, out, stats, *pool)
+                ops.conv3d_k3_pool(cfg, x, x_nrm, packed, bias, out, stats, *pool, accumulate=accumulate)
             else:
                 ops.conv3d_k3(cfg, x, x_nrm, packed, bias, out, stats, accumulate=accumulate)
         return stats, tiles
@@ -144,6 +144,18 @@
         self.launch3(cfg, x[:, :at], x_nrm[:, :at], self.conv3_pack(conv, cfg, cin=(0, at)), b if bias_on == "first" else None, out, want_stats=False)
         return self.launch3(cfg, x[:, at:], x_nrm[:, at:], self.conv3_pack(conv, cfg, cin=(at, cin)), b if bias_on == "second" else None, out, accumulate=True)
 
+    def conv3_slices(self, conv, cfg: int, x, x_nrm, out, width: int = 32, pool=None):
+        cin = x.shape[1]
+        if cin % width or cin < 2 * width:
+            raise RuntimeError(f"monai_amd: conv3_slices needs at least two whole slices of {width} input channels, got {cin}")
+        cuts = [(lo, lo + width) for lo in range(0, cin, width)]
+        packs = [self.conv3_pack(conv, cfg, cin=c) for c in cuts]
+        res = None
+        for i, ((lo, hi), packed) in enumerate(zip(cuts, packs)):
+            last = i == len(cuts) - 1
+            res = self.launch3(cfg, x[:, lo:hi], x_nrm[:, lo:hi], packed, conv.bias if last else None, out, want_stats=i > 0, accumulate=i > 0, pool=pool if last else None)
+        return res
+
     def norm_record(self, raw, stats, tiles: int, norm, slope: float, groups: Optional[int] = None, out=None):
         n, c = raw.shape[:2]
         if not tiles:
diff --git a/monai_amd/networks/nets/basic_unet.py b/monai_amd/networks/nets/basic_unet.py
--- a/monai_amd/networks/nets/basic_unet.py
+++ b/monai_amd/networks/nets/basic_unet.py
@@ -270,32 +270,34 @@
         cin = x.shape[1]
         bounded = x_nrm is not None and bounded and not self.batchnorm
         pool = None
+        scfg = self._slices_cfg(net, cin, cout, d, h, w, bounded)
         if (pool_level and self._slope(net, block.adn) >= 0.0
-                and self._poolable(net, ops.conv3d_k3_select(cin, cout, d, h, w, bounded=bounded), cin, cout, d, h, w, pool_level, x_nrm)):
+                and self._poolable(net, scfg if scfg >= 0 else ops.conv3d_k3_select(cin, cout, d, h, w, bounded=bounded), 32 if scfg >= 0 else cin, cout, d, h, w, pool_level, x_nrm)):
             if self.pool_min[pool_level] is None:
                 self.pool_min[pool_level] = torch.empty_like(self.pool[pool_level])
             pool = (self.pool[pool_level], self.pool_min[pool_level])
-        _, stats, tiles = net._engine.conv3(block.conv, x, x_nrm, out=out, bounded=bounded, want_stats=net.fused_stats and not self.batchnorm, pool=pool)
+        if scfg >= 0:
+            stats, tiles = net._engine.conv3_slices(block.conv, scfg, x, x_nrm, out, pool=pool)
+        else:
+            _, stats, tiles = net._engine.conv3(block.conv, x, x_nrm, out=out, bounded=bounded, want_stats=net.fused_stats and not self.batchnorm, pool=pool)
         self._record(net, block, out, stats, tiles, out_nrm)
         if pool is not None:
             ops.pool_select(*pool, out_nrm)
         return pool is not None
 
+    def _slices_cfg(self, net, cin: int, cout: int, d: int, h: int, w: int, bounded: bool) -> int:
+        if not config.conv_halves() or self.batchnorm or not net.fused_stats or not bounded or cin % 32 or cin < 64:
+            return -1
+        h2, _, hw = split_configs()
+        if ops.conv3d_k3_select(32, cout, d, h, w, bounded=True) != hw or ops.conv3d_k3_select(cin, cout, d, h, w, bounded=True) != h2:
+            return -1
+        return hw
+
     def _halves_cfg(self, net, l: int, cout: int, bounded: bool) -> int:
-        f = net.features
-        if not config.conv_halves() or self.batchnorm or not net.fused_stats or not bounded or 2 * f[l] != int(self.cat[l].shape[1]):
-            return -1
-        _, _, d, h, w = self.cat[l].shape
-        cfg = ops.conv3d_k3_select(f[l], cout, d, h, w, bounded=True)
-        if cfg != split_configs()[2] or ops.conv3d_k3_select(2 * f[l], cout, d, h, w, bounded=True) == cfg:
-            return -1
-        return cfg
+        return self._slices_cfg(net, int(self.cat[l].shape[1]), cout, *self.cat[l].shape[2:], bounded)
 
     def _conv_halves(self, net, block: _Convolution, l: int, cfg: int, out, out_nrm) -> None:
-        fl = net.features[l]
-        for half in ((0, fl), (fl, 2 * fl)):
-            net._engine.conv3_pack(block.conv, cfg, cin=half)
-        stats, tiles = net._engine.conv3_split(block.conv, cfg, self.cat[l], self.cat_nrm[l], fl, out, bias_on="second")
+        stats, tiles = net._engine.conv3_slices(block.conv, cfg, self.cat[l], self.cat_nrm[l], out)
         self._record(net, block, out, stats, tiles, out_nrm)
 
     def _poolable(self, net, cfg: int, cin: int, cout: int, d: int, h: int, w: int, level: int, x_nrm) -> bool:
diff --git a/monai_amd/ops.py b/monai_amd/ops.py
--- a/monai_amd/ops.py
+++ b/monai_amd/ops.py
@@ -257,7 +257,8 @@
 def conv3d_k3_select(cin: int, cout: int, d: int, h: int, w: int, bounded: bool = False, algo: Optional[int] = None) -> int:
     from . import config
 
-    cfg = _lib.lib().query("mh_conv3d_k3_select", config.conv_algo() if algo is None else int(algo), int(bool(bounded)), cin, cout, d, h, w)
+    family = (config.conv_algo() if algo is None else int(algo)) | (0x100 if config.h2w_8x8() else 0)
+    cfg = _lib.lib().query("mh_conv3d_k3_select", family, int(bool(bounded)), cin, cout, d, h, w)
     if not config.small_volume_h2() and cfg == _lib.lib().query("mh_conv3d_k3_h2v_config"):
         cfg = _lib.lib().query("mh_conv3d_k3_select", config.CONV_ALGOS["fp32"], int(bool(bounded)), cin, cout, d, h, w)
     return cfg
@@ -289,6 +290,10 @@
 
 def conv3d_k3_h2w_fits(d: int, h: int, w: int) -> bool:
     return bool(_lib.lib().query("mh_conv3d_k3_h2w_fits", int(d), int(h), int(w)))
+
+
+def conv3d_k3_h2w_geometry(d: int, h: int, w: int) -> int:
+    return int(_lib.lib().query("mh_conv3d_k3_h2w_geometry", int(d), int(h), int(w)))
 
 
 def conv3d_k3_accepts(cfg: int, cin: int, cout: int) -> bool:
@@ -320,12 +325,12 @@
     return bool(_lib.lib().query("mh_conv3d_k3_pool_accepts", int(cfg), int(cin), int(cout), int(d), int(h), int(w)))
 
 
-def conv3d_k3_pool(cfg, x, x_nrm, packed_w, bias, out, stats, pool_max: torch.Tensor, pool_min: torch.Tensor):
+def conv3d_k3_pool(cfg, x, x_nrm, packed_w, bias, out, stats, pool_max: torch.Tensor, pool_min: torch.Tensor, accumulate: bool = False):
     _lib.require_device(x, x_nrm, packed_w, bias, out, stats, pool_max, pool_min)
     if pool_max.shape != pool_min.shape or pool_max.stride() != pool_min.stride() or not pool_max[0].is_contiguous():
         raise RuntimeError("monai_amd.conv3d_k3_pool: pool_max / pool_min must be two equally laid out [N, C, D/2, H/2, W/2] tensors, dense per sample")
     xi, xo = _lib.tensor5(x, x_nrm), _lib.tensor5(out)
-    _lib.lib().call("mh_conv3d_k3_pool_f32", int(cfg), C.byref(xi), _lib.ptr(packed_w), _lib.ptr(bias), C.byref(xo), _lib.ptr(stats), _lib.ptr(pool_max), _lib.ptr(pool_min),
+    _lib.lib().call("mh_conv3d_k3_pool_accumulate_f32" if accumulate else "mh_conv3d_k3_pool_f32", int(cfg), C.byref(xi), _lib.ptr(packed_w), _lib.ptr(bias), C.byref(xo), _lib.ptr(stats), _lib.ptr(pool_max), _lib.ptr(pool_min),
                     int(pool_max.stride(0)), _s(x))
     return out
 
```
